# BUPT-GAMMA/GammaGL

Hardware: AMD Instinct MI355X
Metric: edges aggregated/sec, 3-layer GCN hidden=256 training step, ogbn-products-sized graph (higher is better)
Workload: dtype f32; 1 GPU; products: products-sized R-MAT, N=2449029, E=126167309 directed incl. self-loops, features 100->256x2->47, edge order=src, relabel=random, full-graph GCN train step (fwd+bwd+Adam), 6 aggregations/ste~; association=A (X W), hipgraph=no: eager launches, parallelism=1 GPU, rank0_local_edges=126167309, rank0_owned_rows=2449029, rank0_halo_rows=0, rank0_send_rows=0, matmul_precision=highest (IEEE f32), route=cpp

## Files before the change

### gammagl_amd/_lib.py

```python
import ctypes
import os
from ctypes import POINTER, c_char_p, c_float, c_int, c_int32, c_int64, c_size_t, c_void_p

import torch

_HERE = os.path.dirname(os.path.abspath(__file__))
HIP_LIB_PATH = os.path.join(_HERE, "lib", "libggl_mpops_hip.so")
HOST_LIB_PATH = os.path.join(_HERE, "lib", "libggl_mpops_host.so")

GGL_OK, GGL_EINVAL, GGL_EINDEX, GGL_EDTYPE, GGL_EHIP, GGL_EWORKSPACE = 0, -1, -2, -3, -4, -5
ABI_VERSION = 11


class SegPlanC(ctypes.Structure):

    _fields_ = [
        ("rowptr", c_void_p), ("perm", c_void_p), ("long_rows", c_void_p), ("chunk_ptr", c_void_p),
        ("n_long", c_int64), ("n_chunks", c_int64), ("chunk", c_int64), ("partial", c_void_p),
        ("N", c_int64), ("E", c_int64), ("row_order", c_void_p), ("xcd_run_rows", c_int64),
        ("long_order", c_void_p),
        ("max_len", c_int64),
    ]


# ... 30 lines not shown
    "ggl_plan_rows_bwd_rowptr": (c_int, [_V, _V, c_int64, c_int64, _V, _V, _V, _V, c_size_t, _V, POINTER(c_int64)]),
    "ggl_plan_rows_bwd_fill": (c_int, [_V, _V, _V, c_int64, _V, _V, _V, _V, _V]),
    "ggl_bias_grad_rows": (c_int, [_V, _V, c_int64, c_int64, c_int64, _V, _V, c_size_t, _V]),
    "ggl_partial_bytes": (c_size_t, [c_int, c_int64, c_int64, c_int]),
    "ggl_fill_i64": (c_int, [_V, c_int64, c_int64, _V]),
    "ggl_gather_i64_to_i32": (c_int, [_V, _V, c_int64, _V, _V]),
    "ggl_gather_rows_f32": (c_int, [_V, _V, c_int64, c_int64, _V, _V]),
    "ggl_gather_rows_f32_ex": (c_int, [_V, c_int64, _V, c_int64, c_int64, _V, c_int64, _V]),
    "ggl_ind2ptr_workspace_bytes": (c_size_t, [c_int64, c_int64]),
    "ggl_ind2ptr": (c_int, [_V, c_int64, c_int64, _V, _V, c_size_t, _V]),
    "ggl_ptr2ind": (c_int, [_V, c_int64, c_int64, _V, _V]),
    "ggl_sort_edges_workspace_bytes": (c_size_t, [c_int64, c_int64]),
    "ggl_sort_edges": (c_int, [_V, _V, c_int64, c_int64, _V, _V, c_size_t, _V]),
    "ggl_segment_sum": (c_int, [c_int, _V, _P, c_int64, _V, _V]),
    "ggl_segment_mean": (c_int, [c_int, _V, _P, c_int64, _V, _V]),
    "ggl_segment_max": (c_int, [c_int, _V, _P, c_int64, _V, _V, c_int64, _V]),
    "ggl_spmm_col_blocks": (c_int64, [c_int64, c_int64, c_int64]),
    "ggl_spmm_col_blocks_plan": (c_int64, [c_void_p, c_int64]),
    "ggl_segment_hub16_supported": (c_int, [c_int, c_int64, _V, _V]),
    "ggl_segment_hub16": (c_int, [c_int, c_int, _V, _P, c_int64, _V, _V]),
    "ggl_segment_sum_bwd": (c_int, [c_int, _V, _V, c_int64, c_int64, _V, _V]),
    "ggl_segment_mean_bwd": (c_int, [c_int, _V, _V, _V, c_int64, c_int64, _V, _V]),
    "ggl_segment_max_bwd": (c_int, [c_int, _V, _V, c_int64, c_int64, c_int64, _V, _V]),
    "ggl_spmm_sum": (c_int, [_P, _V, _V, c_int, _V, c_int64, _V, _V]),
    "ggl_spmm_sum_ex": (c_int, [_P, _V, _V, c_int, _V, c_int64, c_int64, _V, c_int64, c_int, _V]),
    "ggl_segment_sum_ex": (c_int, [c_int, _V, c_int64, _P, c_int64, _V, c_int64, c_int, _V]),
    "ggl_spmm_sum_bias_act": (c_int, [_P, _V, _V, c_int, _V, c_int64, _V, c_int, c_float, _V, _V, _V]),
    "ggl_spmm_mean": (c_int, [_P, _V, _V, c_int, _V, c_int64, _V, _V]),
    "ggl_spmm_max": (c_int, [_P, _V, _V, c_int, _V, c_int64, _V, _V, _V]),
    "ggl_spmm_mean_bwd": (c_int, [_P, _V, _V, c_int, _V, _V, c_int64, _V, _V]),
    "ggl_spmm_sum_x16": (c_int, [_P, _V, _V, c_int, c_int, _V, c_int64, c_int64, c_int, _V, c_int64, _V]),
    "ggl_spmm_mean_x16": (c_int, [_P, _V, _V, c_int, c_int, _V, c_int64, c_int64, c_int, _V, c_int64, _V]),
    "ggl_spmm_mean_bwd_x16": (c_int, [_P, _V, _V, c_int, c_int, _V, _V, c_int64, c_int, _V, _V]),
    "ggl_spmm_col_blocks_x16": (c_int64, [c_void_p, c_int64]),
    "ggl_spmm_max_bwd": (c_int, [_P, _V, _V, c_int, _V, _V, c_int64, _V, _V]),
    "ggl_spmm_max_bwd32": (c_int, [_P, _V, _V, c_int, _V, _V, c_int64, _V, _V]),
    "ggl_spmm_max_mask_bytes": (c_size_t, [c_int64, c_int64]),
    "ggl_spmm_max_mask": (c_int, [_P, _V, _V, c_int64, _V, _V]),
    "ggl_spmm_max_mask_words": (c_int64, [c_int64]),
    "ggl_spmm_max_bwd_mask": (c_int, [_P, _V, _V, c_int, _V, _V, _V, c_int64, _V, _V]),
    "ggl_bspmm_sum": (c_int, [_P, _V, _V, c_int, _V, c_int64, c_int64, _V, _V]),
    "ggl_bspmm_grad_w": (c_int, [_V, _V, _V, c_int64, c_int64, c_int64, _V, _V]),
    "ggl_bspmm_grad_w_sorted_scratch_bytes": (c_size_t, [c_int64, c_int64, c_int64, c_int64]),
    "ggl_bspmm_grad_w_sorted": (c_int, [_P, _V, _V, _V, _V, c_int64, c_int64, _V, _V, _V]),
    "ggl_spmm_grad_w_scratch_bytes": (c_size_t, [c_int64, c_int64, c_int64, c_int, c_int]),
    "ggl_spmm_grad_w": (c_int, [_P, _V, _V, c_int, _V, c_int, _V, _V, c_int64, _V, _V, _V]),
    "ggl_colsum_workspace_bytes": (c_size_t, [c_int64, c_int64]),
    "ggl_colsum_f32": (c_int, [_V, c_int64, c_int64, _V, _V, c_size_t, _V]),
    "ggl_bias_act_fwd": (c_int, [_V, _V, c_int64, c_int64, c_int, c_float, _V, _V, _V]),
    "ggl_bias_act_bwd_workspace_bytes": (c_size_t, [c_int64, c_int64]),
    "ggl_bias_act_bwd": (c_int, [_V, _V, c_int64, c_int64, c_int, c_float, _V, _V, _V, _V, c_size_t, _V]),
    "ggl_spmm_epi_ex": (c_int, [_P, _V, _V, c_int, _V, c_int64, c_int64, _V, c_int64, c_int, c_int, _V, c_int64,
                                _V, c_int, c_float, _V, c_int64, c_int64, c_int, _V]),
    "ggl_spmm_epi_x16": (c_int, [_P, _V, _V, c_int, c_int, _V, c_int64, c_int64, c_int, _V, c_int64, c_int, _V, c_int64,
                                 _V, c_int, c_float, _V, c_int64, c_int64, c_int, _V]),
    "ggl_bias_act_fwd_x16": (c_int, [c_int, _V, _V, c_int64, c_int64, c_int, c_float, _V, _V, _V]),
    "ggl_bias_act_bwd_x16": (c_int, [c_int, _V, _V, c_int64, c_int64, c_int, c_float, _V, _V, _V, _V, c_size_t, _V]),
    "ggl_segment_epi": (c_int, [_V, _P, c_int64, c_int, _V, c_int64, _V, c_int, c_float, _V, _V, _V]),
    "ggl_gat_fused_fwd": (c_int, [_P, _V, _V, _V, _V, c_float, c_int64, c_int64, c_float, _V, _V, _V, _V, _V]),
    "ggl_gat_partial_bytes": (c_size_t, [c_int64, c_int64, c_int64]),
    "ggl_gat_fused_bwd_dst": (c_int, [_P, _V, _V, _V, _V, _V, _V, _V, _V, _V, c_float, c_int64, c_int64,
                                      c_float, _V, _V, _V, _V, _V, _V]),
    "ggl_gat_fused_bwd_src": (c_int, [_P, _V, _V, _V, _V, _V, c_int64, c_int64, _V, _V, _V]),
    "ggl_edge_softmax_agg_fwd": (c_int, [_P, _V, _V, _V, c_int64, c_int64, c_float, _V, _V, _V, _V, _V]),
    "ggl_edge_softmax_agg_bwd_dst": (c_int, [_P, _V, _V, _V, _V, _V, _V, _V, c_int64, c_int64, c_float, _V, _V, _V, _V]),
    "ggl_edge_softmax_agg_bwd_src": (c_int, [_P, _V, _V, _V, _V, c_int64, c_int64, _V, _V]),
    "ggl_dot_attn_supported": (c_int, [c_int64, c_int64]),
    "ggl_policy_dot_attn_fused": (c_int, [c_int64, c_int64, c_int64, c_int64]),
    "ggl_dot_attn_fwd": (c_int, [_P, _V, _V, _V, _V, c_float, c_int64, c_int64, c_float, _V, _V, _V, _V, _V, _V]),
    "ggl_gat_fused_fwd_x16": (c_int, [_P, _V, _V, _V, c_int, _V, c_float, c_int64, c_int64, c_float, _V, c_int, _V, _V, _V,
                                      _V]),
    "ggl_gat_fused_bwd_dst_x16": (c_int, [_P, _V, _V, _V, c_int, _V, c_int, _V, c_int, _V, _V, _V, c_float, c_int64,
                                          c_int64, c_float, _V, _V, _V, _V, _V]),
    "ggl_gat_fused_bwd_src_x16": (c_int, [_P, _V, _V, _V, _V, c_int, _V, c_int64, c_int64, c_int, _V, _V, _V]),
    "ggl_gat_fast_supported": (c_int, [c_int64, c_int64]),
    "ggl_gat_fast_fwd": (c_int, [_P, _V, _V, _V, _V, c_int64, c_float, c_int64, c_int64, c_float, _V, _V, _V, _V, _V]),
    "ggl_gat_fast_bwd": (c_int, [_P, _V, _P, _V, _V, _V, _V, _V, _V, _V, _V, _V, c_float, c_int64, c_int64, c_float,
                                 _V, _V, _V, _V, _V, _V]),
    "ggl_gat_sh_supported": (c_int, [c_int64, c_int64, c_int64]),
    "ggl_gat_sh_partial_bytes": (c_size_t, [c_int64, c_int64]),
    "ggl_gat_sh_fwd": (c_int, [_P, _V, _V, _V, _V, c_int64, c_float, c_float, _V, _V, _V, _V, _V]),
    "ggl_gat_sh_stats": (c_int, [_V, _V, _V, _V, _V, c_int64, c_int64, _V, _V]),
    "ggl_gat_sh_bwd": (c_int, [_P, _V, _P, _V, _V, _V, _V, c_int64, _V, _V, _V, _V, c_int64, c_float, c_float, _V,
                               _V, _V, _V, _V]),
    "ggl_segment_softmax_supported": (c_int, [c_int64]),
    "ggl_segment_softmax_partial_bytes": (c_size_t, [c_int64, c_int64]),
    "ggl_segment_softmax_fwd": (c_int, [_V, _P, c_int64, _V, _V]),
    "ggl_segment_softmax_bwd": (c_int, [_V, _V, _P, c_int64, _V, _V]),
    "ggl_sample_count": (c_int, [_V, _V, c_int64, c_int64, c_int64, c_int, _V, _V]),
    "ggl_sample_pick": (c_int, [_V, _V, _V, c_int64, c_int64, c_int, _V, _V, _V, _V, _V]),
    "ggl_sample_hop_workspace_bytes": (c_size_t, [c_int64, c_int64]),
    "ggl_sample_hop": (c_int, [_V, _V, _V, _V, c_int64, c_int64, c_int64, c_int64, c_int64, _V, _V, _V, _V, _V, _V, _V,
                               _V, c_size_t, _V]),
    "ggl_sample_hop_ex": (c_int, [_V, _V, _V, _V, c_int64, c_int64, c_int64, c_int64, c_int64, _V, _V, _V, _V, _V, _V, _V,
                                  _V, c_size_t, _V, _V]),
    "ggl_block_transpose_workspace_bytes": (c_size_t, [c_int64, c_int64]),
    "ggl_block_transpose": (c_int, [_V, _V, c_int64, c_int64, c_int64, _V, _V, _V, c_size_t, _V]),
    "ggl_set_option": (c_int, [c_char_p, c_int64]),
    "ggl_get_option": (c_int64, [c_char_p]),
    "ggl_option_name": (c_char_p, [c_int]),
    "ggl_policy_chunk": (c_int64, [c_int64]),
    "ggl_policy_spmm_width": (c_int64, [c_int, c_int64, c_int64, c_int64]),
    "ggl_policy_head_channels": (c_int64, [c_int64, c_int64, c_int64]),
    "ggl_policy_mean_bwd_prescale": (c_int, [c_int64, c_int64]),
    "ggl_policy_gradw_sorted": (c_int, [c_int64, c_int64]),
    "ggl_policy_maxbwd_form": (c_int, [c_int64, c_int64, c_int64]),
# ... 46 lines not shown
```

### gammagl_amd/autograd.py

```python
import ctypes
import math

import torch
from torch.autograd.function import once_differentiable

from ._lib import _DTYPE_CODE, _X16_DTYPES, _ptr


def _flat(bias, add=None):
    return (bias.contiguous().reshape(-1) if bias is not None else None), (add.contiguous() if add is not None else None)


def segment_function(op):

    class Segment(torch.autograd.Function):
        @staticmethod
        def forward(ctx, eng, x, ids, N):
            ctx.eng = eng
            plan = eng.seg_plan(ids, N)
            out, _ = eng._segment_fwd(op, x, plan)
            ctx.save_for_backward(ids, *((plan.rowptr,) if op == "mean" else ()))
            ctx.x_shape = x.shape
            return out

# ... 539 lines not shown
        eng.spmm_epi_into(blk.plan, blk.col, None, x, y, mean=True, add=a, bias=b, relu=relu)
        ctx.blk, ctx.has_add = blk, add is not None
        ctx.epi = (relu, 0.0, None, None if bias is None else bias.shape)
        ctx.save_for_backward(y)
        return y

    @staticmethod
    def backward(ctx, g):
        eng = ctx.eng
        (y,) = ctx.saved_tensors
        ga, gb = eng._epi_bwd(g, y, *ctx.epi)
        gx = None
        if ctx.needs_input_grad[1]:
            blk = ctx.blk
            planT, dstT = blk.transposed()
            gx, _ = eng._spmm_fwd("mean_bwd", planT, dstT, None, ga, blk.n_src_cap, aux=blk.rowptr)
        return None, gx, None, (ga if ctx.has_add else None), gb, None


class SpMMRows(torch.autograd.Function):

    @staticmethod
    def forward(ctx, eng, gp, w, x, rows, bias):
        ctx.eng = eng
        dev = x.device
        K = int(x.shape[1])
        rp = eng.rows_plan(gp, w, rows)
        y = torch.empty((rp.R, K), dtype=torch.float32, device=dev)
        b, _ = _flat(bias)
        eng.spmm_epi_into(rp.fwd, rp.col, rp.w_fwd, x, y, bias=b)
        ctx.rp, ctx.bshape, ctx.K = rp, (None if bias is None else bias.shape), K
        return y

    @staticmethod
    @once_differentiable
    def backward(ctx, g):
        eng = ctx.eng
        rp, K = ctx.rp, ctx.K
        g = g.contiguous()
        dev = g.device
        gb = None
        if ctx.bshape is not None and ctx.needs_input_grad[5]:
            gb = torch.empty(K, dtype=torch.float32, device=dev)
            wsb = eng.lib.ggl_bias_act_bwd_workspace_bytes(rp.N_dst, K)
            ws = torch.empty(max(wsb, 4), dtype=torch.uint8, device=dev)
            eng._check(eng.lib.ggl_bias_grad_rows(_ptr(g), _ptr(rp.rows), rp.R, rp.N_dst, K, _ptr(gb), _ptr(ws), wsb,
                                                  eng._stream(dev)))
            gb = gb.reshape(ctx.bshape)
        gx = None
        if ctx.needs_input_grad[3]:
            gx = torch.empty((rp.N_src, K), dtype=torch.float32, device=dev)
            eng.spmm_sum_into(rp.bwd, rp.colT, rp.w_bwd, g, gx)
        return None, None, None, gx, None, gb
```

### gammagl_amd/cpp_ops.py

```python
import os

import torch

LIB_PATH = os.path.join(os.path.dirname(os.path.abspath(__file__)), "lib", "libggl_torch.so")
_loaded = False


def available():
    return os.path.exists(LIB_PATH)


def enabled():
    return available() and os.environ.get("GGL_CPP_OPS", "1") != "0"


def load():
    global _loaded
    if not _loaded:
        if not available():
            raise ImportError(f"{LIB_PATH} is not built: run `make -C gammagl_amd/csrc torch` "
                              f"(or __graft_entry__.build())")
        torch.ops.load_library(LIB_PATH)
        _loaded = True
    return torch.ops.ggl


def load_grad():
    load()
    return torch.ops.ggl_grad


def load_attn():
    load()
    return torch.ops.ggl_attn
```

### gammagl_amd/csrc/epilogue.hip

```cpp
#include "common.hpp"

namespace ggl {

struct alignas(8) H4 { uint16_t v[4]; };
template <typename T, int VEC> __device__ __forceinline__ void ldv(const typename TT<T>::S *__restrict__ p, float (&t)[VEC]) {
  if constexpr (!std::is_same<T, float>::value) {
    if (VEC == 4) {
      const H4 v = *reinterpret_cast<const H4 *>(p);
      t[0] = TT<T>::load(v.v[0]); t[1 % VEC] = TT<T>::load(v.v[1]); t[2 % VEC] = TT<T>::load(v.v[2]); t[3 % VEC] = TT<T>::load(v.v[3]);
    } else {
      t[0] = TT<T>::load(p[0]);
    }
  } else if (VEC == 4) {
    const float4 v = *reinterpret_cast<const float4 *>(p);
    t[0] = v.x; t[1 % VEC] = v.y; t[2 % VEC] = v.z; t[3 % VEC] = v.w;
  } else {
    t[0] = p[0];
  }
}
template <typename T, int VEC> __device__ __forceinline__ void stv(typename TT<T>::S *__restrict__ p, const float (&t)[VEC]) {
  if constexpr (!std::is_same<T, float>::value) {
    if (VEC == 4) {
      H4 o;
      o.v[0] = TT<T>::store(t[0]); o.v[1] = TT<T>::store(t[1 % VEC]); o.v[2] = TT<T>::store(t[2 % VEC]); o.v[3] = TT<T>::store(t[3 % VEC]);
// ... 125 lines not shown
      float gv[VEC], yv[VEC];
      ldv<T, VEC>(g + r * K + c * VEC, gv);
      if (MASKED == 1 || MASKED == 2) ldv<T, VEC>(y + r * K + c * VEC, yv);
      else yv[0] = 0.0f;
      finish(r, gv, yv);
    }
    if (partial) {
#pragma unroll
      for (int i = 0; i < VEC; ++i) partial[(block_id() * groups + j) * K + c * VEC + i] = acc[i];
    }
  }
}

static inline void geometry(int64_t N, int64_t K, bool vec4, int *kp, int *groups, int64_t *blocks,
                            int64_t *rpb) {
  const int64_t KV = vec4 ? K / 4 : K;
  *kp = (int)(KV < kBlock ? (KV > 0 ? KV : 1) : kBlock);
  *groups = kBlock / *kp;
  int64_t b = ceil_div(N > 0 ? N : 1, (int64_t)*groups * 8);
  if (b > 4096) b = 4096;
  if (b < 1) b = 1;
  *blocks = b;
  *rpb = ceil_div(N > 0 ? N : 1, b);
}

__global__ __launch_bounds__(kBlock) void bias_grad_rows_kernel(const float *__restrict__ g, const int64_t *__restrict__ rows,
                                                                int64_t R, int64_t N, int64_t K, int64_t nblocks,
                                                                int64_t rows_per_block, int kp, int groups,
                                                                float *__restrict__ partial) {
  const int j = threadIdx.x / kp;
  const int c0 = threadIdx.x - j * kp;
  if (j >= groups || block_id() >= nblocks) return;
  const int64_t KV = K / 4;
  const int64_t r0 = block_id() * rows_per_block;
  const int64_t r1 = (r0 + rows_per_block < N) ? r0 + rows_per_block : N;
  int64_t lo = 0, hi = R;
  while (lo < hi) {
    const int64_t mid = (lo + hi) >> 1;
    if (rows[mid] < r0) lo = mid + 1; else hi = mid;
  }
  for (int64_t c = c0; c < KV; c += kp) {
    float acc[4] = {0.0f, 0.0f, 0.0f, 0.0f};
    for (int64_t i = lo; i < R; ++i) {
      const int64_t r = rows[i];
      if (r >= r1) break;
      if ((int)(r - r0) % groups != j) continue;
      float gv[4];
      ldv<float, 4>(g + i * K + c * 4, gv);
#pragma unroll
      for (int k = 0; k < 4; ++k) acc[k] = __fadd_rn(acc[k], gv[k]);
    }
#pragma unroll
    for (int k = 0; k < 4; ++k) partial[(block_id() * groups + j) * K + c * 4 + k] = acc[k];
  }
}

int rng_advance(int64_t *rng_state, void *stream) {
  GGL_LAUNCH((rng_advance_kernel), 1, 64, as_stream(stream), rng_state, (int64_t)1);
  GGL_LAUNCH_CHECK();
  return GGL_OK;
}

}

using namespace ggl;

template <typename T> static inline bool aligned_v4(const void *p) {
  return (reinterpret_cast<uintptr_t>(p) & (4 * sizeof(typename TT<T>::S) - 1)) == 0;
}

template <typename T>
static int bias_act_fwd(const typename TT<T>::S *a, const float *bias, int64_t N, int64_t K, int relu, float p_drop,
                        int64_t *rng_state, typename TT<T>::S *y, void *stream) {
  GGL_REQUIRE(N >= 0 && K >= 0 && p_drop >= 0.0f && p_drop < 1.0f, GGL_EINVAL, "bad arguments");
  const int64_t total = N * K;
  if (total == 0) return GGL_OK;
  GGL_REQUIRE(a && y, GGL_EINVAL, "NULL pointer");
  GGL_REQUIRE(p_drop == 0.0f || rng_state, GGL_EINVAL, "dropout needs an rng_state");
  uint32_t thresh;
  float scale;
  dropout_params(p_drop, &thresh, &scale);
  hipStream_t s = as_stream(stream);
  const bool vec4 = (K % 4 == 0) && aligned_v4<T>(a) && aligned_v4<T>(y);
  int kp, groups;
  int64_t grid, rpb;
  geometry(N, K, vec4, &kp, &groups, &grid, &rpb);
  if (vec4)
    GGL_LAUNCH((bias_act_fwd_kernel<T, 4>), grid, kBlock, s, a, bias, (const int64_t *)rng_state, y, N, K, grid, rpb,
               kp, groups, relu, thresh, scale);
  else
    GGL_LAUNCH((bias_act_fwd_kernel<T, 1>), grid, kBlock, s, a, bias, (const int64_t *)rng_state, y, N, K, grid, rpb,
               kp, groups, relu, thresh, scale);
  GGL_LAUNCH_CHECK();
  if (thresh) return rng_advance(rng_state, stream);
  return GGL_OK;
}

extern "C" int ggl_bias_act_fwd(const float *a, const float *bias, int64_t N, int64_t K, int relu,
                                float p_drop, int64_t *rng_state, float *y, void *stream) {
  return bias_act_fwd<float>(a, bias, N, K, relu, p_drop, rng_state, y, stream);
}

static int x16_dtype_ok(int dtype, const char *what) {
  if (dtype == GGL_F16 || dtype == GGL_BF16) return GGL_OK;
  set_error("x16: %s must be f16 or bf16 (got dtype code %d)", what, dtype);
  return GGL_EDTYPE;
// ... 29 lines not shown
                        void *workspace, size_t workspace_bytes, void *stream) {
  GGL_REQUIRE(N >= 0 && K >= 0 && p_drop >= 0.0f && p_drop < 1.0f, GGL_EINVAL, "bad arguments");
  if (K == 0) return GGL_OK;
  GGL_REQUIRE((g && ga) || N == 0, GGL_EINVAL, "NULL pointer");
  const bool redraw = p_drop > 0.0f && rng_used != nullptr && !relu;
  const int masked = relu ? 1 : (redraw ? 3 : (p_drop > 0.0f ? 2 : 0));
  uint32_t thresh;
  float scale;
  dropout_params(p_drop, &thresh, &scale);
  GGL_REQUIRE(!masked || masked == 3 || y || N == 0, GGL_EINVAL, "y is needed to rebuild the ReLU/dropout mask");
  GGL_REQUIRE(!gbias || (workspace && workspace_bytes >= ggl_bias_act_bwd_workspace_bytes(N, K)),
              GGL_EWORKSPACE, "bias_act_bwd workspace too small");
  const bool vec4 = (K % 4 == 0) && aligned_v4<T>(g) && aligned_v4<T>(ga) && (!masked || masked == 3 || aligned_v4<T>(y));
  int kp, groups;
  int64_t blocks, rpb;
  geometry(N, K, vec4, &kp, &groups, &blocks, &rpb);
  hipStream_t s = as_stream(stream);
  float *partial = gbias ? static_cast<float *>(workspace) : nullptr;
#define GGL_BAB(V, M)                                                                                    \
  GGL_LAUNCH((bias_act_bwd_kernel<T, V, M>), blocks, kBlock, s, g, y, ga, N, K, blocks, rpb, kp, groups, scale, \
             redraw ? rng_used : nullptr, thresh, partial)
  if (vec4) {
    if (masked == 0) GGL_BAB(4, 0); else if (masked == 1) GGL_BAB(4, 1); else if (masked == 2) GGL_BAB(4, 2); else GGL_BAB(4, 3);
  } else {
    if (masked == 0) GGL_BAB(1, 0); else if (masked == 1) GGL_BAB(1, 1); else if (masked == 2) GGL_BAB(1, 2); else GGL_BAB(1, 3);
  }
#undef GGL_BAB
  GGL_LAUNCH_CHECK();
  if (gbias) {
    const size_t part = bwd_partial_bytes(N, K);
    return ggl_colsum_f32(partial, blocks * groups, K, gbias, static_cast<char *>(workspace) + part,
                          workspace_bytes - part, stream);
  }
  return GGL_OK;
}

extern "C" int ggl_bias_act_bwd(const float *g, const float *y, int64_t N, int64_t K, int relu,
                                float p_drop, const int64_t *rng_used, float *ga, float *gbias,
                                void *workspace, size_t workspace_bytes, void *stream) {
  return bias_act_bwd<float>(g, y, N, K, relu, p_drop, rng_used, ga, gbias, workspace, workspace_bytes, stream);
}

extern "C" int ggl_bias_act_bwd_x16(int dtype, const void *g, const void *y, int64_t N, int64_t K, int relu, float p_drop,
                                    const int64_t *rng_used, void *ga, float *gbias, void *workspace,
                                    size_t workspace_bytes, void *stream) {
  if (int rc = x16_dtype_ok(dtype, "g / y / ga")) return rc;
  const uint16_t *g16 = static_cast<const uint16_t *>(g), *y16 = static_cast<const uint16_t *>(y);
  uint16_t *ga16 = static_cast<uint16_t *>(ga);
  return dtype == GGL_BF16
             ? bias_act_bwd<mxbf16_t>(g16, y16, N, K, relu, p_drop, rng_used, ga16, gbias, workspace, workspace_bytes, stream)
             : bias_act_bwd<mxf16_t>(g16, y16, N, K, relu, p_drop, rng_used, ga16, gbias, workspace, workspace_bytes, stream);
}

extern "C" int ggl_bias_grad_rows(const float *g, const int64_t *rows, int64_t R, int64_t N, int64_t K, float *gbias,
                                  void *workspace, size_t workspace_bytes, void *stream) {
  GGL_REQUIRE(R >= 0 && N >= 0 && R <= N && K > 0 && K % 4 == 0, GGL_EINVAL,
              "bias_grad_rows needs R <= N rows of a multiple of 4 columns");
  GGL_REQUIRE(gbias && ((g && rows) || R == 0), GGL_EINVAL, "NULL pointer");
  GGL_REQUIRE(aligned16(g), GGL_EINVAL, "g must be 16-byte aligned");
  GGL_REQUIRE(workspace && workspace_bytes >= ggl_bias_act_bwd_workspace_bytes(N, K), GGL_EWORKSPACE,
              "bias_grad_rows workspace too small (ggl_bias_act_bwd_workspace_bytes(N, K))");
  int kp, groups;
  int64_t blocks, rpb;
  geometry(N, K, true, &kp, &groups, &blocks, &rpb);
  float *partial = static_cast<float *>(workspace);
  GGL_LAUNCH((bias_grad_rows_kernel), blocks, kBlock, as_stream(stream), g, rows, R, N, K, blocks, rpb, kp, groups, partial);
  GGL_LAUNCH_CHECK();
  const size_t part = bwd_partial_bytes(N, K);
  return ggl_colsum_f32(partial, blocks * groups, K, gbias, static_cast<char *>(workspace) + part, workspace_bytes - part,
                        stream);
}
```

### gammagl_amd/csrc/reduce.hip

```cpp
#include "common.hpp"

namespace ggl {

enum Mode {
  MODE_SEG = 0,
  MODE_SPMM = 1,
  MODE_BSPMM = 2,
  MODE_MEANBWD = 3,
  MODE_MAXBWD = 4,
  MODE_SPMM_EPI = 5,
  MODE_SEG_EPI = 6,
  MODE_MAXBWD32 = 7,
  MODE_MAXBWDM = 8
};
constexpr bool maxbwd_like(int mode) { return mode == MODE_MAXBWD || mode == MODE_MAXBWD32 || mode == MODE_MAXBWDM; }
constexpr bool spmm_like(int mode) { return mode == MODE_SPMM || mode == MODE_SPMM_EPI; }
constexpr bool seg_like(int mode) { return mode == MODE_SEG || mode == MODE_SEG_EPI; }
constexpr bool epi_mode(int mode) { return mode == MODE_SPMM_EPI || mode == MODE_SEG_EPI; }

enum IdxMode { IDX_RUNTIME = -1, IDX_NONE = 0, IDX_DIRECT = 1, IDX_PERM = 2 };

struct ReduceDims {
  int64_t N, K, E;
  int64_t arg_fill;
  int64_t chunk;
  int64_t nblocks;
  int64_t H, C;
  int64_t n_long, n_chunks;
  int64_t chunk_blocks;
  int exact_long;
  int logL;
  int swizzle;
  int w_by_pos;
  int64_t x_ld, out_ld;
  int accumulate;
  int epi_relu;
  int epi_vec;
  uint32_t epi_thresh;
  float epi_scale;
  int64_t epi_K, epi_col0;
  int64_t add_ld;
  int64_t mask_words;
  int64_t mask_col0;
};

template <typename S> struct RPtrs {
  const S *__restrict__ x;
  const int32_t *__restrict__ perm;
  const int32_t *__restrict__ col;
  const float *__restrict__ w;
  const int64_t *__restrict__ rowptr;
  const int64_t *__restrict__ aux_rowptr;
  const int64_t *__restrict__ aux_arg;
  const float *__restrict__ epi_bias;
  const int64_t *__restrict__ epi_rng;
  const S *__restrict__ epi_add;
};

template <typename S, int VEC> struct VecIO {
  static __device__ __forceinline__ void load(const S *__restrict__ p, S (&v)[VEC]) {
#pragma unroll
    for (int i = 0; i < VEC; ++i) v[i] = p[i];
  }
  static __device__ __forceinline__ void store(S *__restrict__ p, const S (&v)[VEC]) {
#pragma unroll
    for (int i = 0; i < VEC; ++i) p[i] = v[i];
  }
};
template <> struct VecIO<float, 4> {
  static __device__ __forceinline__ void load(const float *__restrict__ p, float (&v)[4]) {
    const float4 t = *reinterpret_cast<const float4 *>(p);
    v[0] = t.x; v[1] = t.y; v[2] = t.z; v[3] = t.w;
  }
  static __device__ __forceinline__ void store(float *__restrict__ p, const float (&v)[4]) {
    float4 t;
    t.x = v[0]; t.y = v[1]; t.z = v[2]; t.w = v[3];
    *reinterpret_cast<float4 *>(p) = t;
  }
};

template <> struct VecIO<float, 8> {
  static __device__ __forceinline__ void load(const float *__restrict__ p, float (&v)[8]) {
    const float4 t = *reinterpret_cast<const float4 *>(p), u = *reinterpret_cast<const float4 *>(p + 4);
    v[0] = t.x; v[1] = t.y; v[2] = t.z; v[3] = t.w; v[4] = u.x; v[5] = u.y; v[6] = u.z; v[7] = u.w;
  }
  static __device__ __forceinline__ void store(float *__restrict__ p, const float (&v)[8]) {
    float4 t, u;
    t.x = v[0]; t.y = v[1]; t.z = v[2]; t.w = v[3]; u.x = v[4]; u.y = v[5]; u.z = v[6]; u.w = v[7];
    *reinterpret_cast<float4 *>(p) = t;
    *reinterpret_cast<float4 *>(p + 4) = u;
  }
};
template <> struct VecIO<uint16_t, 8> {
  static __device__ __forceinline__ void load(const uint16_t *__restrict__ p, uint16_t (&v)[8]) {
    const uint4 t = *reinterpret_cast<const uint4 *>(p);
    v[0] = (uint16_t)t.x; v[1] = (uint16_t)(t.x >> 16); v[2] = (uint16_t)t.y; v[3] = (uint16_t)(t.y >> 16);
// ... 184 lines not shown
      for (int u = 0; u < TB; ++u) accumulate(raw[u], xrow[u], wv[u], who[u]);
    }
  }
  const int rem = (int)(end - p);
  if (rem > 0) {
    int64_t xrow[TB], who[TB];
    float wv[TB];
    S raw[TB][VEC];
#pragma unroll
    for (int u = 0; u < TB - 1; ++u)
      if (u < rem) element(p + u, xrow[u], wv[u], who[u]);
#pragma unroll
    for (int u = 0; u < TB - 1; ++u)
      if (u < rem) RowIO<S, VEC, RAG>::load(q.x + xrow[u] * d.x_ld + kk, raw[u], nv);
#pragma unroll
    for (int u = 0; u < TB - 1; ++u)
      if (u < rem) accumulate(raw[u], xrow[u], wv[u], who[u]);
  }
}

template <typename T, int VEC, int OP>
__device__ __forceinline__ void init_acc(typename TT<T>::A (&acc)[VEC], argreg_t (&arg)[VEC],
                                         int64_t arg_fill) {
#pragma unroll
  for (int i = 0; i < VEC; ++i) {
    acc[i] = (OP == OP_MAX) ? TT<T>::lowest() : TT<T>::zero();
    arg[i] = (argreg_t)arg_fill;
  }
}

template <typename T, int VEC, int OP, bool RAG = false>
__device__ __forceinline__ void seed_acc(const ReduceDims &d, const typename TO<T>::O *__restrict__ out,
                                         int64_t row, int64_t kk, typename TT<T>::A (&acc)[VEC]) {
  if (OP == OP_SUM && d.accumulate) {
    typename TO<T>::O o[VEC];
    RowIO<typename TO<T>::O, VEC, RAG>::load(out + row * d.out_ld + kk, o, valid_lanes<VEC, RAG>(d.K, kk));
#pragma unroll
    for (int i = 0; i < VEC; ++i) acc[i] = TO<T>::oload(o[i]);
  }
}

template <typename S, int VEC> struct EpiPre {
  float b[VEC];
  S a[VEC];
  uint32_t rw[VEC > 4 ? VEC : 4];
};
constexpr bool epi_late(int vec) { return vec > 4; }
template <int VEC, bool RAG>
__device__ __forceinline__ void epi_words(const int64_t *__restrict__ rng, const ReduceDims &d, int64_t row, int64_t kg, int nv,
                                          uint32_t (&rw)[VEC > 4 ? VEC : 4]) {
#pragma unroll
  for (int i = 0; i < (VEC > 4 ? VEC : 4); ++i) rw[i] = 0xffffffffu;
  if (!d.epi_thresh) return;
  const int64_t ev = d.epi_vec;
  const int sh = ev == 4 ? 2 : 0;
  const int64_t KV = (d.epi_K + ev - 1) >> sh;
  if (VEC > 1 && ev == 1 && (RAG || VEC > 4)) {
#pragma unroll
    for (int i = 0; i < VEC; ++i)
      rw[i] = i < nv ? philox4x32_10((uint64_t)(row * KV + kg + i), (uint64_t)rng[1], (uint64_t)rng[0]).x : 0xffffffffu;
  } else {
#pragma unroll
    for (int v = 0; v < (VEC > 4 ? VEC / 4 : 1); ++v) {
      const U4 u = philox4x32_10((uint64_t)(row * KV + (kg >> sh) + v), (uint64_t)rng[1], (uint64_t)rng[0]);
      rw[4 * v] = u.x; rw[4 * v + 1] = u.y; rw[4 * v + 2] = u.z; rw[4 * v + 3] = u.w;
    }
  }
}
template <typename T, int VEC, int MODE, bool RAG>
__device__ __forceinline__ void epi_prefetch(const RPtrs<typename TT<T>::S> &q, const ReduceDims &d, int64_t row,
                                             int64_t kk, EpiPre<typename TT<T>::S, VEC> &pre) {
  if (!epi_mode(MODE)) return;
  using S = typename TT<T>::S;
  const int nv = valid_lanes<VEC, RAG>(d.K, kk);
#pragma unroll
  for (int i = 0; i < VEC; ++i) pre.b[i] = (q.epi_bias && (!RAG || i < nv)) ? q.epi_bias[kk + i] : 0.0f;
  if (q.epi_add) RowIO<S, VEC, RAG>::load(q.epi_add + row * d.add_ld + kk, pre.a, nv);
  epi_words<VEC, RAG>(q.epi_rng, d, row, d.epi_col0 + kk, nv, pre.rw);
}

template <typename T, int VEC, int OP, int MODE, bool RAG = false>
__device__ __forceinline__ void finish_row(const RPtrs<typename TT<T>::S> &q, const ReduceDims &d,
                                           typename TO<T>::O *__restrict__ out,
                                           int64_t *__restrict__ argout, int64_t K, int64_t row,
                                           int64_t len, int64_t kk, typename TT<T>::A (&acc)[VEC],
                                           const argreg_t (&arg)[VEC], const EpiPre<typename TT<T>::S, VEC> &pre) {
  using O = typename TO<T>::O;
  const int nv = valid_lanes<VEC, RAG>(K, kk);
  if (OP == OP_MEAN) {
    if (seg_like(MODE)) {
      const typename TT<T>::A c = TT<T>::count(len);
      if (TT<T>::gt1(c)) {
#pragma unroll
        for (int i = 0; i < VEC; ++i) acc[i] = TT<T>::div(acc[i], c);
      }
    } else {
      if (len > 0) {
#pragma unroll
        for (int i = 0; i < VEC; ++i) acc[i] = (typename TT<T>::A)__fdiv_rn((float)acc[i], (float)len);
      }
    }
  }
  if (epi_mode(MODE)) {
    const int64_t ev = d.epi_vec;
    const int64_t kg = d.epi_col0 + kk;
    const uint32_t (&rw)[VEC > 4 ? VEC : 4] = pre.rw;
// ... 145 lines not shown
    init_acc<T, 1, OP>(acc, arg, d.arg_fill);
    seed_acc<T, 1, OP>(d, out, row, k, acc);
    for (int64_t c = c0; c < c1; ++c) {
      const A v = TO<T>::pload(partial[c * d.K + k]);
      if (OP == OP_MAX) {
        if (TT<T>::less(acc[0], v)) {
          acc[0] = v;
          arg[0] = (argreg_t)partial_arg[c * d.K + k];
        }
      } else {
        acc[0] = TT<T>::add(acc[0], v);
      }
    }
    EpiPre<typename TT<T>::S, 1> pre;
    epi_prefetch<T, 1, MODE, false>(q, d, row, k, pre);
    finish_row<T, 1, OP, MODE>(q, d, out, argout, d.K, row, len, k, acc, arg, pre);
  }
}

struct ReduceArgs {
  const void *x;
  const int32_t *perm;
  const int32_t *col;
  const float *w;
  int w_by_pos;
  const int64_t *rowptr;
  int64_t N, K, E;
  void *out;
  int64_t *arg;
  int64_t arg_fill;
  int64_t chunk;
  int64_t H, C;
  const int64_t *aux_rowptr;
  const int64_t *aux_arg;
  const int32_t *long_rows;
  const int64_t *chunk_ptr;
  const int32_t *row_order;
  const int32_t *long_order;
  int64_t max_len;
  int64_t xcd_run_rows;
  int64_t n_long, n_chunks;
  void *partial;
  int64_t *partial_arg;
  int64_t x_ld, out_ld;
  int accumulate;
  const float *epi_bias;
  const int64_t *epi_rng;
  int epi_relu;
  uint32_t epi_thresh;
  float epi_scale;
  const void *epi_add;
  int64_t add_ld;
  int64_t epi_K, epi_col0;
  int phase;
  int hub_forked;
  int64_t mask_words;
};

static inline int pow2_ceil_log2(int64_t v) {
  int l = 0;
  while (((int64_t)1 << l) < v) ++l;
  return l;
}

#define GGL_RPTR_ARGS(S)                                                                           \
  static_cast<const S *>(a.x), a.perm, a.col, a.w, a.rowptr, a.aux_rowptr, a.aux_arg, a.epi_bias, a.epi_rng, static_cast<const S *>(a.epi_add)

template <typename T, int OP, int MODE> constexpr bool exact_long_mode() {
  return OP != OP_MAX && ((std::is_same<T, float>::value && (seg_like(MODE) || spmm_like(MODE) || MODE == MODE_BSPMM)) ||
                          (std::is_same<T, double>::value && (MODE == MODE_SEG)) ||
                          (mx_code<T>::value != 0 && spmm_like(MODE)));
}

template <typename T, int OP, int MODE> static bool exact_long_applies(const ReduceArgs &a) {
#ifdef GGL_EMULATE
  return false;
#else
  if constexpr (exact_long_mode<T, OP, MODE>())
    return a.n_long > 0 && options().exact_long_rows != 0 && a.E < ((int64_t)1 << 31) &&
           (options().exact_long_max <= 0 || a.max_len <= options().exact_long_max);
  return false;
#endif
}

template <typename T, int MODE> static HubF32Args hub_args_of(const ReduceArgs &a, int64_t x_ld) {
  HubF32Args h{};
  constexpr int kWords = std::is_same<T, double>::value ? 2 : 1;
  h.f64 = kWords == 2 ? 1 : 0;
  h.x16 = mx_code<T>::value;
  h.x = reinterpret_cast<const float *>(a.x);
  h.x_ld = x_ld * kWords;
  h.perm = a.perm;
  h.col = seg_like(MODE) ? nullptr : a.col;
  h.w = seg_like(MODE) ? nullptr : a.w;
  h.w_by_pos = a.w_by_pos;
  h.H = a.H;
  h.C = (MODE == MODE_BSPMM) ? a.C : 0;
  h.rowptr = a.rowptr;
  h.long_rows = a.long_rows;
  h.long_order = a.long_order;
  h.n_long = a.n_long;
  h.K = a.K * kWords;
  h.partial = static_cast<float *>(a.partial);
  h.avg_long_len = a.n_chunks * a.chunk / (a.n_long > 0 ? a.n_long : 1);
  return h;
}
// ... 30 lines not shown
  }
#endif
  const int64_t grid = d.chunk_blocks + d.nblocks;
  GGL_REQUIRE(grid < ((int64_t)1 << 31), GGL_EINVAL, "grid too large");
  const int32_t *order = (options().row_order && (!uniform || options().row_order > 1)) ? a.row_order : nullptr;
#define GGL_RR_ARGS GGL_RPTR_ARGS(S), order, a.long_rows, a.chunk_ptr, static_cast<P *>(a.partial), a.partial_arg, out, a.arg, d
  if (a.phase == 2) {
  } else if (uniform) {
    if constexpr (!RAG) {
      if (std::is_same<T, float>::value && VEC == 4 && OP == OP_SUM && spmm_like(MODE) &&
          options().unroll >= 8) {
        GGL_LAUNCH((row_reduce_kernel<T, VEC, OP, MODE, IDX, std::is_same<T, float>::value, 8>), grid,
                   kBlock, stream, GGL_RR_ARGS);
      } else {
        GGL_LAUNCH((row_reduce_kernel<T, VEC, OP, MODE, IDX, std::is_same<T, float>::value, 4>), grid,
                   kBlock, stream, GGL_RR_ARGS);
      }
    }
  } else if (!RAG && (OP != OP_MAX || options().unroll_narrow_max) && d.logL <= 2 && options().unroll_narrow > 4) {
    GGL_LAUNCH((row_reduce_kernel<T, VEC, OP, MODE, IDX, false, 16>), grid, kBlock, stream, GGL_RR_ARGS);
  } else {
    GGL_LAUNCH((row_reduce_kernel<T, VEC, OP, MODE, IDX, false, 4, RAG>), grid, kBlock, stream, GGL_RR_ARGS);
  }
#undef GGL_RR_ARGS
  GGL_LAUNCH_CHECK();
  if (a.phase == 1) return GGL_OK;
#ifndef GGL_EMULATE
  if (forked) {
    const int rc = hub_f32_join(stream, forked);
    if (rc) return rc;
  }
#endif
  if (a.n_long > 0) {
    GGL_LAUNCH((long_final_kernel<T, OP, MODE>), a.n_long, kBlock, stream, a.rowptr, a.long_rows,
               a.chunk_ptr, static_cast<const P *>(a.partial), (const int64_t *)a.partial_arg, out,
               a.arg, a.epi_bias, a.epi_rng, static_cast<const S *>(a.epi_add), d);
    GGL_LAUNCH_CHECK();
  }
  return GGL_OK;
}

template <typename T, int VEC, int OP, int MODE, bool STATIC_IDX, bool RAG = false>
static int launch_typed(const ReduceArgs &a, hipStream_t stream) {
  ReduceDims d{};
  d.N = a.N; d.K = a.K; d.E = a.E; d.arg_fill = a.arg_fill; d.chunk = a.chunk; d.H = a.H; d.C = a.C;
  d.n_long = a.n_long; d.n_chunks = a.n_chunks; d.w_by_pos = a.w_by_pos;
  d.x_ld = a.x_ld > 0 ? a.x_ld : a.K; d.out_ld = a.out_ld > 0 ? a.out_ld : a.K; d.accumulate = a.accumulate;
  d.epi_relu = a.epi_relu; d.epi_thresh = a.epi_thresh; d.epi_scale = a.epi_scale;
  d.epi_K = a.epi_K > 0 ? a.epi_K : a.K; d.epi_col0 = a.epi_col0;
  d.epi_vec = (d.epi_K % 4 == 0) ? 4 : 1;
  d.add_ld = a.add_ld > 0 ? a.add_ld : a.K;
  d.mask_words = a.mask_words;
  d.mask_col0 = 0;
  const int64_t kv = ceil_div(a.K, VEC);
  d.logL = pow2_ceil_log2(kv < kWave ? kv : kWave);
  if (d.logL > 6) d.logL = 6;
  const int rows_per_block = kWavesPerBlock * (kWave >> d.logL);
  d.nblocks = ceil_div(a.N, rows_per_block);
  d.swizzle = (int)options().xcd_swizzle;
  if (a.xcd_run_rows > 0 && !d.swizzle) {
    const int64_t run_blocks = a.xcd_run_rows / rows_per_block;
    if (run_blocks >= 2 && d.nblocks >= 16 * run_blocks) d.swizzle = (int)run_blocks;
  }
  GGL_REQUIRE(d.nblocks < ((int64_t)1 << 30), GGL_EINVAL, "too many rows for one launch");
  GGL_REQUIRE(!RAG || (a.K >= VEC && !a.accumulate), GGL_EINVAL, "ragged rows: K >= the lane vector, no accumulate");
  if (a.N <= 0 || a.K <= 0) return GGL_OK;
  if constexpr (!STATIC_IDX || RAG) {
    return launch_idx<T, VEC, OP, MODE, IDX_RUNTIME, RAG>(a, d, stream);
  } else if constexpr (seg_like(MODE)) {
    if (a.perm) return launch_idx<T, VEC, OP, MODE, IDX_PERM>(a, d, stream);
    return launch_idx<T, VEC, OP, MODE, IDX_DIRECT>(a, d, stream);
  } else {
    if (!a.w) return launch_idx<T, VEC, OP, MODE, IDX_NONE>(a, d, stream);
    if (a.w_by_pos || !a.perm) return launch_idx<T, VEC, OP, MODE, IDX_DIRECT>(a, d, stream);
    return launch_idx<T, VEC, OP, MODE, IDX_PERM>(a, d, stream);
  }
}

template <int OP, int MODE>
static int launch_f32(const ReduceArgs &a, hipStream_t stream) {
  constexpr bool kStatic = (seg_like(MODE) || spmm_like(MODE) || MODE == MODE_MAXBWDM);
  const bool vec4 = !options().force_generic && (a.K % 4 == 0) && aligned16(a.x) &&
                    aligned16(a.out) && (!a.partial || aligned16(a.partial)) &&
                    (a.x_ld % 4 == 0) && (a.out_ld % 4 == 0) && (MODE != MODE_BSPMM || a.C % 4 == 0) &&
                    (!a.epi_add || (aligned16(a.epi_add) && a.add_ld % 4 == 0));
  if (vec4) return launch_typed<float, 4, OP, MODE, kStatic>(a, stream);
  if constexpr (seg_like(MODE) || spmm_like(MODE)) {
    if (!options().force_generic && options().ragged4 && a.K >= 32 && a.K <= 128 && !a.accumulate &&
        (OP != OP_MAX || spmm_like(MODE) || options().ragged_max))
      return launch_typed<float, 4, OP, MODE, kStatic, true>(a, stream);
  }
  return launch_typed<float, 1, OP, MODE, kStatic>(a, stream);
}

static int64_t col_block_width(int64_t E, int64_t K, int64_t N, int64_t xcd_run_rows = 0) {
  if (N > 0 && E < options().col_block_min_degree * N) return 0;
  int64_t bw = options().col_block;
  if (bw > 0 && E < options().col_block_min_edges) bw *= 2;
  else if (bw > 0 && xcd_run_rows > 0 && K >= 4 * bw && K % (2 * bw) == 0) bw *= 2;
  if (bw <= 0 || bw % 4 != 0 || K < 2 * bw || K % 4 != 0) return 0;
  if (K % bw != 0 && K <= 256) return 0;
  return bw;
}
extern "C" int64_t ggl_spmm_col_blocks(int64_t E, int64_t K, int64_t N) {
  const int64_t bw = col_block_width(E, K, N);
  return bw > 0 ? (K + bw - 1) / bw : 1;
// ... 275 lines not shown
}

extern "C" int ggl_spmm_sum(const ggl_segplan_t *plan, const int32_t *col, const float *w,
                            int w_by_pos, const float *x, int64_t K, float *out, void *stream) {
  return ggl_spmm_sum_ex(plan, col, w, w_by_pos, x, 0, K, out, 0, 0, stream);
}

extern "C" int ggl_spmm_sum_ex(const ggl_segplan_t *plan, const int32_t *col, const float *w, int w_by_pos,
                               const float *x, int64_t x_ld, int64_t K, float *out, int64_t out_ld,
                               int accumulate, void *stream) {
  ReduceArgs a{};
  int rc = spmm_common(a, plan, col, w, w_by_pos, x, K, out, false);
  if (rc) return rc;
  GGL_REQUIRE((x_ld == 0 || x_ld >= K) && (out_ld == 0 || out_ld >= K), GGL_EINVAL, "row stride < K");
  a.x_ld = x_ld; a.out_ld = out_ld; a.accumulate = accumulate ? 1 : 0;
  return launch_f32_cols<OP_SUM, MODE_SPMM>(a, as_stream(stream));
}

static int fill_epilogue(ReduceArgs &a, const void *add, int64_t add_ld, const float *bias, int relu, float p_drop,
                         int64_t *rng_state) {
  GGL_REQUIRE(p_drop >= 0.0f && p_drop < 1.0f, GGL_EINVAL, "p_drop must be in [0, 1)");
  GGL_REQUIRE(p_drop == 0.0f || rng_state, GGL_EINVAL, "dropout needs an rng_state");
  a.epi_bias = bias;
  a.epi_add = add; a.add_ld = add_ld;
  a.epi_rng = rng_state;
  a.epi_relu = relu ? 1 : 0;
  dropout_params(p_drop, &a.epi_thresh, &a.epi_scale);
  return GGL_OK;
}

extern "C" int ggl_spmm_epi_ex(const ggl_segplan_t *plan, const int32_t *col, const float *w, int w_by_pos,
                               const float *x, int64_t x_ld, int64_t K, float *out, int64_t out_ld,
                               int accumulate, int mean, const float *add, int64_t add_ld, const float *bias,
                               int relu, float p_drop, int64_t *rng_state, int64_t epi_K, int64_t epi_col0,
                               int advance_rng, void *stream) {
  ReduceArgs a{};
  int rc = spmm_common(a, plan, col, w, w_by_pos, x, K, out, false);
  if (rc) return rc;
  GGL_REQUIRE((x_ld == 0 || x_ld >= K) && (out_ld == 0 || out_ld >= K) && (add_ld == 0 || add_ld >= K),
              GGL_EINVAL, "row stride < K");
  GGL_REQUIRE(!(mean && accumulate), GGL_EINVAL, "mean cannot accumulate onto a partial result");
  rc = fill_epilogue(a, add, add_ld, bias, relu, p_drop, rng_state);
  if (rc) return rc;
  GGL_REQUIRE(epi_col0 >= 0 && (epi_K == 0 || epi_col0 + K <= epi_K), GGL_EINVAL, "column block outside the row");
  a.x_ld = x_ld; a.out_ld = out_ld; a.accumulate = accumulate ? 1 : 0;
  a.epi_K = epi_K; a.epi_col0 = epi_col0;
  rc = !mean ? launch_f32_cols<OP_SUM, MODE_SPMM_EPI>(a, as_stream(stream))
             : launch_f32_cols<OP_MEAN, MODE_SPMM_EPI>(a, as_stream(stream));
  if (rc) return rc;
  if (a.epi_thresh && advance_rng && plan->N > 0 && K > 0) return rng_advance(rng_state, stream);
  return GGL_OK;
}

extern "C" int ggl_spmm_sum_bias_act(const ggl_segplan_t *plan, const int32_t *col, const float *w,
                                     int w_by_pos, const float *x, int64_t K, const float *bias, int relu,
                                     float p_drop, int64_t *rng_state, float *out, void *stream) {
  return ggl_spmm_epi_ex(plan, col, w, w_by_pos, x, 0, K, out, 0, 0, 0, nullptr, 0, bias, relu, p_drop, rng_state, 0, 0, 1,
                         stream);
}

extern "C" int ggl_segment_epi(const float *x, const ggl_segplan_t *plan, int64_t K, int mean, const float *add,
                               int64_t add_ld, const float *bias, int relu, float p_drop, int64_t *rng_state,
                               float *out, void *stream) {
  ReduceArgs a{};
  int rc = fill_plan(a, plan, GGL_F32, K, false);
  if (rc) return rc;
  GGL_REQUIRE((x || plan->E * K == 0) && (out || plan->N * K == 0), GGL_EINVAL, "x/out is NULL");
  GGL_REQUIRE(add_ld == 0 || add_ld >= K, GGL_EINVAL, "row stride < K");
  rc = fill_epilogue(a, add, add_ld, bias, relu, p_drop, rng_state);
  if (rc) return rc;
  a.x = x;
  a.out = out;
  rc = mean ? launch_f32<OP_MEAN, MODE_SEG_EPI>(a, as_stream(stream))
            : launch_f32<OP_SUM, MODE_SEG_EPI>(a, as_stream(stream));
  if (rc) return rc;
  if (a.epi_thresh && plan->N > 0 && K > 0) return rng_advance(rng_state, stream);
  return GGL_OK;
}

extern "C" int ggl_spmm_mean(const ggl_segplan_t *plan, const int32_t *col, const float *w,
                             int w_by_pos, const float *x, int64_t K, float *out, void *stream) {
  ReduceArgs a{};
  int rc = spmm_common(a, plan, col, w, w_by_pos, x, K, out, false);
  if (rc) return rc;
  return launch_f32_cols<OP_MEAN, MODE_SPMM>(a, as_stream(stream));
}

extern "C" int ggl_spmm_max(const ggl_segplan_t *plan, const int32_t *col, const float *w,
                            int w_by_pos, const float *x, int64_t K, float *out, int64_t *argsrc,
                            void *stream) {
  ReduceArgs a{};
  int rc = spmm_common(a, plan, col, w, w_by_pos, x, K, out, true);
  if (rc) return rc;
  GGL_REQUIRE(argsrc || plan->N * K == 0, GGL_EINVAL, "argsrc is NULL");
  a.arg = argsrc;
  a.arg_fill = 0;
  return launch_f32<OP_MAX, MODE_SPMM>(a, as_stream(stream));
}

extern "C" int ggl_spmm_mean_bwd(const ggl_segplan_t *planT, const int32_t *colT, const float *w,
                                 int w_by_pos, const float *g, const int64_t *fwd_rowptr, int64_t K,
                                 float *gx, void *stream) {
  ReduceArgs a{};
  int rc = spmm_common(a, planT, colT, w, w_by_pos, g, K, gx, false);
  if (rc) return rc;
  GGL_REQUIRE(fwd_rowptr != nullptr, GGL_EINVAL, "fwd_rowptr is NULL");
// ... 295 lines not shown
```

### gammagl_amd/csrc/torch/ggl_torch.cpp

```cpp
#include <ATen/ATen.h>
#include <ATen/core/dispatch/Dispatcher.h>
#include <c10/core/DeviceGuard.h>
#include <c10/hip/HIPGraphsC10Utils.h>
#include <c10/hip/HIPStream.h>
#include <dlfcn.h>
#include <torch/csrc/autograd/custom_function.h>
#include <torch/library.h>

#include <cstdlib>
#include <cstring>
#include <list>
#include <memory>
#include <mutex>
#include <string>

#include "ggl_mpops.h"

namespace ggl_torch {

using at::Tensor;
using torch::autograd::AutogradContext;
using torch::autograd::variable_list;

#define GGL_FNS(X)                                                                                                  \
  X(ggl_abi_version) X(ggl_last_error) X(ggl_plan_workspace_bytes) X(ggl_plan_build) X(ggl_plan_long_workspace_bytes) \
  X(ggl_plan_long_count) X(ggl_plan_long_fill) X(ggl_partial_bytes) X(ggl_gather_i64_to_i32) X(ggl_gather_rows_f32)  \
  X(ggl_segment_sum) X(ggl_segment_mean) X(ggl_segment_max) X(ggl_segment_hub16_supported) X(ggl_segment_hub16)      \
  X(ggl_segment_sum_bwd) X(ggl_segment_mean_bwd) X(ggl_segment_max_bwd) X(ggl_spmm_sum) X(ggl_spmm_mean)             \
  X(ggl_spmm_max) X(ggl_spmm_mean_bwd) X(ggl_spmm_max_bwd) X(ggl_bspmm_sum) X(ggl_bspmm_grad_w)                      \
  X(ggl_bspmm_grad_w_sorted_scratch_bytes) X(ggl_bspmm_grad_w_sorted)                                                \
  X(ggl_spmm_grad_w_scratch_bytes) X(ggl_spmm_grad_w)                                                                \
  X(ggl_gat_partial_bytes) X(ggl_gat_fused_fwd) X(ggl_gat_fused_bwd_dst) X(ggl_gat_fused_bwd_src)                      \
  X(ggl_gat_fused_fwd_x16) X(ggl_gat_fused_bwd_dst_x16) X(ggl_gat_fused_bwd_src_x16)                                    \
  X(ggl_edge_softmax_agg_fwd) X(ggl_edge_softmax_agg_bwd_dst) X(ggl_edge_softmax_agg_bwd_src)                          \
  X(ggl_dot_attn_supported) X(ggl_policy_dot_attn_fused) X(ggl_dot_attn_fwd)                                           \
  X(ggl_gat_fast_supported) X(ggl_gat_fast_fwd) X(ggl_gat_fast_bwd) X(ggl_bias_act_fwd)                                \
  X(ggl_bias_act_bwd_workspace_bytes) X(ggl_bias_act_bwd) X(ggl_spmm_epi_ex) X(ggl_segment_epi)                        \
  X(ggl_sample_hop_workspace_bytes) X(ggl_sample_hop)                                                                \
  X(ggl_policy_chunk) X(ggl_policy_spmm_width) X(ggl_policy_head_channels) X(ggl_policy_mean_bwd_prescale)            \
  X(ggl_policy_gradw_sorted) X(ggl_policy_xcd_run_rows) X(ggl_policy_row_order)                                     \
  X(ggl_spmm_max_mask_bytes) X(ggl_spmm_max_mask) X(ggl_spmm_max_bwd_mask) X(ggl_get_option)                         \
  X(ggl_spmm_max_bwd32) X(ggl_policy_maxbwd_form)                                                                   \
  X(ggl_segment_softmax_supported) X(ggl_segment_softmax_partial_bytes) X(ggl_segment_softmax_fwd) X(ggl_segment_softmax_bwd) \
  X(ggl_policy_softmax_sublanes) X(ggl_spmm_sum_x16) X(ggl_spmm_mean_x16) X(ggl_spmm_mean_bwd_x16)                    \
  X(ggl_plan_rows_workspace_bytes) X(ggl_plan_rows_rank) X(ggl_plan_rows_fwd_rowptr) X(ggl_plan_rows_fwd_fill)        \
  X(ggl_plan_rows_bwd_rowptr) X(ggl_plan_rows_bwd_fill) X(ggl_bias_grad_rows)                                          \
  X(ggl_spmm_epi_x16) X(ggl_bias_act_fwd_x16) X(ggl_bias_act_bwd_x16)

struct Api {
  void *handle = nullptr;
  std::string path;
#define X(n) decltype(&::n) n = nullptr;
  GGL_FNS(X)
#undef X
};

static std::string here() {
  Dl_info info;
  if (dladdr(reinterpret_cast<void *>(&here), &info) == 0 || info.dli_fname == nullptr) return ".";
  std::string p(info.dli_fname);
  auto slash = p.rfind('/');
  return slash == std::string::npos ? "." : p.substr(0, slash);
}

static Api load(const char *env, const char *file, const char *what) {
  Api a;
  const char *over = std::getenv(env);
  a.path = over != nullptr ? std::string(over) : here() + "/" + file;
  a.handle = dlopen(a.path.c_str(), RTLD_NOW | RTLD_LOCAL);
  TORCH_CHECK(a.handle != nullptr, "gammagl_amd: cannot load ", a.path, " (", dlerror(), "): ", what,
              " tensors are served by this library only — build it with `make -C gammagl_amd/csrc`");
#define X(n)                                                                     \
  a.n = reinterpret_cast<decltype(a.n)>(dlsym(a.handle, #n));                    \
  TORCH_CHECK(a.n != nullptr, "gammagl_amd: ", a.path, " does not export " #n);
  GGL_FNS(X)
#undef X
  TORCH_CHECK(a.ggl_abi_version() == GGL_ABI_VERSION, "gammagl_amd: ", a.path, " has C ABI version ",
              a.ggl_abi_version(), ", this binding was built against ", GGL_ABI_VERSION);
  return a;
}

static const Api &api_for(const c10::Device &d) {
  if (d.is_cuda()) {
    static const Api hip = load("GGL_TORCH_HIP_LIB", "libggl_mpops_hip.so", "GPU");
    return hip;
  }
  TORCH_CHECK(d.is_cpu(), "gammagl_amd: no kernels for device ", d);
  static const Api host = load("GGL_TORCH_HOST_LIB", "libggl_mpops_host.so", "CPU");
  return host;
}

static void check(const Api &a, int rc) {
  if (rc == GGL_OK) return;
  const char *m = a.ggl_last_error();
  std::string msg(m != nullptr ? m : "");
  TORCH_CHECK_INDEX(rc != GGL_EINDEX, msg);
  TORCH_CHECK(false, "ggl_mpops error ", rc, ": ", msg);
}

static void *stream_of(const c10::Device &d) {
// ... 1257 lines not shown
  const Api &a = api_for(x.device());
  const int64_t K = s.x.size(1);
  if (add.defined()) {
    if (x16) {
      TORCH_CHECK(add.scalar_type() == s.x.scalar_type(), "expected scalar type Float (add in x's dtype, ", s.x.scalar_type(),
                  ") but found ", add.scalar_type(), " (add)");
    } else {
      f32("add", add);
    }
    TORCH_CHECK(add.dim() == 2 && add.size(0) == s.gp->N_dst && add.size(1) == K, "add must be [destination rows, feature width]");
    add = add.contiguous();
  }
  if (bias.defined()) {
    f32("bias", bias);
    bias = bias.contiguous().reshape({-1});
    TORCH_CHECK(bias.numel() == K, "bias must hold one value per column");
  }
  const SegPlan &p_ = *s.gp->fwd;
  Tensor y = at::empty({s.gp->N_dst, K}, s.x.options());
  Tensor part;
  if (x16) {
    if (p_.n_long > 0)
      part = at::empty({static_cast<int64_t>(a.ggl_partial_bytes(GGL_F32, p_.n_chunks, K, 0)) + 16}, s.x.options().dtype(at::kByte));
  } else {
    part = partial_for(a, p_, s.x, K, false);
  }
  ggl_segplan_t cs = p_.c(part);
  Tensor keep;
  auto [wp, by_pos] = weights_for(a, *s.gp, p_, s.w, keep);
  const Draw d = draw(x.device(), p);
  if (x16) {
    const int xc = dtype_code(s.x);
    check(a, a.ggl_spmm_epi_x16(&cs, s.gp->col.data_ptr<int32_t>(), wp, by_pos, xc, s.x.data_ptr(), K, K, xc, y.data_ptr(), K,
                                mean ? 1 : 0, add.defined() ? add.data_ptr() : nullptr, add.defined() ? K : 0,
                                bias.defined() ? bias.data_ptr<float>() : nullptr, relu ? 1 : 0, static_cast<float>(p), d.ptr(),
                                0, 0, 1, stream_of(x.device())));
    return {y, d.used};
  }
  check(a, a.ggl_spmm_epi_ex(&cs, s.gp->col.data_ptr<int32_t>(), wp, by_pos, s.x.data_ptr<float>(), K, K, y.data_ptr<float>(),
                             K, 0, mean ? 1 : 0, add.defined() ? add.data_ptr<float>() : nullptr, add.defined() ? K : 0,
                             bias.defined() ? bias.data_ptr<float>() : nullptr, relu ? 1 : 0, static_cast<float>(p),
                             d.ptr(), 0, 0, 1, stream_of(x.device())));
  return {y, d.used};
}

struct RowsPlan {
  int64_t R = 0, N_dst = 0, N_src = 0;
  Tensor rows, col, colT, w_fwd, w_bwd;
  std::shared_ptr<SegPlan> fwd, bwd;
  bool has_w = false;
  const void *w_storage = nullptr;
  int64_t w_offset = 0, w_version = 0;
  c10::optional<c10::weak_intrusive_ptr<c10::StorageImpl>> w_ref;
};

static Cache<RowsPlan> &rows_cache() {
  static Cache<RowsPlan> c(8);
  return c;
}

static std::shared_ptr<SegPlan> plan_from_rowptr(const Api &a, const Tensor &rowptr, int64_t E, int64_t chunk, void *st) {
  auto p = std::make_shared<SegPlan>();
  p->N = rowptr.size(0) - 1;
  p->E = E;
  p->chunk = chunk;
  p->rowptr = rowptr;
  p->sorted = true;
  p->max_len = p->N > 0 ? p->counts().max().item<int64_t>() : 0;
  fill_long_rows(a, *p, st);
  p->uid = ++g_plans_built;
  return p;
}

static std::shared_ptr<RowsPlan> rows_plan(GraphPlan &gp, const Tensor &index, const Tensor &w, const Tensor &rows_in) {
  TORCH_CHECK(rows_in.dim() == 1 && rows_in.scalar_type() == at::kLong, "rows must be a 1-D int64 tensor, got ", rows_in.sizes(),
              " ", rows_in.scalar_type());
  const void *w_storage = w.defined() ? w.storage().unsafeGetStorageImpl() : nullptr;
  const int64_t w_offset = w.defined() ? w.storage_offset() : 0;
  const int64_t w_version = (w.defined() && !w.is_inference()) ? static_cast<int64_t>(w._version()) : 0;
  TensorKey k = TensorKey::of(rows_in, static_cast<int64_t>(gp.fwd->uid),
                              static_cast<int64_t>(reinterpret_cast<uintptr_t>(w_storage)));
  if (auto hit = rows_cache().get(k)) {
    if (hit->has_w == w.defined() && hit->w_storage == w_storage && hit->w_offset == w_offset && hit->w_version == w_version &&
        (!hit->has_w || !hit->w_ref->expired())) {
      ++g_plan_hits;
      return hit;
    }
  }
  const auto dev = rows_in.device();
  TORCH_CHECK(!capturing(dev), "spmm_rows: the restricted plan of this row list must be built before a hipGraph capture "
                               "(run one eager step first)");
  const Api &a = api_for(dev);
  void *st = stream_of(dev);
  gp.need_bwd(index);
  Tensor rows = rows_in.contiguous();
  const int64_t R = rows.size(0), N = gp.N_dst, E = gp.E;
  auto i64 = rows.options(), i32 = rows.options().dtype(at::kInt), f32o = rows.options().dtype(at::kFloat);
  const size_t wsb = a.ggl_plan_rows_workspace_bytes(E, std::max(gp.N_dst, gp.N_src), R);
  Tensor ws = at::empty({static_cast<int64_t>(wsb)}, rows.options().dtype(at::kByte));
  Tensor rank = at::empty({std::max<int64_t>(N, 1)}, i32);
  check(a, a.ggl_plan_rows_rank(rows.data_ptr<int64_t>(), R, N, rank.data_ptr<int32_t>(), ws.data_ptr(), wsb, st));
  auto rp = std::make_shared<RowsPlan>();
  rp->R = R;
  rp->N_dst = gp.N_dst;
  rp->N_src = gp.N_src;
  rp->rows = rows;
// ... 33 lines not shown
                                       const OptT_ &bias_) {
  c10::OptionalDeviceGuard guard(x.device());
  SpArgs s = spmm_args(index, weight, x);
  Tensor bias = opt(bias_);
  same_device({&x, &rows, &bias});
  TORCH_CHECK(s.x.dim() == 2 && s.x.size(1) > 0 && s.x.size(1) % 4 == 0,
              "spmm_rows needs a 2-D f32 x whose width is a multiple of 4, got ", x.sizes());
  const Api &a = api_for(x.device());
  const int64_t K = s.x.size(1);
  if (bias.defined()) {
    f32("bias", bias);
    bias = bias.contiguous().reshape({-1});
    TORCH_CHECK(bias.numel() == K, "bias must hold one value per column");
  }
  auto rp = rows_plan(*s.gp, index, s.w, rows);
  const SegPlan &p_ = *rp->fwd;
  Tensor y = at::empty({rp->R, K}, s.x.options());
  Tensor part = partial_for(a, p_, s.x, K, false);
  ggl_segplan_t cs = p_.c(part);
  check(a, a.ggl_spmm_epi_ex(&cs, rp->col.data_ptr<int32_t>(), rp->has_w ? rp->w_fwd.data_ptr<float>() : nullptr, 1,
                             s.x.data_ptr<float>(), K, K, y.data_ptr<float>(), K, 0, 0, nullptr, 0,
                             bias.defined() ? bias.data_ptr<float>() : nullptr, 0, 0.0f, nullptr, 0, 0, 1, stream_of(x.device())));
  return y;
}

static std::tuple<Tensor, Tensor> spmm_rows_backward_kernel(const Tensor &index, const OptT_ &weight, const Tensor &grad,
                                                            const Tensor &rows, int64_t n_src, bool has_bias) {
  Tensor g = grad.contiguous(), w = opt_dense(weight);
  f32("grad", g);
  if (w.defined()) f32("weight", w);
  c10::OptionalDeviceGuard guard(g.device());
  const Api &a = api_for(g.device());
  auto gp = bwd_plan(index, n_src);
  auto rp = rows_plan(*gp, index, w, rows);
  TORCH_CHECK(g.dim() == 2 && g.size(0) == rp->R && g.size(1) % 4 == 0, "grad must be [len(rows), K], K a multiple of 4");
  const int64_t K = g.size(1);
  void *st = stream_of(g.device());
  Tensor gb = at::empty({has_bias ? K : 0}, g.options());
  if (has_bias) {
    const size_t wsb = a.ggl_bias_act_bwd_workspace_bytes(rp->N_dst, K);
    Tensor ws = at::empty({static_cast<int64_t>(std::max<size_t>(wsb, 4))}, g.options().dtype(at::kByte));
    check(a, a.ggl_bias_grad_rows(g.data_ptr<float>(), rp->rows.data_ptr<int64_t>(), rp->R, rp->N_dst, K, gb.data_ptr<float>(),
                                  ws.data_ptr(), wsb, st));
  }
  const SegPlan &p_ = *rp->bwd;
  Tensor gx = at::empty({rp->N_src, K}, g.options());
  Tensor part = partial_for(a, p_, g, K, false);
  ggl_segplan_t cs = p_.c(part);
  check(a, a.ggl_spmm_sum(&cs, rp->colT.data_ptr<int32_t>(), rp->has_w ? rp->w_bwd.data_ptr<float>() : nullptr, 1,
                          g.data_ptr<float>(), K, gx.data_ptr<float>(), st));
  return {gx, gb};
}

static Tensor segment_epi_forward_kernel(const Tensor &x_, const Tensor &index, int64_t N, bool mean, const OptT_ &add_,
                                         const OptT_ &bias_, bool relu) {
  seg_args(x_, index);
  Tensor x = x_.contiguous(), add = opt(add_), bias = opt(bias_);
  same_device({&x, &add, &bias});
  f32("msg", x);
  TORCH_CHECK(x.dim() == 2, "segment_epi expects [E, K] messages");
  c10::OptionalDeviceGuard guard(x.device());
  const Api &a = api_for(x.device());
  auto plan = seg_plan(index, N);
  const int64_t K = x.size(1);
  if (add.defined()) {
    f32("add", add);
    TORCH_CHECK(add.dim() == 2 && add.size(0) == N && add.size(1) == K, "add must be [num_segments, feature width]");
    add = add.contiguous();
  }
  if (bias.defined()) {
    f32("bias", bias);
    bias = bias.contiguous().reshape({-1});
    TORCH_CHECK(bias.numel() == K, "bias must hold one value per column");
  }
  Tensor y = at::empty({N, K}, x.options());
  Tensor part = partial_for(a, *plan, x, K, false);
  ggl_segplan_t cs = plan->c(part);
  check(a, a.ggl_segment_epi(x.data_ptr<float>(), &cs, K, mean ? 1 : 0, add.defined() ? add.data_ptr<float>() : nullptr, 0,
                             bias.defined() ? bias.data_ptr<float>() : nullptr, relu ? 1 : 0, 0.0f, nullptr,
                             y.data_ptr<float>(), stream_of(x.device())));
  return y;
}

static std::tuple<Tensor, Tensor, Tensor, Tensor, Tensor> sample_hop_kernel(const Tensor &rowptr, const Tensor &col,
                                                                            const Tensor &seeds, const Tensor &n_seeds,
                                                                            int64_t num_nodes, int64_t fanout, int64_t e_cap,
                                                                            int64_t s_cap, Tensor &first_pos) {
  same_device({&rowptr, &col, &seeds, &n_seeds, &first_pos});
  const Tensor *all5[5] = {&rowptr, &col, &seeds, &n_seeds, &first_pos};
  for (const Tensor *t : all5)
    TORCH_CHECK(t->scalar_type() == at::kLong && t->is_contiguous(), "sample_hop takes contiguous int64 tensors");
  TORCH_CHECK(fanout > 0 && first_pos.numel() >= num_nodes && rowptr.numel() == num_nodes + 1, "bad sample_hop arguments");
  c10::OptionalDeviceGuard guard(rowptr.device());
  const Api &a = api_for(rowptr.device());
  const int64_t b_cap = seeds.size(0);
  auto i64 = rowptr.options();
  Tensor out_rowptr = at::empty({b_cap + 1}, i64), out_col = at::empty({std::max<int64_t>(e_cap, 1)}, i64.dtype(at::kInt));
  Tensor out_eid = at::empty({std::max<int64_t>(e_cap, 1)}, i64), out_nid = at::empty({s_cap}, i64), counts = at::empty({3}, i64);
  const size_t wsb = a.ggl_sample_hop_workspace_bytes(b_cap, e_cap);
  Tensor ws = at::empty({static_cast<int64_t>(wsb)}, i64.dtype(at::kByte));
  Tensor rng = rng_state(rowptr.device());
  check(a, a.ggl_sample_hop(rowptr.data_ptr<int64_t>(), col.data_ptr<int64_t>(), seeds.data_ptr<int64_t>(),
                            n_seeds.data_ptr<int64_t>(), b_cap, num_nodes, fanout, e_cap, s_cap, rng.data_ptr<int64_t>(),
                            first_pos.data_ptr<int64_t>(), out_rowptr.data_ptr<int64_t>(), out_col.data_ptr<int32_t>(),
                            out_eid.data_ptr<int64_t>(), out_nid.data_ptr<int64_t>(), counts.data_ptr<int64_t>(), ws.data_ptr(),
                            wsb, stream_of(rowptr.device())));
// ... 359 lines not shown
    ctx->saved_data["p"] = p;
    ctx->saved_data["has_add"] = opt(add).defined();
    save_bias(ctx, bias);
    return std::get<0>(r);
  }
  static variable_list backward(AutogradContext *ctx, variable_list grads) {
    auto s = ctx->get_saved_variables();
    auto [ga, gb] = epi_backward(ctx, grads[0], s[2], ctx->saved_data["p"].toDouble(), s[3]);
    OptT_ w = s[1].defined() ? OptT_(s[1]) : OptT_();
    static auto sum_bwd = op_handle<SpSig>("ggl::spmm_sum_backward");
    static auto mean_bwd = op_handle<SpSig>("ggl::spmm_mean_backward");
    const bool mean = ctx->saved_data["mean"].toBool();
    Tensor gx = mean ? mean_bwd.call(s[0], w, ga) : sum_bwd.call(s[0], w, ga);
    return {Tensor(), grad_w(s, 4, ga, mean), gx, Tensor(), ctx->saved_data["has_add"].toBool() ? ga : Tensor(), gb, Tensor(),
            Tensor()};
  }
};
static Tensor spmm_epi_autograd(const Tensor &index, const OptT_ &weight, const Tensor &x, bool mean, const OptT_ &add,
                                const OptT_ &bias, bool relu, double p) {
  if (x.dim() == 2 && (x.size(1) % 4 == 0 || is_x16(x))) return SpMMEpiFn::apply(index, weight, x, mean, add, bias, relu, p);
  Tensor out = mean ? spmm_mean_autograd(index, weight, x) : spmm_sum_autograd(index, weight, x);
  if (opt(add).defined()) out = out + *add;
  return BiasActFn::apply(out, bias, relu, p);
}

struct SpMMRowsFn : public torch::autograd::Function<SpMMRowsFn> {
  static Tensor forward(AutogradContext *ctx, const Tensor &index, const OptT_ &weight, const Tensor &x, const Tensor &rows,
                        const OptT_ &bias) {
    at::AutoDispatchBelowADInplaceOrView below;
    static auto op = op_handle<Tensor(const Tensor &, const OptT_ &, const Tensor &, const Tensor &, const OptT_ &)>(
        "ggl::spmm_rows_forward");
    Tensor y = op.call(index, weight, x, rows, bias);
    ctx->save_for_backward({index, opt(weight), rows});
    ctx->saved_data["n_src"] = x.size(0);
    save_bias(ctx, bias);
    return y;
  }
  static variable_list backward(AutogradContext *ctx, variable_list grads) {
    auto s = ctx->get_saved_variables();
    static auto op = op_handle<std::tuple<Tensor, Tensor>(const Tensor &, const OptT_ &, const Tensor &, const Tensor &, int64_t,
                                                          bool)>("ggl::spmm_rows_backward");
    OptT_ w = s[1].defined() ? OptT_(s[1]) : OptT_();
    auto r = op.call(s[0], w, grads[0], s[2], ctx->saved_data["n_src"].toInt(), has_bias(ctx));
    return {Tensor(), Tensor(), std::get<0>(r), Tensor(), bias_grad(ctx, std::get<1>(r))};
  }
};
static Tensor spmm_rows_autograd(const Tensor &index, const OptT_ &weight, const Tensor &x, const Tensor &rows,
                                 const OptT_ &bias) {
  TORCH_CHECK(!(opt(weight).defined() && opt(weight).requires_grad()),
              "spmm_rows has no gradient for the edge weights: pass detached weights (bspmm_sum is the op with a weight gradient)");
  return SpMMRowsFn::apply(index, weight, x, rows, bias);
}

struct SegEpiFn : public torch::autograd::Function<SegEpiFn> {
  static Tensor forward(AutogradContext *ctx, const Tensor &x, const Tensor &index, int64_t N, bool mean, const OptT_ &add,
                        const OptT_ &bias, bool relu) {
    at::AutoDispatchBelowADInplaceOrView below;
    static auto op = op_handle<Tensor(const Tensor &, const Tensor &, int64_t, bool, const OptT_ &, const OptT_ &, bool)>(
        "ggl::segment_epi_forward");
    Tensor y = op.call(x, index, N, mean, add, bias, relu);
    ctx->save_for_backward({index, y});
    ctx->saved_data["x_shape"] = x.sizes().vec();
    ctx->saved_data["N"] = N;
    ctx->saved_data["mean"] = mean;
    ctx->saved_data["relu"] = relu;
    ctx->saved_data["has_add"] = opt(add).defined();
    save_bias(ctx, bias);
    return y;
  }
  static variable_list backward(AutogradContext *ctx, variable_list grads) {
    auto s = ctx->get_saved_variables();
    auto [ga, gb] = epi_backward(ctx, grads[0], s[1], 0.0, at::empty({0}, s[0].options()));
    auto shape = ctx->saved_data["x_shape"].toIntVector();
    Tensor gx;
    if (ctx->saved_data["mean"].toBool()) {
      static auto op = op_handle<Tensor(const Tensor &, const Tensor &, int64_t, c10::IntArrayRef)>("ggl::segment_mean_backward");
      gx = op.call(ga, s[0], ctx->saved_data["N"].toInt(), shape);
    } else {
      static auto op = op_handle<Tensor(const Tensor &, const Tensor &, c10::IntArrayRef)>("ggl::segment_sum_backward");
      gx = op.call(ga, s[0], shape);
    }
    return {gx, Tensor(), Tensor(), Tensor(), ctx->saved_data["has_add"].toBool() ? ga : Tensor(), gb, Tensor()};
  }
};
static Tensor segment_epi_autograd(const Tensor &x, const Tensor &index, int64_t N, bool mean, const OptT_ &add,
                                   const OptT_ &bias, bool relu) {
  return SegEpiFn::apply(x, index, N, mean, add, bias, relu);
}

static Tensor seg_meta(const Tensor &x, const Tensor &, int64_t N) { return at::empty(out_shape(x, N), x.options()); }
static std::tuple<Tensor, Tensor> seg_max_meta(const Tensor &x, const Tensor &, int64_t N) {
  return {at::empty(out_shape(x, N), x.options()), at::empty(out_shape(x, N), x.options().dtype(at::kLong))};
}
static Tensor like_x_meta(const Tensor &, const OptT &, const Tensor &x) { return at::empty_like(x); }
static Tensor x16_meta(const Tensor &, const OptT &, const Tensor &x, bool out_f32) {
  return out_f32 ? at::empty(x.sizes(), x.options().dtype(at::kFloat)) : at::empty_like(x);
}
static Tensor spmm_grad_w_meta(const Tensor &index, const Tensor &, const Tensor &g, bool) {
  return at::empty({index.size(1)}, g.options().dtype(at::kFloat));
}
static std::tuple<Tensor, Tensor> spmm_max_arg_meta(const Tensor &, const OptT &, const Tensor &x) {
  return {at::empty_like(x), at::empty(x.sizes(), x.options().dtype(at::kLong))};
}
static Tensor bspmm_meta(const Tensor &, const Tensor &, const Tensor &x) { return at::empty_like(x); }
static Tensor softmax_meta(const Tensor &x, const Tensor &, int64_t) { return at::empty_like(x); }
static Tensor softmax_bwd_meta(const Tensor &, const Tensor &y, const Tensor &, int64_t) { return at::empty_like(y); }
// ... 53 lines not shown
          at::empty({0}, o.dtype(at::kLong)), keep ? at::empty({index.size(1), v.size(1)}, o) : at::empty({0}, o)};
}
static std::tuple<Tensor, Tensor, Tensor> dot_bwd_meta(const Tensor &, const Tensor &q, const Tensor &k, const Tensor &v, const Tensor &,
                                                       const Tensor &, const Tensor &, const Tensor &, const Tensor &, const Tensor &,
                                                       int64_t, double, double, bool need_q, bool need_k, bool need_v) {
  auto e = [&]() { return at::empty({0}, v.options()); };
  return {need_q ? at::empty_like(q) : e(), need_k ? at::empty_like(k) : e(), need_v ? at::empty_like(v) : e()};
}
static Tensor dot_meta(const Tensor &, const Tensor &q, const Tensor &, const Tensor &v, c10::optional<int64_t> n,
                       c10::optional<double>, double) {
  const int64_t N = n.has_value() ? *n : q.size(0);
  if (v.dim() == 2) return at::empty({N, v.size(1)}, v.options());
  return at::empty({N, v.size(1), v.size(2)}, v.options());
}
static std::tuple<Tensor, Tensor, Tensor, Tensor, bool> gat_csr_fwd_meta(const Tensor &rp, const Tensor &, const Tensor &,
                                                                         const Tensor &, const Tensor &, const Tensor &,
                                                                         const Tensor &, const Tensor &x, double, double) {
  const int64_t n = rp.size(0) - 1;
  auto o = x.options(), f = x.options().dtype(at::kFloat);
  return {at::empty({n, x.size(1), x.size(2)}, o), at::empty({n, x.size(1)}, f), at::empty({n, x.size(1)}, f),
          at::empty({0}, o.dtype(at::kLong)), false};
}
static std::tuple<Tensor, Tensor, Tensor> gat_csr_bwd_meta(const Tensor &, const Tensor &, const Tensor &, const Tensor &,
                                                           const Tensor &, const Tensor &el, const Tensor &er, const Tensor &x,
                                                           const Tensor &, const Tensor &, const Tensor &, const Tensor &,
                                                           const Tensor &, double, double, bool) {
  return {at::empty_like(el), at::empty_like(er), at::empty_like(x)};
}
static Tensor gat_csr_meta(const Tensor &rp, const Tensor &, const Tensor &, const Tensor &, const Tensor &, const Tensor &,
                           const Tensor &, const Tensor &x, double, double) {
  return at::empty({rp.size(0) - 1, x.size(1), x.size(2)}, x.options());
}
static std::tuple<Tensor, Tensor> bias_fwd_meta(const Tensor &a, const OptT_ &, bool, double) {
  return {at::empty_like(a), at::empty({0}, a.options().dtype(at::kLong))};
}
static std::tuple<Tensor, Tensor> bias_bwd_meta(const Tensor &g, const Tensor &, bool hb, bool, double, const Tensor &) {
  const int64_t N = g.dim() > 0 ? g.size(0) : 1;
  return {at::empty_like(g), at::empty({hb && N > 0 ? g.numel() / N : 0}, g.options().dtype(at::kFloat))};
}
static Tensor bias_meta(const Tensor &a, const OptT_ &, bool, double) { return at::empty_like(a); }
static std::tuple<Tensor, Tensor> epi_fwd_meta(const Tensor &, const OptT_ &, const Tensor &x, bool, const OptT_ &, const OptT_ &,
                                               bool, double) {
  return {at::empty_like(x), at::empty({0}, x.options().dtype(at::kLong))};
}
static Tensor epi_meta(const Tensor &, const OptT_ &, const Tensor &x, bool, const OptT_ &, const OptT_ &, bool, double) {
  return at::empty_like(x);
}
static Tensor rows_meta(const Tensor &, const OptT_ &, const Tensor &x, const Tensor &rows, const OptT_ &) {
  return at::empty({rows.size(0), x.size(1)}, x.options());
}
static std::tuple<Tensor, Tensor> rows_bwd_meta(const Tensor &, const OptT_ &, const Tensor &g, const Tensor &, int64_t n_src,
                                                bool hb) {
  return {at::empty({n_src, g.size(1)}, g.options()), at::empty({hb ? g.size(1) : 0}, g.options())};
}
static Tensor seg_epi_meta(const Tensor &x, const Tensor &, int64_t N, bool, const OptT_ &, const OptT_ &, bool) {
  return at::empty(out_shape(x, N), x.options());
}

static void clear_caches() {
  seg_cache().clear();
  graph_cache().clear();
  csr_cache().clear();
  rows_cache().clear();
}
static std::vector<int64_t> plan_stats() {
  return {static_cast<int64_t>(g_plans_built.load()), static_cast<int64_t>(g_plan_hits.load())};
}

}

TORCH_LIBRARY(ggl, m) {
  m.def("segment_sum(Tensor x, Tensor index, int N) -> Tensor");
  m.def("segment_mean(Tensor x, Tensor index, int N) -> Tensor");
  m.def("segment_max(Tensor x, Tensor index, int N) -> (Tensor, Tensor)");
  m.def("segment_softmax(Tensor x, Tensor index, int N) -> Tensor");
  m.def("segment_softmax_backward(Tensor grad, Tensor y, Tensor index, int N) -> Tensor");
  m.def("spmm_sum(Tensor index, Tensor? weight, Tensor x) -> Tensor");
  m.def("spmm_mean(Tensor index, Tensor? weight, Tensor x) -> Tensor");
  m.def("spmm_max(Tensor index, Tensor? weight, Tensor x) -> Tensor");
  m.def("bspmm_sum(Tensor index, Tensor weight, Tensor x) -> Tensor");
  m.def("spmm_sum_x16(Tensor index, Tensor? weight, Tensor x, bool out_f32=False) -> Tensor");
  m.def("spmm_mean_x16(Tensor index, Tensor? weight, Tensor x, bool out_f32=False) -> Tensor");
  m.def("segment_sum_backward(Tensor grad, Tensor index, int[] x_shape) -> Tensor");
  m.def("segment_mean_backward(Tensor grad, Tensor index, int N, int[] x_shape) -> Tensor");
  m.def("segment_max_backward(Tensor grad, Tensor arg, int[] x_shape) -> Tensor");
  m.def("spmm_sum_backward(Tensor index, Tensor? weight, Tensor grad) -> Tensor");
  m.def("spmm_mean_backward(Tensor index, Tensor? weight, Tensor grad) -> Tensor");
  m.def("spmm_max_arg(Tensor index, Tensor? weight, Tensor x) -> (Tensor, Tensor)");
  m.def("spmm_max_backward(Tensor index, Tensor? weight, Tensor grad, Tensor arg) -> Tensor");
  m.def("bspmm_sum_backward(Tensor index, Tensor weight, Tensor x, Tensor grad) -> (Tensor, Tensor)");
  m.def("gat_fused(Tensor index, Tensor el, Tensor er, Tensor x, float negative_slope=0.2, int? num_nodes=None, "
        "float dropout_rate=0.0) -> Tensor");
  m.def("gat_fused_forward(Tensor index, Tensor el, Tensor er, Tensor x, float negative_slope, int num_nodes, "
        "float dropout_rate) -> (Tensor, Tensor, Tensor, Tensor, bool)");
  m.def("gat_fused_backward(Tensor index, Tensor el, Tensor er, Tensor x, Tensor grad, Tensor out, Tensor rowmax, "
        "Tensor rowden, Tensor rng_used, float negative_slope, int num_nodes, float dropout_rate, bool fast) -> "
        "(Tensor, Tensor, Tensor)");
  m.def("gat_fused_x16(Tensor index, Tensor el, Tensor er, Tensor x, float negative_slope=0.2, int? num_nodes=None, "
        "float dropout_rate=0.0, bool out_f32=False) -> Tensor");
  m.def("gat_fused_x16_forward(Tensor index, Tensor el, Tensor er, Tensor x, float negative_slope, int num_nodes, "
        "float dropout_rate, bool out_f32) -> (Tensor, Tensor, Tensor, Tensor)");
  m.def("gat_fused_csr(Tensor row_ptr, Tensor col_ind, Tensor col_ptr, Tensor row_ind, Tensor permute, Tensor el, "
        "Tensor er, Tensor x, float negative_slope=0.2, float dropout_rate=0.0) -> Tensor");
  m.def("gat_fused_csr_forward(Tensor row_ptr, Tensor col_ind, Tensor col_ptr, Tensor row_ind, Tensor permute, Tensor el, "
        "Tensor er, Tensor x, float negative_slope, float dropout_rate) -> (Tensor, Tensor, Tensor, Tensor, bool)");
  m.def("gat_fused_csr_backward(Tensor row_ptr, Tensor col_ind, Tensor col_ptr, Tensor row_ind, Tensor permute, Tensor el, "
// ... 72 lines not shown
  m.impl("bias_act", ggl_torch::bias_act_autograd);
  m.impl("spmm_epi", ggl_torch::spmm_epi_autograd);
  m.impl("segment_epi", ggl_torch::segment_epi_autograd);
  m.impl("spmm_rows", ggl_torch::spmm_rows_autograd);
}

TORCH_LIBRARY_IMPL(ggl, Meta, m) {
  m.impl("segment_sum", ggl_torch::seg_meta);
  m.impl("segment_mean", ggl_torch::seg_meta);
  m.impl("segment_max", ggl_torch::seg_max_meta);
  m.impl("segment_softmax", ggl_torch::softmax_meta);
  m.impl("segment_softmax_backward", ggl_torch::softmax_bwd_meta);
  m.impl("spmm_sum", ggl_torch::like_x_meta);
  m.impl("spmm_mean", ggl_torch::like_x_meta);
  m.impl("spmm_max", ggl_torch::like_x_meta);
  m.impl("bspmm_sum", ggl_torch::bspmm_meta);
  m.impl("spmm_sum_x16", ggl_torch::x16_meta);
  m.impl("spmm_mean_x16", ggl_torch::x16_meta);
  m.impl("segment_sum_backward", ggl_torch::seg_bwd_meta);
  m.impl("segment_mean_backward", ggl_torch::seg_mean_bwd_meta);
  m.impl("segment_max_backward", ggl_torch::seg_bwd_meta);
  m.impl("spmm_sum_backward", ggl_torch::like_x_meta);
  m.impl("spmm_mean_backward", ggl_torch::like_x_meta);
  m.impl("spmm_max_arg", ggl_torch::spmm_max_arg_meta);
  m.impl("spmm_max_backward", ggl_torch::spmm_max_bwd_meta);
  m.impl("bspmm_sum_backward", ggl_torch::bspmm_bwd_meta);
  m.impl("gat_fused", ggl_torch::gat_meta);
  m.impl("gat_fused_forward", ggl_torch::gat_fwd_meta);
  m.impl("gat_fused_x16", ggl_torch::gat_x16_meta);
  m.impl("gat_fused_x16_forward", ggl_torch::gat_x16_fwd_meta);
  m.impl("gat_fused_backward", ggl_torch::gat_bwd_meta);
  m.impl("gat_fused_csr", ggl_torch::gat_csr_meta);
  m.impl("gat_fused_csr_forward", ggl_torch::gat_csr_fwd_meta);
  m.impl("gat_fused_csr_backward", ggl_torch::gat_csr_bwd_meta);
  m.impl("bias_act", ggl_torch::bias_meta);
  m.impl("bias_act_forward", ggl_torch::bias_fwd_meta);
  m.impl("bias_act_backward", ggl_torch::bias_bwd_meta);
  m.impl("spmm_epi", ggl_torch::epi_meta);
  m.impl("spmm_epi_forward", ggl_torch::epi_fwd_meta);
  m.impl("segment_epi", ggl_torch::seg_epi_meta);
  m.impl("spmm_rows", ggl_torch::rows_meta);
  m.impl("spmm_rows_forward", ggl_torch::rows_meta);
  m.impl("spmm_rows_backward", ggl_torch::rows_bwd_meta);
  m.impl("segment_epi_forward", ggl_torch::seg_epi_meta);
}

TORCH_LIBRARY(ggl_grad, m) {
  m.def("spmm_grad_w(Tensor index, Tensor x, Tensor grad, bool mean) -> Tensor");
}
TORCH_LIBRARY_IMPL(ggl_grad, CPU, m) { m.impl("spmm_grad_w", ggl_torch::spmm_grad_w_kernel); }
TORCH_LIBRARY_IMPL(ggl_grad, CUDA, m) { m.impl("spmm_grad_w", ggl_torch::spmm_grad_w_kernel); }
TORCH_LIBRARY_IMPL(ggl_grad, Meta, m) { m.impl("spmm_grad_w", ggl_torch::spmm_grad_w_meta); }

TORCH_LIBRARY(ggl_attn, m) {
  m.def("edge_softmax_aggregate(Tensor index, Tensor logits, Tensor x, int? num_nodes=None, float dropout_rate=0.) -> Tensor");
  m.def("edge_softmax_aggregate_forward(Tensor index, Tensor logits, Tensor x, int num_nodes, float dropout_rate) -> "
        "(Tensor, Tensor, Tensor, Tensor)");
  m.def("edge_softmax_aggregate_backward(Tensor index, Tensor logits, Tensor x, Tensor grad, Tensor out, Tensor rowmax, "
        "Tensor rowden, Tensor rng_used, int num_nodes, float dropout_rate, bool need_logits, bool need_x) -> (Tensor, Tensor)");
  m.def("dot_attention(Tensor index, Tensor q, Tensor k, Tensor v, int? num_nodes=None, float? scale=None, "
        "float dropout_rate=0.) -> Tensor");
  m.def("dot_attention_forward(Tensor index, Tensor q, Tensor k, Tensor v, int num_nodes, float scale, float dropout_rate, "
        "bool keep_logits) -> (Tensor, Tensor, Tensor, Tensor, Tensor)");
  m.def("dot_attention_backward(Tensor index, Tensor q, Tensor k, Tensor v, Tensor logits, Tensor grad, Tensor out, "
        "Tensor rowmax, Tensor rowden, Tensor rng_used, int num_nodes, float scale, float dropout_rate, bool need_q, "
        "bool need_k, bool need_v) -> (Tensor, Tensor, Tensor)");
}
#define GGL_ATTN_IMPL(KEY)                                                                          \
  TORCH_LIBRARY_IMPL(ggl_attn, KEY, m) {                                                            \
    m.impl("edge_softmax_aggregate_forward", ggl_torch::esa_forward_kernel);                        \
    m.impl("edge_softmax_aggregate_backward", ggl_torch::esa_backward_kernel);                      \
    m.impl("dot_attention_forward", ggl_torch::dot_forward_kernel);                                 \
    m.impl("dot_attention_backward", ggl_torch::dot_backward_kernel);                               \
  }
GGL_ATTN_IMPL(CPU)
GGL_ATTN_IMPL(CUDA)
#undef GGL_ATTN_IMPL
TORCH_LIBRARY_IMPL(ggl_attn, Autograd, m) {
  m.impl("edge_softmax_aggregate", ggl_torch::esa_autograd);
  m.impl("dot_attention", ggl_torch::dot_autograd);
}
TORCH_LIBRARY_IMPL(ggl_attn, Meta, m) {
  m.impl("edge_softmax_aggregate", ggl_torch::esa_meta);
  m.impl("edge_softmax_aggregate_forward", ggl_torch::esa_fwd_meta);
  m.impl("edge_softmax_aggregate_backward", ggl_torch::esa_bwd_meta);
  m.impl("dot_attention", ggl_torch::dot_meta);
  m.impl("dot_attention_forward", ggl_torch::dot_fwd_meta);
  m.impl("dot_attention_backward", ggl_torch::dot_bwd_meta);
}
```

### gammagl_amd/dist.py

```python
import os
import time

import torch
import torch.distributed as dist
import torch.nn.functional as F

from . import engine as _default_engine
from .dense import wgrad

HALO_CHUNKS = int(os.environ.get("GGL_HALO_CHUNKS", "0"))
DIST_EXACT = os.environ.get("GGL_DIST_EXACT", "1") == "1"
A2A_MODE = os.environ.get("GGL_HALO_A2A", "a2a")
OUT_ROWS = os.environ.get("GGL_OUT_ROWS", "1") != "0"


def balanced_bounds(dst, num_nodes, world):
    deg = torch.bincount(dst, minlength=num_nodes)
    cum = torch.cumsum(deg, 0)
    total = int(cum[-1]) if num_nodes > 0 else 0
    targets = torch.arange(1, world, device=dst.device, dtype=torch.float64) * (total / world)
    cuts = torch.searchsorted(cum.double(), targets).clamp(max=num_nodes)
    return [0] + [int(c) for c in cuts.tolist()] + [int(num_nodes)]


class _Done:

    def wait(self):
        return True


class _Works:

    def __init__(self, works):
        self.works = list(works)

    def wait(self):
        for w in self.works:
            w.wait()
        return True


def _cpp_ops():
    from . import cpp_ops

    return cpp_ops.load()


def _default_route(eng):
    want = os.environ.get("GGL_ROUTE", "auto")
    if want not in ("auto", "cpp", "ctypes"):
        raise ValueError(f"GGL_ROUTE={want!r}: expected auto, cpp or ctypes")
    if want == "ctypes":
        return "ctypes"
    from . import cpp_ops

    product = getattr(eng, "is_product", False)
    if want == "cpp":
        if not cpp_ops.available():
            raise ImportError(f"GGL_ROUTE=cpp but {cpp_ops.LIB_PATH} is not built")
        return "cpp"
    return "cpp" if (product and cpp_ops.enabled()) else "ctypes"


class PartitionedGraph:

    def __init__(self, edge_index, edge_weight, num_nodes, rank=0, world=1, group=None, eng=None,
# ... 16 lines not shown
               send_rows=None):
        self.eng = eng if eng is not None else _default_engine()
        self.rank, self.world, self.group = rank, world, group
        self.route = _default_route(self.eng)
        self.dry = send_rows is not None
        self.comm = world > 1 or self_halo_from is not None or self.dry
        _apply_dist_exact(self)
        dev = s.device
        self.bounds = list(bounds)
        lo, hi = self.bounds[rank], self.bounds[rank + 1]
        self.lo, self.hi, self.n_local, self.n_global = lo, hi, hi - lo, int(num_nodes)
        self.e_global = int(e_global)
        self.e_local = int(s.shape[0])
        is_loc = (s >= lo) & (s < (hi if self_halo_from is None else int(self_halo_from)))
        self.ei_loc = torch.stack([s[is_loc] - lo, d[is_loc]]).contiguous()
        self.w_loc = w[is_loc].contiguous()
        self.gp_loc = self.eng.graph_plan(self.ei_loc, self.n_local, self.n_local)
        rem = ~is_loc
        rs, rd = s[rem], d[rem]
        self.halo_ids = torch.unique(rs)
        self.n_halo = int(self.halo_ids.shape[0])
        bt = torch.tensor(self.bounds, device=dev, dtype=torch.int64)
        owner_start = torch.searchsorted(self.halo_ids, bt)
        self.recv_splits = (owner_start[1:] - owner_start[:-1]).tolist()
        if self.n_halo > 0:
            self.ei_halo = torch.stack([torch.searchsorted(self.halo_ids, rs), rd]).contiguous()
            self.w_halo = w[rem].contiguous()
            self.gp_halo = self.eng.graph_plan(self.ei_halo, self.n_local, self.n_halo)
        else:
            self.ei_halo = self.w_halo = self.gp_halo = None
        del rs, rd, rem, is_loc
        if self.dry:
            self.send_splits = [int(t.numel()) for t in send_rows]
            self.send_idx = torch.cat([t.to(torch.int64) for t in send_rows]).contiguous()
        elif self.comm:
            rc = torch.tensor(self.recv_splits, device=dev, dtype=torch.int64)
            sc = torch.empty_like(rc)
            dist.all_to_all_single(sc, rc, group=group)
            self.send_splits = sc.tolist()
            req = torch.empty(int(sc.sum()), device=dev, dtype=torch.int64)
            dist.all_to_all_single(req, self.halo_ids.contiguous(), self.send_splits, self.recv_splits,
                                   group=group)
            self.send_idx = (req - lo).contiguous()
        else:
            self.send_splits = [0]
            self.send_idx = torch.empty(0, device=dev, dtype=torch.int64)
        assert self.send_idx.numel() == 0 or (int(self.send_idx.min()) >= 0 and int(self.send_idx.max()) < self.n_local)
        self.n_send = int(self.send_idx.shape[0])
        self.send_plan = self.eng.seg_plan(self.send_idx, self.n_local) if self.n_send > 0 else None
        self._bufs = {}
        self.halo_chunks = {}
        self._const = {}
        self.profile = None

    def _buf(self, tag, rows, cols, dtype, device):
        need = int(rows) * int(cols)
        b = self._bufs.get(tag)
        if b is None or b.device != device or b.dtype != dtype or b.numel() < need:
            b = torch.empty(max(need, 1), dtype=dtype, device=device)
            self._bufs[tag] = b
        return b[:need].view(int(rows), int(cols))

    def with_halo(self, x):
        if not self.comm:
            return x
        key = (x.untyped_storage()._cdata, x.storage_offset(), tuple(x.shape), x._version, str(x.device))
        hit = self._const.get(key)
        if hit is None:
            with torch.no_grad():
                xc = x.detach().contiguous()
                send = xc.index_select(0, self.send_idx) if self.n_send > 0 else xc.new_empty((0,) + tuple(xc.shape[1:]))
                recv = torch.empty((self.n_halo,) + tuple(xc.shape[1:]), dtype=xc.dtype, device=xc.device)
                if self.dry:
                    recv.zero_()
                else:
                    dist.all_to_all_single(recv, send, self.recv_splits, self.send_splits, group=self.group)
                hit = torch.cat([xc, recv], 0)
            self._const.clear()
            self._const[key] = hit
            self._const_ref = x
        return hit

    def _note(self, **kw):
        if self.profile is not None:
            for k, v in kw.items():
                self.profile[k] = self.profile.get(k, 0) + v

    def _timed_wait(self, work, dev):
        if self.profile is None:
            work.wait()
            return
        if dev.type == "cuda":
            e0, e1 = torch.cuda.Event(enable_timing=True), torch.cuda.Event(enable_timing=True)
            e0.record()
            work.wait()
            e1.record()
            self.profile.setdefault("_events", []).append((e0, e1))
        else:
            t0 = time.perf_counter()
            work.wait()
            self.profile["exposed_ms"] = self.profile.get("exposed_ms", 0.0) + (time.perf_counter() - t0) * 1e3

    def profile_summary(self, steps):
        p = dict(self.profile or {})
        ev = p.pop("_events", [])
        ms = p.pop("exposed_ms", 0.0) + sum(a.elapsed_time(b) for a, b in ev)
        s = max(int(steps), 1)
        return {"halo_exposed_ms": ms / s, "a2a_calls": p.get("a2a_calls", 0) / s,
                "a2a_GB_in": p.get("bytes_in", 0) / s / 1e9, "a2a_GB_out": p.get("bytes_out", 0) / s / 1e9}

    def _a2a(self, out_rows, inp, out_splits, in_splits, tag="a2a"):
        out = self._buf(tag, out_rows, inp.shape[1], inp.dtype, inp.device)
        self._note(a2a_calls=1, bytes_in=out.numel() * out.element_size(), bytes_out=inp.numel() * inp.element_size())
        if self.dry:
            out.zero_()
            return out, _Done()
        if A2A_MODE == "p2p":
            ops, o0, i0 = [], 0, 0
            me = dist.get_rank(self.group)
            for peer, (no, ni) in enumerate(zip(out_splits, in_splits)):
                if peer == me:
                    if no:
                        out[o0:o0 + no].copy_(inp[i0:i0 + ni])
                elif no or ni:
                    gpeer = dist.get_global_rank(self.group, peer) if self.group is not None else peer
                    if ni:
                        ops.append(dist.P2POp(dist.isend, inp[i0:i0 + ni], gpeer, group=self.group))
                    if no:
                        ops.append(dist.P2POp(dist.irecv, out[o0:o0 + no], gpeer, group=self.group))
                o0, i0 = o0 + no, i0 + ni
            return out, (_Works(dist.batch_isend_irecv(ops)) if ops else _Done())
        work = dist.all_to_all_single(out, inp, out_splits, in_splits, group=self.group, async_op=True)
        return out, work

    def release(self):
        _restore_dist_exact(self)

    def aggregate(self, h, bias=None, relu=False, p_drop=0.0, training=True, halo_included=False, out_rows=None):
        p = float(p_drop) if training else 0.0
        if out_rows is not None:
            if self.comm or halo_included or relu or p > 0 or h.shape[1] % 4 != 0:
                raise RuntimeError("aggregate(out_rows=...) is the one-GPU output layer's form: no halo, no ReLU / dropout, "
                                   "a feature width that is a multiple of 4")
            if self.route == "cpp":
                return _cpp_ops().spmm_rows(self.ei_loc, self.w_loc, h, out_rows, bias)
            return self.eng.spmm_rows(self.gp_loc, self.w_loc, h, out_rows, bias)
        if self.route == "cpp" and not self.comm and not halo_included and h.shape[1] % 4 == 0:
            return _cpp_ops().spmm_epi(self.ei_loc, self.w_loc, h, False, None, bias, bool(relu), p)
        return _HaloAggregate.apply(h, self, bias, bool(relu), p, bool(halo_included))


def _restore_dist_exact(pg):
    before = getattr(pg.eng, "_exact_before_dist", None)
    if before is not None:
        pg.eng.lib.ggl_set_option(b"exact_long_rows", int(before))
        del pg.eng._exact_before_dist


def _apply_dist_exact(pg):
    if pg.comm and not DIST_EXACT:
        if not hasattr(pg.eng, "_exact_before_dist"):
            pg.eng._exact_before_dist = int(pg.eng.lib.ggl_get_option(b"exact_long_rows"))
        pg.eng.lib.ggl_set_option(b"exact_long_rows", 0)
        import warnings

        warnings.warn("GGL_DIST_EXACT=0: library option exact_long_rows set to 0 for this process until "
                      "PartitionedGraph.release() (partitioned hub rows walk chunked)", stacklevel=3)


class _HaloAggregate(torch.autograd.Function):
    @staticmethod
    def _pad4(t):
        k = t.shape[1]
        return t if k % 4 == 0 else torch.nn.functional.pad(t, (0, (-k) % 4))

    @staticmethod
    def _chunks(K, pg=None, kind="exchange"):
        tuned = pg.halo_chunks.get(kind) if (pg is not None and K >= 128) else None
        n = HALO_CHUNKS if HALO_CHUNKS > 0 else tuned if tuned else (4 if K >= 256 else 2 if K >= 128 else 1)
        while n > 1 and K % (4 * n) != 0:
            n -= 1
        w = K // n
        return [(i * w, (i + 1) * w) for i in range(n)]

    @staticmethod
    def forward(ctx, h, pg, bias, relu, p_drop, pre=False):
        eng = pg.eng
        pre = bool(pre and pg.comm)
        if h.shape[0] != pg.n_local + (pg.n_halo if pre else 0):
            raise RuntimeError(f"aggregate: expected {pg.n_local + (pg.n_halo if pre else 0)} rows, got {h.shape[0]}")
        ctx.k_orig = h.shape[1]
        epi = bias is not None or relu or p_drop > 0
        fused = epi and h.shape[1] % 4 == 0
        h = _HaloAggregate._pad4(h.contiguous())
        K = h.shape[1]
        dev = h.device
# ... 129 lines not shown
        ctx.side, ctx.sink, ctx.pad_out = side, sink, int(pad_out)
        wt = w.t() if not pad_out else F.pad(w, (0, 0, 0, int(pad_out))).t()
        return x @ wt

    @staticmethod
    def backward(ctx, g):
        x, w = ctx.saved_tensors
        side, n_out = ctx.side, w.shape[0]
        gx = None
        if ctx.needs_input_grad[0]:
            gx = g @ (w if not ctx.pad_out else F.pad(w, (0, 0, 0, ctx.pad_out)))
        gw = None
        if ctx.needs_input_grad[1]:
            g = g.contiguous()
            if side is None or not g.is_cuda:
                gw = wgrad(g, x)[:n_out]
            else:
                cur = torch.cuda.current_stream(g.device)
                side.wait_stream(cur)
                with torch.cuda.stream(side):
                    gws = wgrad(g, x)[:n_out]
                gws.record_stream(cur)
                ctx.sink.append((w, gws, g, x))
        return gx, gw, None, None, None


class DistGCN(torch.nn.Module):

    def __init__(self, feature_dim, hidden_dim, num_class, num_layers=3, drop_rate=0.5, overlap_wgrad=True,
                 aggregate_first=False, const_input_halo=True):
        super().__init__()
        self.overlap_wgrad, self.aggregate_first = overlap_wgrad, aggregate_first
        self.const_input_halo = const_input_halo
        self.agg_per_step = 2 * num_layers
        dims = [feature_dim] + [hidden_dim] * (num_layers - 1) + [num_class]
        self.lin = torch.nn.ModuleList([torch.nn.Linear(a, b, bias=False) for a, b in zip(dims[:-1], dims[1:])])
        self.bias = torch.nn.ParameterList([torch.nn.Parameter(torch.zeros(1, b)) for b in dims[1:]])
        for lin in self.lin:
            torch.nn.init.xavier_uniform_(lin.weight)
        self.dropout = torch.nn.Dropout(drop_rate)
        self.side = None
        self._sink = []

    def join(self):
        if self.side is not None:
            torch.cuda.current_stream().wait_stream(self.side)
        for w, gw, *_held in self._sink:
            if w.grad is None:
                w.grad = gw
            else:
                w.grad.add_(gw)
        self._sink.clear()

    def forward(self, x, pg, out_rows=None):
        n = len(self.lin)
        if x.is_cuda and self.side is None and self.overlap_wgrad:
            self.side = torch.cuda.Stream(device=x.device)
        n_agg = 0
        pre = bool(self.const_input_halo and pg.comm and not x.requires_grad)
        if pre:
            x = pg.with_halo(x)
        for i in range(n):
            hidden = i < n - 1
            n_out = self.lin[i].weight.shape[0]
            pad = (-n_out) % 4 if n_out >= 8 else 0
            bias = self.bias[i] if not pad else F.pad(self.bias[i], (0, pad))
            p = self.dropout.p if hidden else 0.0
            if self.aggregate_first and x.shape[1] < n_out and x.shape[1] % 4 == 0:
                n_agg += 2 if x.requires_grad else 1
                z = pg.aggregate(x, halo_included=pre)
                h = _LinearSideWgrad.apply(z, self.lin[i].weight, self.side, self._sink, pad)
                x = pg.eng.bias_act(h, bias, relu=hidden, p_drop=p, training=self.training)
            else:
                n_agg += 2
                if pre and (n_out + pad) % 4 == 0:
                    x = _ConstInputLayer.apply(x, self.lin[i].weight, pg, bias, hidden,
                                               p if self.training else 0.0, pad)
                else:
                    h = _LinearSideWgrad.apply(x, self.lin[i].weight, self.side, self._sink, pad)
                    rows = out_rows if (i == n - 1 and out_rows is not None and not pg.comm and not pre
                                        and (n_out + pad) % 4 == 0) else None
                    x = pg.aggregate(h, bias, relu=hidden, p_drop=p, training=self.training, halo_included=pre, out_rows=rows)
                    if rows is not None:
                        out_rows = None
                        if pad:
                            x = x[:, :n_out].contiguous()
                        continue
            pre = False
            if pad:
                x = x[:, :n_out]
        self.agg_per_step = n_agg
        return x if out_rows is None else x[out_rows]


class DistGCNTrainer:
    def __init__(self, pg, feature_dim, hidden_dim, num_class, num_layers=3, drop_rate=0.5, lr=0.01,
                 l2_coef=5e-4, seed=0, device="cuda", aggregate_first=False, capturable=False, const_input_halo=True):
        self.pg = pg
        torch.manual_seed(seed)
        self.net = DistGCN(feature_dim, hidden_dim, num_class, num_layers, drop_rate,
                           aggregate_first=aggregate_first, const_input_halo=const_input_halo).to(device)
        on_gpu = torch.device(device).type == "cuda"
        try:
            self.opt = torch.optim.Adam(self.net.parameters(), lr=lr, weight_decay=l2_coef, fused=on_gpu,
                                        capturable=bool(capturable) and on_gpu)
        except (RuntimeError, TypeError):
            self.opt = torch.optim.Adam(self.net.parameters(), lr=lr, weight_decay=l2_coef)
        self.graph = None
        from .plans import _PlanCache

        self._rows_ok = _PlanCache(cap=16)
        torch.manual_seed(seed + 1000 * (pg.rank + 1))

    def _out_rows(self, train_local):
        if not OUT_ROWS or self.pg.comm or not torch.is_tensor(train_local) or train_local.dtype != torch.int64 \
                or train_local.dim() != 1:
            return None
        if int(self.pg.ei_loc.shape[1]) >= 2**31 - 1:
            return None
        ok = self._rows_ok.get(train_local, ())
        if ok is None:
            if train_local.is_cuda and torch.cuda.is_current_stream_capturing():
                return None
            t = train_local
            ok = bool(t.numel() == 0 or (int(t[0]) >= 0 and int(t[-1]) < self.pg.n_local and
                                         (t.numel() == 1 or bool((t[1:] > t[:-1]).all()))))
            self._rows_ok.put(train_local, (), ok)
        return train_local if ok else None

    def step(self, x_local, y_local, train_local, n_train_global):
        pg = self.pg
        self.net.train()
        self.opt.zero_grad(set_to_none=True)
        rows = self._out_rows(train_local)
        if rows is not None:
# ... 112 lines not shown
```

### gammagl_amd/ops.py

```python
import ctypes
import math
import os

import torch
from torch.multiprocessing.reductions import StorageWeakRef

from . import _lib, autograd
from ._lib import _DTYPE_CODE, _FLOAT_DTYPES, _X16_DTYPES, _ptr
from .plans import GraphPlan, RowsPlan, SegPlan, _PlanCache

DEFAULT_CHUNK = int(os.environ.get("GGL_LONG_ROW", "0"))


class Engine:
    def __init__(self, lib, require_cuda=True, cpu_only=False):
        self.lib = lib
        self.require_cuda = require_cuda
        self.is_product = False
        self.cpu_only = cpu_only
        self.seg_cache = _PlanCache()
        self.graph_cache = _PlanCache()
        self.w_cache = _PlanCache(cap=8)
        self.rows_cache = _PlanCache(cap=8)
        self._rng = {}
# ... 155 lines not shown

    def graph_plan(self, index, n_dst, n_src=None):
        n_src = n_dst if n_src is None else n_src
        gp = self.graph_cache.get(index, (int(n_dst), int(n_src), self.chunk))
        if gp is None:
            self._dev(index)
            if index.dim() != 2 or index.shape[0] != 2:
                raise RuntimeError("index must have shape [2, num_edges]")
            idx = index if index.dtype == torch.int64 else index.to(torch.int64)
            gp = GraphPlan(self, idx.contiguous(), n_dst, n_src)
            self.graph_cache.put(index, (int(n_dst), int(n_src), self.chunk), gp)
        else:
            self.stats["plan_hits"] += 1
        return gp

    def graph_plan_from_csr(self, row_ptr, col_ind, col_ptr, row_ind, permute, n_rows=None, n_cols=None):
        n_rows = int(row_ptr.shape[0]) - 1 if n_rows is None else int(n_rows)
        n_cols = int(col_ptr.shape[0]) - 1 if n_cols is None else int(n_cols)
        extra = ("csr", n_rows, n_cols, self.chunk) + tuple(_PlanCache.key(t, ()) for t in (col_ind, col_ptr, row_ind, permute))
        gp = self.graph_cache.get(row_ptr, extra)
        if gp is not None and any(r.expired() for r in gp.aux.get("_csr_refs", ())):
            gp = None
        if gp is None:
            gp = GraphPlan.from_csr(self, row_ptr, col_ind, col_ptr, row_ind, permute, n_rows, n_cols)
            gp.aux["_csr_refs"] = tuple(StorageWeakRef(t.untyped_storage()) for t in (col_ind, col_ptr, row_ind, permute))
            self.graph_cache.put(row_ptr, extra, gp)
        else:
            self.stats["plan_hits"] += 1
        return gp

    def rows_plan(self, gp, weight, rows):
        if rows.dim() != 1 or rows.dtype != torch.int64:
            raise RuntimeError(f"rows must be a 1-D int64 tensor, got {tuple(rows.shape)} {rows.dtype}")
        self._dev(rows, weight)
        extra = ("rows", gp.fwd.uid, gp.N_dst, gp.N_src) + (_PlanCache.key(weight, ()) if weight is not None else (None,))
        rp = self.rows_cache.get(rows, extra)
        if rp is not None and (rp.w_ref is None or not rp.w_ref.expired()):
            self.stats["plan_hits"] += 1
            return rp
        if rows.is_cuda and torch.cuda.is_current_stream_capturing():
            raise RuntimeError("spmm_rows: the restricted plan of this row list must be built before a hipGraph capture "
                               "(run one eager step first)")
        rows = rows.contiguous()
        dev, L, st = rows.device, self.lib, self._stream(rows.device)
        R, N, E = int(rows.shape[0]), gp.N_dst, gp.E
        wsb = L.ggl_plan_rows_workspace_bytes(E, max(gp.N_dst, gp.N_src), R)
        ws = torch.empty(wsb, dtype=torch.uint8, device=dev)
        rank = torch.empty(max(N, 1), dtype=torch.int32, device=dev)
        self._check(L.ggl_plan_rows_rank(_ptr(rows), R, N, _ptr(rank), _ptr(ws), wsb, st))
        bwd, colT = gp.bwd, gp.colT
        w = weight
        rp = RowsPlan()
        rp.R, rp.N_dst, rp.N_src, rp.rows = R, gp.N_dst, gp.N_src, rows
        rp.w_ref = StorageWeakRef(weight.untyped_storage()) if weight is not None else None
        rowptr_r = torch.empty(R + 1, dtype=torch.int64, device=dev)
        n = ctypes.c_int64(0)
        self._check(L.ggl_plan_rows_fwd_rowptr(_ptr(gp.fwd.rowptr), _ptr(rows), R, _ptr(rowptr_r), _ptr(ws), wsb, st,
                                               ctypes.byref(n)))
        E_r = int(n.value)
        rp.col = torch.empty(E_r, dtype=torch.int32, device=dev)
        rp.w_fwd = torch.empty(E_r, dtype=torch.float32, device=dev) if w is not None else None
        wperm = gp.fwd.perm if gp.fwd.perm is not None else gp.fwd.wperm
        self._check(L.ggl_plan_rows_fwd_fill(_ptr(gp.fwd.rowptr), _ptr(gp.col), _ptr(w), _ptr(wperm), _ptr(rows), R,
                                             _ptr(rowptr_r), E_r, _ptr(rp.col), _ptr(rp.w_fwd), st))
        rp.fwd = self.plan_from_rowptr(rowptr_r, E_r, chunk=gp.fwd.chunk)
        pos = torch.empty(E + 1, dtype=torch.int32, device=dev)
        rowptrT_r = torch.empty(gp.N_src + 1, dtype=torch.int64, device=dev)
        self._check(L.ggl_plan_rows_bwd_rowptr(_ptr(bwd.rowptr), _ptr(colT), gp.N_src, E, _ptr(rank), _ptr(pos),
                                               _ptr(rowptrT_r), _ptr(ws), wsb, st, ctypes.byref(n)))
        if int(n.value) != E_r:
            raise RuntimeError(f"restricted plans disagree: {E_r} forward elements, {int(n.value)} transposed")
        rp.colT = torch.empty(E_r, dtype=torch.int32, device=dev)
        rp.w_bwd = torch.empty(E_r, dtype=torch.float32, device=dev) if w is not None else None
        wpermT = bwd.perm if bwd.perm is not None else bwd.wperm
        self._check(L.ggl_plan_rows_bwd_fill(_ptr(colT), _ptr(w), _ptr(wpermT), E, _ptr(rank), _ptr(pos), _ptr(rp.colT),
                                             _ptr(rp.w_bwd), st))
        rp.bwd = self.plan_from_rowptr(rowptrT_r, E_r, chunk=bwd.chunk)
        del pos, rank, ws
        self.rows_cache.put(rows, extra, rp)
        return rp

    def spmm_rows(self, gp, weight, x, rows, bias=None):
        self._dev(x, weight, bias, rows)
        self._check_f32("x", x)
        if x.dim() != 2 or x.shape[1] % 4 != 0 or x.shape[1] == 0:
            raise RuntimeError(f"spmm_rows needs a 2-D f32 x whose width is a multiple of 4, got {tuple(x.shape)}")
        if int(x.shape[0]) != gp.N_src:
            raise RuntimeError(f"spmm_rows: x has {int(x.shape[0])} rows, the graph {gp.N_src} source nodes")
        if weight is not None and weight.requires_grad:
            raise RuntimeError("spmm_rows has no gradient for the edge weights: pass detached weights (c_bspmm_sum is the "
                               "op with a weight gradient)")
        weight = self._check_weight(weight, gp)
        if bias is not None:
            self._check_f32("bias", bias)
            if bias.numel() != x.shape[1]:
                raise RuntimeError("bias must hold one value per column")
        return autograd.SpMMRows.apply(self, gp, weight, x.contiguous(), rows, bias)

    def gather_i32(self, src_i64, perm):
        dev = src_i64.device
        src_i64 = src_i64.contiguous()
        E = int(src_i64.shape[0])
        out = torch.empty(E, dtype=torch.int32, device=dev)
        self._check(self.lib.ggl_gather_i64_to_i32(_ptr(src_i64), _ptr(perm), E, _ptr(out),
                                                   self._stream(dev)))
        return out

    @staticmethod
    def _hub_partial(plan, nbytes, dev):
        if plan.n_long == 0:
            return None
        return torch.empty(nbytes(plan.n_chunks) + 16, dtype=torch.uint8, device=dev)

    def _partial(self, plan, dtype, K, with_arg, dev):
        return self._hub_partial(
            plan, lambda n: self.lib.ggl_partial_bytes(_DTYPE_CODE[dtype], n, K, 1 if with_arg else 0), dev)

    def _softmax_partial(self, plan, K, dev):
        return self._hub_partial(plan, lambda n: self.lib.ggl_segment_softmax_partial_bytes(n, K), dev)

    def _gat_partial(self, plan, H, C, dev):
        return self._hub_partial(plan, lambda n: self.lib.ggl_gat_partial_bytes(n, H, C), dev)

    def _gat_sh_partial(self, plan, width, dev):
        return self._hub_partial(plan, lambda n: self.lib.ggl_gat_sh_partial_bytes(n, width), dev)

    def _softmax_width(self, x, plan):
        E = int(x.shape[0])
        if E != plan.E:
            raise IndexError("fisrt dimension of x and index should be same")
        self._check_f32("x", x)
        K = int(math.prod(x.shape[1:]))
        if not self.lib.ggl_segment_softmax_supported(K):
            raise RuntimeError(f"segment_softmax: no kernel for rows of {K} columns (ggl_segment_softmax_supported); "
                               "gammagl_amd.utils.segment_softmax composes such rows from the segment ops")
        return K

    def _softmax_fwd(self, x, plan):
        K = self._softmax_width(x, plan)
        dev = x.device
        y = torch.empty_like(x)
        part = self._softmax_partial(plan, K, dev)
        cs = plan.c_struct(part)
        self._check(self.lib.ggl_segment_softmax_fwd(_ptr(x), ctypes.byref(cs), K, _ptr(y), self._stream(dev)))
        return y

    def _softmax_bwd(self, y, g, plan):
        K = self._softmax_width(y, plan)
        dev = y.device
        g = g.contiguous()
# ... 613 lines not shown
```

### gammagl_amd/plans.py

```python
import os
from collections import OrderedDict

import torch
from torch.multiprocessing.reductions import StorageWeakRef

from ._lib import SegPlanC


class SegPlan:

    __slots__ = ("N", "E", "rowptr", "perm", "is_sorted", "max_len", "chunk", "long_rows", "chunk_ptr", "n_long", "n_chunks",
                 "device", "row_order", "uid", "xcd_run", "order_fn", "uses", "wperm", "long_order", "hub_first")

    def __init__(self, N, E, rowptr, chunk, max_len, device, perm=None, is_sorted=True, n_long=0, n_chunks=0, long_rows=None,
                 chunk_ptr=None, long_order=None, row_order=None, order_fn=None, uses=0, xcd_run=0, hub_first=False,
                 wperm=None, uid=-1):
        self.N, self.E, self.rowptr, self.chunk, self.max_len, self.device = int(N), int(E), rowptr, int(chunk), int(max_len), device
        self.perm, self.is_sorted = perm, is_sorted
        self.n_long, self.n_chunks, self.long_rows, self.chunk_ptr, self.long_order = n_long, n_chunks, long_rows, chunk_ptr, long_order
        self.row_order, self.order_fn, self.uses = row_order, order_fn, uses
        self.xcd_run, self.hub_first, self.wperm, self.uid = xcd_run, hub_first, wperm, uid

    def c_struct(self, partial=None, perm_override=None, unsplit=False, skip_long=False):
        perm = self.perm if perm_override is None else perm_override
# ... 75 lines not shown
        pos = torch.arange(S, device=self.col.device, dtype=torch.int64) * (E // S)
        rows = torch.searchsorted(self.fwd.rowptr, pos, right=True) - 1
        near = (self.col[pos].long() - rows).abs() < max(N // 64, 4096)
        return float(near.float().mean())

    def _schedule(self):
        eng = self.engine
        run = int(eng.xcd_run_rows)
        if run < 0:
            need = int(eng.lib.ggl_policy_xcd_run_rows(self.E, 1.0)) > 0 or int(eng.lib.ggl_policy_xcd_run_rows(self.E, 0.0)) > 0
            run = int(eng.lib.ggl_policy_xcd_run_rows(self.E, self.locality() if need else 0.0))
        self.fwd.xcd_run = run
        if self._bwd is not None:
            self._bwd.xcd_run = run

    @property
    def rowidx(self):
        if self._rowidx is None:
            if self.index is not None:
                self._rowidx = self.engine.gather_i32(self.index[1], self.fwd.perm)
            else:
                self._rowidx = torch.repeat_interleave(
                    torch.arange(self.N_dst, device=self.fwd.rowptr.device, dtype=torch.int32), self.fwd.counts())
        return self._rowidx

    @property
    def bwd(self):
        if self._bwd is None:
            self._bwd = self.engine.seg_plan(self.index[0], self.N_src)
            self._colT = self.engine.gather_i32(self.index[1], self._bwd.perm)
            self._bwd.xcd_run = self.fwd.xcd_run
        return self._bwd

    @property
    def colT(self):
        self.bwd
        return self._colT

    @property
    def posT(self):
        if self._posT is None:
            E, dev = self.E, self.index.device
            ar = torch.arange(E, device=dev, dtype=torch.int32)
            pf = self.fwd.perm if self.fwd.perm is not None else ar
            pt = self.bwd.perm if self.bwd.perm is not None else ar
            inv = torch.empty(E, device=dev, dtype=torch.int32)
            inv[pf.long()] = ar
            self._posT = inv[pt.long()].contiguous()
        return self._posT


class RowsPlan:

    __slots__ = ("R", "N_dst", "N_src", "rows", "fwd", "col", "w_fwd", "bwd", "colT", "w_bwd", "w_ref")


class _PlanCache:

    def __init__(self, cap=16, max_bytes=None):
        self.cap = cap
        self.max_bytes = int(float(os.environ.get("GGL_PLAN_CACHE_GB", "48")) * 2**30) if max_bytes is None else max_bytes
        self.d = OrderedDict()
        self.bytes = 0
        self.verify = os.environ.get("GGL_VERIFY_PLANS", "0") == "1"

    @staticmethod
    def key(t, extra):
        st = t.untyped_storage()
        return (st._cdata, t.storage_offset(), tuple(t.shape), tuple(t.stride()), t._version,
                t.dtype, str(t.device)) + tuple(extra)

    @staticmethod
    def _checksum(t):
        if t.numel() == 0:
            return (0, 0, 0)
        f = t.reshape(-1)
        return (int(f[0]), int(f[-1]), int(f.sum()))

    @staticmethod
    def _nbytes(val):
        if isinstance(val, SegPlan):
            own = sum(t.untyped_storage().nbytes() for t in (val.rowptr, val.perm, val.long_rows, val.chunk_ptr)
                      if t is not None)
            return own + 4 * val.N
        seen, total = set(), 0

        def visit(o, depth=0):
            nonlocal total
            if isinstance(o, torch.Tensor):
                k = o.untyped_storage()._cdata
                if k not in seen:
                    seen.add(k)
                    total += o.untyped_storage().nbytes()
            elif depth < 3 and hasattr(o, "__slots__"):
                for a in o.__slots__:
                    if a not in ("engine", "index"):
                        visit(getattr(o, a, None), depth + 1)
            elif depth < 3 and isinstance(o, dict):
                for v in o.values():
                    visit(v, depth + 1)

        visit(val)
        return total

    def get(self, t, extra):
        k = self.key(t, extra)
        hit = self.d.get(k)
# ... 29 lines not shown
```

### include/ggl_mpops.h

```cpp
#ifndef GGL_MPOPS_H
#define GGL_MPOPS_H

#include <stddef.h>
#include <stdint.h>

#ifdef __cplusplus
extern "C" {
#endif

#define GGL_ABI_VERSION 11

enum {
  GGL_U8 = 0, GGL_I8 = 1, GGL_I16 = 2, GGL_I32 = 3, GGL_I64 = 4,
  GGL_F16 = 5, GGL_BF16 = 6, GGL_F32 = 7, GGL_F64 = 8
};

enum {
  GGL_OK = 0,
  GGL_EINVAL = -1,
  GGL_EINDEX = -2,
  GGL_EDTYPE = -3,
  GGL_EHIP = -4,
  GGL_EWORKSPACE = -5
};
// ... 99 lines not shown
int ggl_spmm_mean_bwd(const ggl_segplan_t *planT, const int32_t *colT, const float *w, int w_by_pos,
                      const float *g, const int64_t *fwd_rowptr, int64_t K, float *gx,
                      void *stream);
int ggl_spmm_max_bwd(const ggl_segplan_t *planT, const int32_t *colT, const float *w, int w_by_pos,
                     const float *g, const int64_t *argsrc, int64_t K, float *gx, void *stream);
int ggl_spmm_sum_x16(const ggl_segplan_t *plan, const int32_t *col, const float *w, int w_by_pos, int x_dtype,
                     const void *x, int64_t x_ld, int64_t K, int out_dtype, void *out, int64_t out_ld, void *stream);
int ggl_spmm_mean_x16(const ggl_segplan_t *plan, const int32_t *col, const float *w, int w_by_pos, int x_dtype,
                      const void *x, int64_t x_ld, int64_t K, int out_dtype, void *out, int64_t out_ld, void *stream);
int ggl_spmm_mean_bwd_x16(const ggl_segplan_t *planT, const int32_t *colT, const float *w, int w_by_pos, int g_dtype,
                          const void *g, const int64_t *fwd_rowptr, int64_t K, int gx_dtype, void *gx, void *stream);
int64_t ggl_spmm_col_blocks_x16(const ggl_segplan_t *plan, int64_t K);
int ggl_spmm_max_bwd32(const ggl_segplan_t *planT, const int32_t *colT, const float *w, int w_by_pos,
                       const float *g, const int32_t *argsrc32, int64_t K, float *gx, void *stream);
int64_t ggl_spmm_max_mask_words(int64_t K);
size_t ggl_spmm_max_mask_bytes(int64_t E, int64_t K);
int ggl_spmm_max_mask(const ggl_segplan_t *planF, const int32_t *colF, const int64_t *argsrc, int64_t K, uint32_t *mask,
                      void *stream);
int ggl_spmm_max_bwd_mask(const ggl_segplan_t *planT, const int32_t *colT, const float *w, int w_by_pos,
                          const float *g, const uint32_t *mask, const int32_t *mask_pos, int64_t K, float *gx,
                          void *stream);

int ggl_bspmm_sum(const ggl_segplan_t *plan, const int32_t *col, const float *w, int w_by_pos,
                  const float *x, int64_t H, int64_t C, float *out, void *stream);
int ggl_bspmm_grad_w(const int64_t *index , const float *x, const float *g,
                     int64_t E, int64_t H, int64_t C, float *gw, void *stream);
size_t ggl_bspmm_grad_w_sorted_scratch_bytes(int64_t E, int64_t N, int64_t H, int64_t C);
int ggl_bspmm_grad_w_sorted(const ggl_segplan_t *plan, const int32_t *col, const int32_t *rowidx, const float *x,
                            const float *g, int64_t H, int64_t C, float *gw, float *scratch, void *stream);
size_t ggl_spmm_grad_w_scratch_bytes(int64_t E, int64_t N_dst, int64_t K, int x_dtype, int mean);
int ggl_spmm_grad_w(const ggl_segplan_t *plan, const int32_t *col, const int32_t *rowidx, int x_dtype, const void *x,
                    int g_dtype, const void *g, const int64_t *mean_rowptr, int64_t K, float *gw, void *scratch,
                    void *stream);

size_t ggl_colsum_workspace_bytes(int64_t N, int64_t K);
int ggl_colsum_f32(const float *g, int64_t N, int64_t K, float *out, void *workspace,
                   size_t workspace_bytes, void *stream);

int ggl_bias_act_fwd(const float *a, const float *bias, int64_t N, int64_t K, int relu, float p_drop,
                     int64_t *rng_state, float *y, void *stream);
int ggl_spmm_sum_bias_act(const ggl_segplan_t *plan, const int32_t *col, const float *w, int w_by_pos,
                          const float *x, int64_t K, const float *bias, int relu, float p_drop,
                          int64_t *rng_state, float *out, void *stream);
size_t ggl_bias_act_bwd_workspace_bytes(int64_t N, int64_t K);
int ggl_bias_act_bwd(const float *g, const float *y, int64_t N, int64_t K, int relu, float p_drop,
                     const int64_t *rng_used, float *ga, float *gbias, void *workspace,
                     size_t workspace_bytes, void *stream);
int ggl_bias_grad_rows(const float *g, const int64_t *rows, int64_t R, int64_t N, int64_t K, float *gbias,
                       void *workspace, size_t workspace_bytes, void *stream);
int ggl_spmm_epi_ex(const ggl_segplan_t *plan, const int32_t *col, const float *w, int w_by_pos,
                    const float *x, int64_t x_ld, int64_t K, float *out, int64_t out_ld, int accumulate,
                    int mean, const float *add, int64_t add_ld, const float *bias, int relu, float p_drop,
                    int64_t *rng_state, int64_t epi_K, int64_t epi_col0, int advance_rng, void *stream);
int ggl_spmm_epi_x16(const ggl_segplan_t *plan, const int32_t *col, const float *w, int w_by_pos, int x_dtype, const void *x,
                     int64_t x_ld, int64_t K, int out_dtype, void *out, int64_t out_ld, int mean, const void *add,
                     int64_t add_ld, const float *bias, int relu, float p_drop, int64_t *rng_state, int64_t epi_K,
                     int64_t epi_col0, int advance_rng, void *stream);
int ggl_bias_act_fwd_x16(int dtype, const void *a, const float *bias, int64_t N, int64_t K, int relu, float p_drop,
                         int64_t *rng_state, void *y, void *stream);
int ggl_bias_act_bwd_x16(int dtype, const void *g, const void *y, int64_t N, int64_t K, int relu, float p_drop,
                         const int64_t *rng_used, void *ga, float *gbias, void *workspace, size_t workspace_bytes,
                         void *stream);
int ggl_segment_epi(const float *x, const ggl_segplan_t *plan, int64_t K, int mean, const float *add,
                    int64_t add_ld, const float *bias, int relu, float p_drop, int64_t *rng_state, float *out,
                    void *stream);

int ggl_gat_fused_fwd(const ggl_segplan_t *plan, const int32_t *col, const float *el,
                      const float *er, const float *x, float slope, int64_t H, int64_t C,
                      float p_drop, int64_t *rng_state, float *out, float *rowmax, float *rowden,
                      void *stream);
size_t ggl_gat_partial_bytes(int64_t n_chunks, int64_t H, int64_t C);
int ggl_gat_fused_bwd_dst(const ggl_segplan_t *plan, const int32_t *col, const int32_t *rowidx,
                          const float *el, const float *er, const float *x, const float *g,
                          const float *out, const float *rowmax, const float *rowden, float slope,
                          int64_t H, int64_t C, float p_drop, const int64_t *rng_used, float *alpha,
                          float *de, float *ger, float *dot_ws, void *stream);
int ggl_gat_fused_bwd_src(const ggl_segplan_t *planT, const int32_t *colT, const int32_t *posT,
                          const float *alpha, const float *de, const float *g, int64_t H,
                          int64_t C, float *gx, float *gel, void *stream);
int ggl_gat_fused_fwd_x16(const ggl_segplan_t *plan, const int32_t *col, const float *el, const float *er, int x_dtype,
                          const void *x, float slope, int64_t H, int64_t C, float p_drop, int64_t *rng_state,
                          int out_dtype, void *out, float *rowmax, float *rowden, void *stream);
int ggl_gat_fused_bwd_dst_x16(const ggl_segplan_t *plan, const int32_t *col, const float *el, const float *er,
                              int x_dtype, const void *x, int g_dtype, const void *g, int out_dtype, const void *out,
                              const float *rowmax, const float *rowden, float slope, int64_t H, int64_t C, float p_drop,
                              const int64_t *rng_used, float *alpha, float *de, float *ger, void *stream);
int ggl_gat_fused_bwd_src_x16(const ggl_segplan_t *planT, const int32_t *colT, const int32_t *posT, const float *alpha,
                              const float *de, int g_dtype, const void *g, int64_t H, int64_t C, int gx_dtype, void *gx,
                              float *gel, void *stream);
int ggl_edge_softmax_agg_fwd(const ggl_segplan_t *plan, const int32_t *col, const float *z, const float *x, int64_t H,
                             int64_t C, float p_drop, int64_t *rng_state, float *out, float *rowmax, float *rowden,
                             void *stream);
int ggl_edge_softmax_agg_bwd_dst(const ggl_segplan_t *plan, const int32_t *col, const float *z, const float *x,
                                 const float *g, const float *out, const float *rowmax, const float *rowden, int64_t H,
                                 int64_t C, float p_drop, const int64_t *rng_used, float *alpha, float *gz, void *stream);
int ggl_edge_softmax_agg_bwd_src(const ggl_segplan_t *planT, const int32_t *colT, const int32_t *posT, const float *alpha,
                                 const float *g, int64_t H, int64_t C, float *gx, void *stream);
int ggl_dot_attn_supported(int64_t H, int64_t C);
int ggl_policy_dot_attn_fused(int64_t H, int64_t C, int64_t E, int64_t N_in);
int ggl_dot_attn_fwd(const ggl_segplan_t *plan, const int32_t *col, const float *q, const float *k, const float *v,
                     float scale, int64_t H, int64_t C, float p_drop, int64_t *rng_state, float *out, float *rowmax,
                     float *rowden, float *z_out, void *stream);
int ggl_gat_fast_supported(int64_t H, int64_t C);
int ggl_gat_fast_fwd(const ggl_segplan_t *plan, const int32_t *col, const float *el, const float *er,
                     const float *x, int64_t N_src, float slope, int64_t H, int64_t C, float p_drop,
                     int64_t *rng_state, float *out, float *rowmax, float *rowden, void *stream);
// ... 66 lines not shown
```

Before: 10.88 billion edges/s.

## Restrict penultimate GCN layer to source rows feeding the output rows

Adds row-restricted aggregation paths. One is a SpMM with a fused bias/ReLU/dropout epilogue over a listed subset of destination rows; the other aggregates from a compacted source set, each with a matching rows-aware backward kernel. The layer stack can now compute the second-to-last layer only for the nodes whose features the restricted last layer reads, so aggregation and epilogue work on unneeded rows is skipped. In exchange it adds extra planning work (unique sources, a rank map, a compacted backward plan) that is cached per rows tensor. On a dense R-MAT graph the needed source set may cover most nodes, and the path only runs under a HIDDEN_ROWS setting and an output-row restriction.

```diff
diff --git a/gammagl_amd/_lib.py b/gammagl_amd/_lib.py
--- a/gammagl_amd/_lib.py
+++ b/gammagl_amd/_lib.py
@@ -106,6 +106,9 @@
     "ggl_bias_act_bwd": (c_int, [_V, _V, c_int64, c_int64, c_int, c_float, _V, _V, _V, _V, c_size_t, _V]),
     "ggl_spmm_epi_ex": (c_int, [_P, _V, _V, c_int, _V, c_int64, c_int64, _V, c_int64, c_int, c_int, _V, c_int64,
                                 _V, c_int, c_float, _V, c_int64, c_int64, c_int, _V]),
+    "ggl_spmm_rows_epi": (c_int, [_P, _V, _V, c_int, _V, c_int64, c_int64, _V, c_int64, _V, c_int64, _V, c_int, c_float, _V,
+                                  c_int64, c_int64, c_int, _V]),
+    "ggl_bias_act_bwd_rows": (c_int, [_V, _V, _V, c_int64, c_int64, c_int64, c_int, c_float, _V, c_int, _V, _V, _V, c_size_t, _V]),
     "ggl_spmm_epi_x16": (c_int, [_P, _V, _V, c_int, c_int, _V, c_int64, c_int64, c_int, _V, c_int64, c_int, _V, c_int64,
                                  _V, c_int, c_float, _V, c_int64, c_int64, c_int, _V]),
     "ggl_bias_act_fwd_x16": (c_int, [c_int, _V, _V, c_int64, c_int64, c_int, c_float, _V, _V, _V]),
diff --git a/gammagl_amd/autograd.py b/gammagl_amd/autograd.py
--- a/gammagl_amd/autograd.py
+++ b/gammagl_amd/autograd.py
@@ -615,3 +615,97 @@
             gx = torch.empty((rp.N_src, K), dtype=torch.float32, device=dev)
             eng.spmm_sum_into(rp.bwd, rp.colT, rp.w_bwd, g, gx)
         return None, None, None, gx, None, gb
+
+
+class SpMMRowsEpi(torch.autograd.Function):
+
+    @staticmethod
+    def forward(ctx, eng, gp, w, x, rows, bias, relu, p_drop, full=False):
+        ctx.eng = eng
+        dev = x.device
+        K = int(x.shape[1])
+        rp = eng.rows_plan(gp, w, rows)
+        rng, rng_used = eng._draw(dev, p_drop)
+        b, _ = _flat(bias)
+        if full:
+            y = torch.empty((gp.N_dst, K), dtype=torch.float32, device=dev)
+            eng.spmm_epi_into(gp.fwd, gp.col, w, x, y, bias=b, relu=relu, p_drop=p_drop, rng=rng)
+        else:
+            y = torch.empty((rp.R, K), dtype=torch.float32, device=dev)
+            plan = rp.fwd
+            part = eng._partial(plan, torch.float32, K, False, dev)
+            ww, w_by_pos, wp = eng._weights(plan, rp.w_fwd)
+            cs = plan.c_struct(part, wp)
+            eng._check(eng.lib.ggl_spmm_rows_epi(ctypes.byref(cs), _ptr(rp.col), _ptr(ww), w_by_pos, _ptr(x), K, K, _ptr(y), K,
+                                                 _ptr(rp.rows), rp.N_dst, _ptr(b), int(relu), float(p_drop), _ptr(rng), 0, 0, 1,
+                                                 eng._stream(dev)))
+        ctx.rp, ctx.K, ctx.full = rp, K, bool(full)
+        ctx.epi = (relu, p_drop, rng_used, None if bias is None else bias.shape)
+        ctx.save_for_backward(y if (relu or p_drop > 0) else None)
+        return y
+
+    @staticmethod
+    @once_differentiable
+    def backward(ctx, g):
+        eng, rp, K = ctx.eng, ctx.rp, ctx.K
+        relu, p_drop, rng_used, bshape = ctx.epi
+        (y,) = ctx.saved_tensors
+        g = g.contiguous()
+        dev = g.device
+        masked = relu or p_drop > 0
+        if ctx.full and not masked:
+            g = g.index_select(0, rp.rows)
+        ga, gb = g, None
+        if masked or bshape is not None:
+            ga = torch.empty((rp.R, K), dtype=torch.float32, device=dev) if masked else g
+            gb = torch.empty(K, dtype=torch.float32, device=dev) if bshape is not None else None
+            wsb = eng.lib.ggl_bias_act_bwd_workspace_bytes(rp.N_dst, K)
+            ws = torch.empty(max(wsb, 4), dtype=torch.uint8, device=dev)
+            if relu or p_drop > 0:
+                eng._check(eng.lib.ggl_bias_act_bwd_rows(_ptr(g), _ptr(y), _ptr(rp.rows), rp.R, rp.N_dst, K, int(relu),
+                                                         float(p_drop), _ptr(rng_used), int(ctx.full), _ptr(ga), _ptr(gb),
+                                                         _ptr(ws), wsb, eng._stream(dev)))
+            else:
+                eng._check(eng.lib.ggl_bias_grad_rows(_ptr(g), _ptr(rp.rows), rp.R, rp.N_dst, K, _ptr(gb), _ptr(ws), wsb,
+                                                      eng._stream(dev)))
+            gb = gb.reshape(bshape) if gb is not None else None
+        gx = None
+        if ctx.needs_input_grad[3]:
+            gx = torch.empty((rp.N_src, K), dtype=torch.float32, device=dev)
+            eng.spmm_sum_into(rp.bwd, rp.colT, rp.w_bwd, ga, gx)
+        return None, None, None, gx, None, gb, None, None, None
+
+
+class SpMMRowsFrom(torch.autograd.Function):
+
+    @staticmethod
+    def forward(ctx, eng, gp, w, x, rows, src_rows, bias):
+        ctx.eng = eng
+        K = int(x.shape[1])
+        rp = eng.rows_plan(gp, w, rows)
+        col_c, bwd_c = eng.rows_src_plan(rp, src_rows)
+        y = torch.empty((rp.R, K), dtype=torch.float32, device=x.device)
+        b, _ = _flat(bias)
+        eng.spmm_epi_into(rp.fwd, col_c, rp.w_fwd, x, y, bias=b)
+        ctx.rp, ctx.bwd_c, ctx.bshape, ctx.K = rp, bwd_c, (None if bias is None else bias.shape), K
+        return y
+
+    @staticmethod
+    @once_differentiable
+    def backward(ctx, g):
+        eng, rp, K = ctx.eng, ctx.rp, ctx.K
+        g = g.contiguous()
+        dev = g.device
+        gb = None
+        if ctx.bshape is not None and ctx.needs_input_grad[6]:
+            gb = torch.empty(K, dtype=torch.float32, device=dev)
+            wsb = eng.lib.ggl_bias_act_bwd_workspace_bytes(rp.N_dst, K)
+            ws = torch.empty(max(wsb, 4), dtype=torch.uint8, device=dev)
+            eng._check(eng.lib.ggl_bias_grad_rows(_ptr(g), _ptr(rp.rows), rp.R, rp.N_dst, K, _ptr(gb), _ptr(ws), wsb,
+                                                  eng._stream(dev)))
+            gb = gb.reshape(ctx.bshape)
+        gx = None
+        if ctx.needs_input_grad[3]:
+            gx = torch.empty((ctx.bwd_c.N, K), dtype=torch.float32, device=dev)
+            eng.spmm_sum_into(ctx.bwd_c, rp.colT, rp.w_bwd, g, gx)
+        return None, None, None, gx, None, None, gb
diff --git a/gammagl_amd/cpp_ops.py b/gammagl_amd/cpp_ops.py
--- a/gammagl_amd/cpp_ops.py
+++ b/gammagl_amd/cpp_ops.py
@@ -33,3 +33,8 @@
 def load_attn():
     load()
     return torch.ops.ggl_attn
+
+
+def load_rows():
+    load()
+    return torch.ops.ggl_rows
diff --git a/gammagl_amd/csrc/epilogue.hip b/gammagl_amd/csrc/epilogue.hip
--- a/gammagl_amd/csrc/epilogue.hip
+++ b/gammagl_amd/csrc/epilogue.hip
@@ -201,6 +201,55 @@
     }
 #pragma unroll
     for (int k = 0; k < 4; ++k) partial[(block_id() * groups + j) * K + c * 4 + k] = acc[k];
+  }
+}
+
+template <int MASKED>
+__global__ __launch_bounds__(kBlock) void bias_act_bwd_rows_kernel(const float *__restrict__ g, const float *__restrict__ y,
+                                                                   float *__restrict__ ga, const int64_t *__restrict__ rows,
+                                                                   int64_t R, int64_t N, int64_t K, int64_t nblocks,
+                                                                   int64_t rows_per_block, int kp, int groups, float scale,
+                                                                   const int64_t *__restrict__ rng, uint32_t drop_thresh,
+                                                                   float *__restrict__ partial, int gy_full) {
+  const int j = threadIdx.x / kp;
+  const int c0 = threadIdx.x - j * kp;
+  if (j >= groups || block_id() >= nblocks) return;
+  const int64_t KV = K / 4;
+  const int64_t r0 = block_id() * rows_per_block;
+  const int64_t r1 = (r0 + rows_per_block < N) ? r0 + rows_per_block : N;
+  int64_t lo = 0, hi = R;
+  while (lo < hi) {
+    const int64_t mid = (lo + hi) >> 1;
+    if (rows[mid] < r0) lo = mid + 1; else hi = mid;
+  }
+  for (int64_t c = c0; c < KV; c += kp) {
+    float acc[4] = {0.0f, 0.0f, 0.0f, 0.0f};
+    for (int64_t i = lo; i < R; ++i) {
+      const int64_t r = rows[i];
+      if (r >= r1) break;
+      if ((int)(r - r0) % groups != j) continue;
+      float gv[4], yv[4] = {0.0f, 0.0f, 0.0f, 0.0f};
+      const int64_t gi = gy_full ? r : i;
+      ldv<float, 4>(g + gi * K + c * 4, gv);
+      if (MASKED == 1 || MASKED == 2) ldv<float, 4>(y + gi * K + c * 4, yv);
+      uint32_t rw[4] = {0xffffffffu, 0xffffffffu, 0xffffffffu, 0xffffffffu};
+      if (MASKED == 3) {
+        const U4 u = philox4x32_10((uint64_t)(r * KV + c), (uint64_t)rng[1], (uint64_t)rng[0]);
+        rw[0] = u.x; rw[1] = u.y; rw[2] = u.z; rw[3] = u.w;
+      }
+#pragma unroll
+      for (int k = 0; k < 4; ++k) {
+        if (MASKED == 1) gv[k] = (yv[k] > 0.0f) ? __fmul_rn(gv[k], scale) : 0.0f;
+        else if (MASKED == 2) gv[k] = (yv[k] != 0.0f) ? __fmul_rn(gv[k], scale) : 0.0f;
+        else if (MASKED == 3) gv[k] = (rw[k] >= drop_thresh) ? __fmul_rn(gv[k], scale) : 0.0f;
+        acc[k] = __fadd_rn(acc[k], gv[k]);
+      }
+      stv<float, 4>(ga + i * K + c * 4, gv);
+    }
+    if (partial) {
+#pragma unroll
+      for (int k = 0; k < 4; ++k) partial[(block_id() * groups + j) * K + c * 4 + k] = acc[k];
+    }
   }
 }
 
@@ -336,6 +385,42 @@
              : bias_act_bwd<mxf16_t>(g16, y16, N, K, relu, p_drop, rng_used, ga16, gbias, workspace, workspace_bytes, stream);
 }
 
+extern "C" int ggl_bias_act_bwd_rows(const float *g, const float *y, const int64_t *rows, int64_t R, int64_t N, int64_t K,
+                                     int relu, float p_drop, const int64_t *rng_used, int gy_full, float *ga, float *gbias,
+                                     void *workspace, size_t workspace_bytes, void *stream) {
+  GGL_REQUIRE(R >= 0 && N >= 0 && R <= N && K > 0 && K % 4 == 0 && p_drop >= 0.0f && p_drop < 1.0f, GGL_EINVAL,
+              "bias_act_bwd_rows needs R <= N rows of a multiple of 4 columns and p_drop in [0, 1)");
+  GGL_REQUIRE((g && ga && rows) || R == 0, GGL_EINVAL, "NULL pointer");
+  const bool redraw = p_drop > 0.0f && rng_used != nullptr && !relu;
+  const int masked = relu ? 1 : (redraw ? 3 : (p_drop > 0.0f ? 2 : 0));
+  GGL_REQUIRE(!masked || masked == 3 || y || R == 0, GGL_EINVAL, "y is needed to rebuild the ReLU/dropout mask");
+  GGL_REQUIRE(aligned16(g) && aligned16(ga) && (masked == 0 || masked == 3 || aligned16(y)), GGL_EINVAL,
+              "g, y and ga must be 16-byte aligned");
+  GGL_REQUIRE(!gbias || (workspace && workspace_bytes >= ggl_bias_act_bwd_workspace_bytes(N, K)), GGL_EWORKSPACE,
+              "bias_act_bwd_rows workspace too small (ggl_bias_act_bwd_workspace_bytes(N, K))");
+  if (R == 0 && !gbias) return GGL_OK;
+  uint32_t thresh;
+  float scale;
+  dropout_params(p_drop, &thresh, &scale);
+  int kp, groups;
+  int64_t blocks, rpb;
+  geometry(N, K, true, &kp, &groups, &blocks, &rpb);
+  hipStream_t s = as_stream(stream);
+  float *partial = gbias ? static_cast<float *>(workspace) : nullptr;
+#define GGL_BABR(M)                                                                                                     \
+  GGL_LAUNCH((bias_act_bwd_rows_kernel<M>), blocks, kBlock, s, g, y, ga, rows, R, N, K, blocks, rpb, kp, groups, scale, \
+             redraw ? rng_used : nullptr, thresh, partial, gy_full ? 1 : 0)
+  if (masked == 0) GGL_BABR(0); else if (masked == 1) GGL_BABR(1); else if (masked == 2) GGL_BABR(2); else GGL_BABR(3);
+#undef GGL_BABR
+  GGL_LAUNCH_CHECK();
+  if (gbias) {
+    const size_t part = bwd_partial_bytes(N, K);
+    return ggl_colsum_f32(partial, blocks * groups, K, gbias, static_cast<char *>(workspace) + part, workspace_bytes - part,
+                          stream);
+  }
+  return GGL_OK;
+}
+
 extern "C" int ggl_bias_grad_rows(const float *g, const int64_t *rows, int64_t R, int64_t N, int64_t K, float *gbias,
                                   void *workspace, size_t workspace_bytes, void *stream) {
   GGL_REQUIRE(R >= 0 && N >= 0 && R <= N && K > 0 && K % 4 == 0, GGL_EINVAL,
diff --git a/gammagl_amd/csrc/reduce.hip b/gammagl_amd/csrc/reduce.hip
--- a/gammagl_amd/csrc/reduce.hip
+++ b/gammagl_amd/csrc/reduce.hip
@@ -42,6 +42,7 @@
   int64_t add_ld;
   int64_t mask_words;
   int64_t mask_col0;
+  const int64_t *epi_rows;
 };
 
 template <typename S> struct RPtrs {
@@ -332,6 +333,7 @@
 #pragma unroll
   for (int i = 0; i < (VEC > 4 ? VEC : 4); ++i) rw[i] = 0xffffffffu;
   if (!d.epi_thresh) return;
+  if (d.epi_rows) row = d.epi_rows[row];
   const int64_t ev = d.epi_vec;
   const int sh = ev == 4 ? 2 : 0;
   const int64_t KV = (d.epi_K + ev - 1) >> sh;
@@ -583,6 +585,7 @@
   const void *epi_add;
   int64_t add_ld;
   int64_t epi_K, epi_col0;
+  const int64_t *epi_rows;
   int phase;
   int hub_forked;
   int64_t mask_words;
@@ -719,6 +722,7 @@
   d.add_ld = a.add_ld > 0 ? a.add_ld : a.K;
   d.mask_words = a.mask_words;
   d.mask_col0 = 0;
+  d.epi_rows = a.epi_rows;
   const int64_t kv = ceil_div(a.K, VEC);
   d.logL = pow2_ceil_log2(kv < kWave ? kv : kWave);
   if (d.logL > 6) d.logL = 6;
@@ -1100,6 +1104,29 @@
   return GGL_OK;
 }
 
+extern "C" int ggl_spmm_rows_epi(const ggl_segplan_t *plan, const int32_t *col, const float *w, int w_by_pos,
+                                 const float *x, int64_t x_ld, int64_t K, float *out, int64_t out_ld,
+                                 const int64_t *rows, int64_t N_full, const float *bias, int relu, float p_drop,
+                                 int64_t *rng_state, int64_t epi_K, int64_t epi_col0, int advance_rng, void *stream) {
+  ReduceArgs a{};
+  int rc = spmm_common(a, plan, col, w, w_by_pos, x, K, out, false);
+  if (rc) return rc;
+  GGL_REQUIRE(K % 4 == 0, GGL_EINVAL, "spmm_rows_epi needs a multiple of 4 columns");
+  GGL_REQUIRE((x_ld == 0 || x_ld >= K) && (out_ld == 0 || out_ld >= K), GGL_EINVAL, "row stride < K");
+  GGL_REQUIRE(rows || plan->N == 0, GGL_EINVAL, "rows is NULL");
+  GGL_REQUIRE(N_full >= plan->N, GGL_EINVAL, "more listed rows than the graph has");
+  rc = fill_epilogue(a, nullptr, 0, bias, relu, p_drop, rng_state);
+  if (rc) return rc;
+  GGL_REQUIRE(epi_col0 >= 0 && (epi_K == 0 || epi_col0 + K <= epi_K), GGL_EINVAL, "column block outside the row");
+  a.x_ld = x_ld; a.out_ld = out_ld;
+  a.epi_K = epi_K; a.epi_col0 = epi_col0;
+  a.epi_rows = rows;
+  rc = launch_f32_cols<OP_SUM, MODE_SPMM_EPI>(a, as_stream(stream));
+  if (rc) return rc;
+  if (a.epi_thresh && advance_rng && N_full > 0 && K > 0) return rng_advance(rng_state, stream);
+  return GGL_OK;
+}
+
 extern "C" int ggl_spmm_sum_bias_act(const ggl_segplan_t *plan, const int32_t *col, const float *w,
                                      int w_by_pos, const float *x, int64_t K, const float *bias, int relu,
                                      float p_drop, int64_t *rng_state, float *out, void *stream) {
diff --git a/gammagl_amd/csrc/torch/ggl_torch.cpp b/gammagl_amd/csrc/torch/ggl_torch.cpp
--- a/gammagl_amd/csrc/torch/ggl_torch.cpp
+++ b/gammagl_amd/csrc/torch/ggl_torch.cpp
@@ -45,7 +45,8 @@
   X(ggl_policy_softmax_sublanes) X(ggl_spmm_sum_x16) X(ggl_spmm_mean_x16) X(ggl_spmm_mean_bwd_x16)                    \
   X(ggl_plan_rows_workspace_bytes) X(ggl_plan_rows_rank) X(ggl_plan_rows_fwd_rowptr) X(ggl_plan_rows_fwd_fill)        \
   X(ggl_plan_rows_bwd_rowptr) X(ggl_plan_rows_bwd_fill) X(ggl_bias_grad_rows)                                          \
-  X(ggl_spmm_epi_x16) X(ggl_bias_act_fwd_x16) X(ggl_bias_act_bwd_x16)
+  X(ggl_spmm_epi_x16) X(ggl_bias_act_fwd_x16) X(ggl_bias_act_bwd_x16)                                                  \
+  X(ggl_spmm_rows_epi) X(ggl_bias_act_bwd_rows)
 
 struct Api {
   void *handle = nullptr;
@@ -1409,6 +1410,13 @@
   const void *w_storage = nullptr;
   int64_t w_offset = 0, w_version = 0;
   c10::optional<c10::weak_intrusive_ptr<c10::StorageImpl>> w_ref;
+  Tensor srcs;
+  Tensor c_col;
+  std::shared_ptr<SegPlan> c_bwd;
+  const void *c_storage = nullptr;
+  int64_t c_offset = 0, c_numel = 0, c_version = 0;
+  c10::optional<c10::weak_intrusive_ptr<c10::StorageImpl>> c_ref;
+  std::mutex mu;
 };
 
 static Cache<RowsPlan> &rows_cache() {
@@ -1548,6 +1556,207 @@
   return {gx, gb};
 }
 
+static void no_capture(const c10::Device &dev, const char *what) {
+  TORCH_CHECK(!capturing(dev), what, " must be built before a hipGraph capture (run one eager step first)");
+}
+
+static Tensor rows_sources_kernel(const Tensor &index, const OptT_ &weight, const Tensor &rows, int64_t n) {
+  Tensor w = opt_dense(weight);
+  same_device({&index, &w, &rows});
+  if (w.defined()) f32("weight", w);
+  c10::OptionalDeviceGuard guard(rows.device());
+  auto gp = graph_plan(index, n, n);
+  auto rp = rows_plan(*gp, index, w, rows);
+  std::lock_guard<std::mutex> lock(rp->mu);
+  if (!rp->srcs.defined()) {
+    no_capture(rows.device(), "rows_sources: the source list");
+    rp->srcs = std::get<0>(at::_unique(rp->col, true, false)).to(at::kLong);
+  } else {
+    ++g_plan_hits;
+  }
+  return rp->srcs;
+}
+
+struct SrcPlan {
+  Tensor col;
+  std::shared_ptr<SegPlan> bwd;
+};
+static SrcPlan rows_src_plan(RowsPlan &rp, const Tensor &src_in) {
+  TORCH_CHECK(src_in.dim() == 1 && src_in.scalar_type() == at::kLong, "src_rows must be a 1-D int64 tensor, got ", src_in.sizes(),
+              " ", src_in.scalar_type());
+  const void *storage = src_in.storage().unsafeGetStorageImpl();
+  const int64_t offset = src_in.storage_offset(), numel = src_in.numel();
+  const int64_t version = src_in.is_inference() ? 0 : static_cast<int64_t>(src_in._version());
+  std::lock_guard<std::mutex> lock(rp.mu);
+  if (rp.c_bwd && rp.c_storage == storage && rp.c_offset == offset && rp.c_numel == numel && rp.c_version == version &&
+      !rp.c_ref->expired()) {
+    ++g_plan_hits;
+    return {rp.c_col, rp.c_bwd};
+  }
+  const auto dev = src_in.device();
+  no_capture(dev, "spmm_rows_from: the compacted-source plan");
+  const Api &a = api_for(dev);
+  void *st = stream_of(dev);
+  Tensor src = src_in.contiguous();
+  const int64_t S = src.size(0), E_r = rp.col.size(0);
+  const size_t wsb = a.ggl_plan_rows_workspace_bytes(E_r, rp.N_src, S);
+  Tensor ws = at::empty({static_cast<int64_t>(wsb)}, src.options().dtype(at::kByte));
+  Tensor rank = at::empty({std::max<int64_t>(rp.N_src, 1)}, src.options().dtype(at::kInt));
+  check(a, a.ggl_plan_rows_rank(src.data_ptr<int64_t>(), S, rp.N_src, rank.data_ptr<int32_t>(), ws.data_ptr(), wsb, st));
+  Tensor col_c = rank.index_select(0, rp.col.to(at::kLong));
+  TORCH_CHECK(E_r == 0 || col_c.min().item<int32_t>() >= 0,
+              "src_rows does not hold every source of the edges into the listed rows");
+  Tensor rowptr_c = at::cat({rp.bwd->rowptr.index_select(0, src), rp.bwd->rowptr.slice(0, rp.N_src, rp.N_src + 1)});
+  rp.c_bwd = plan_from_rowptr(a, rowptr_c, E_r, rp.bwd->chunk, st);
+  rp.c_col = col_c;
+  rp.c_storage = storage;
+  rp.c_offset = offset;
+  rp.c_numel = numel;
+  rp.c_version = version;
+  rp.c_ref = src_in.storage().getWeakStorageImpl();
+  return {rp.c_col, rp.c_bwd};
+}
+
+static Tensor rows_bias(const OptT_ &bias_, int64_t K) {
+  Tensor bias = opt(bias_);
+  if (bias.defined()) {
+    f32("bias", bias);
+    bias = bias.contiguous().reshape({-1});
+    TORCH_CHECK(bias.numel() == K, "bias must hold one value per column");
+  }
+  return bias;
+}
+
+static std::tuple<Tensor, Tensor> spmm_rows_epi_forward_kernel(const Tensor &index, const OptT_ &weight, const Tensor &x,
+                                                               const Tensor &rows, const OptT_ &bias_, bool relu, double p,
+                                                               bool full) {
+  c10::OptionalDeviceGuard guard(x.device());
+  SpArgs s = spmm_args(index, weight, x);
+  same_device({&x, &rows});
+  TORCH_CHECK(s.x.dim() == 2 && s.x.size(1) > 0 && s.x.size(1) % 4 == 0,
+              "spmm_rows_epi needs a 2-D f32 x whose width is a multiple of 4, got ", x.sizes());
+  TORCH_CHECK(p >= 0.0 && p < 1.0, "p_drop must be in [0, 1)");
+  const Api &a = api_for(x.device());
+  const int64_t K = s.x.size(1);
+  Tensor bias = rows_bias(bias_, K);
+  same_device({&x, &bias});
+  auto rp = rows_plan(*s.gp, index, s.w, rows);
+  if (full)
+    return spmm_epi_forward_kernel(index, weight, x, false, OptT_(), bias_, relu, p);
+  const SegPlan &p_ = *rp->fwd;
+  Tensor y = at::empty({rp->R, K}, s.x.options());
+  Tensor part = partial_for(a, p_, s.x, K, false);
+  ggl_segplan_t cs = p_.c(part);
+  const Draw d = draw(x.device(), p);
+  check(a, a.ggl_spmm_rows_epi(&cs, rp->col.data_ptr<int32_t>(), rp->has_w ? rp->w_fwd.data_ptr<float>() : nullptr, 1,
+                               s.x.data_ptr<float>(), K, K, y.data_ptr<float>(), K, rp->rows.data_ptr<int64_t>(), rp->N_dst,
+                               bias.defined() ? bias.data_ptr<float>() : nullptr, relu ? 1 : 0, static_cast<float>(p), d.ptr(),
+                               0, 0, 1, stream_of(x.device())));
+  return {y, d.used};
+}
+
+static std::tuple<Tensor, Tensor> spmm_rows_epi_backward_kernel(const Tensor &index, const OptT_ &weight, const Tensor &grad,
+                                                                const Tensor &y, const Tensor &rows, int64_t n_src,
+                                                                bool has_bias, bool relu, double p, const Tensor &rng_used,
+                                                                bool full) {
+  Tensor g = grad.contiguous(), w = opt_dense(weight);
+  f32("grad", g);
+  if (w.defined()) f32("weight", w);
+  c10::OptionalDeviceGuard guard(g.device());
+  const Api &a = api_for(g.device());
+  auto gp = bwd_plan(index, n_src);
+  auto rp = rows_plan(*gp, index, w, rows);
+  TORCH_CHECK(g.dim() == 2 && g.size(0) == (full ? rp->N_dst : rp->R) && g.size(1) % 4 == 0,
+              "grad must be [len(rows), K] ([N, K] for the full form), K a multiple of 4");
+  const int64_t K = g.size(1);
+  void *st = stream_of(g.device());
+  const bool masked = relu || p > 0;
+  if (full && !masked) g = g.index_select(0, rp->rows);
+  Tensor ga = g, gb = at::empty({has_bias ? K : 0}, g.options());
+  if (masked || has_bias) {
+    const size_t wsb = a.ggl_bias_act_bwd_workspace_bytes(rp->N_dst, K);
+    Tensor ws = at::empty({static_cast<int64_t>(std::max<size_t>(wsb, 4))}, g.options().dtype(at::kByte));
+    if (masked) {
+      Tensor yc = y.contiguous();
+      TORCH_CHECK(yc.sizes() == g.sizes() && yc.scalar_type() == at::kFloat, "y must be the forward's f32 output, shaped like grad");
+      ga = at::empty({rp->R, K}, g.options());
+      check(a, a.ggl_bias_act_bwd_rows(g.data_ptr<float>(), yc.data_ptr<float>(), rp->rows.data_ptr<int64_t>(), rp->R,
+                                       rp->N_dst, K, relu ? 1 : 0, static_cast<float>(p), used_ptr(p, rng_used), full ? 1 : 0,
+                                       ga.data_ptr<float>(), has_bias ? gb.data_ptr<float>() : nullptr, ws.data_ptr(), wsb, st));
+    } else {
+      check(a, a.ggl_bias_grad_rows(g.data_ptr<float>(), rp->rows.data_ptr<int64_t>(), rp->R, rp->N_dst, K,
+                                    gb.data_ptr<float>(), ws.data_ptr(), wsb, st));
+    }
+  }
+  const SegPlan &p_ = *rp->bwd;
+  Tensor gx = at::empty({rp->N_src, K}, g.options());
+  Tensor part = partial_for(a, p_, g, K, false);
+  ggl_segplan_t cs = p_.c(part);
+  check(a, a.ggl_spmm_sum(&cs, rp->colT.data_ptr<int32_t>(), rp->has_w ? rp->w_bwd.data_ptr<float>() : nullptr, 1,
+                          ga.data_ptr<float>(), K, gx.data_ptr<float>(), st));
+  return {gx, gb};
+}
+
+static Tensor spmm_rows_from_forward_kernel(const Tensor &index, const OptT_ &weight, const Tensor &x, const Tensor &rows,
+                                            const Tensor &src_rows, int64_t n, const OptT_ &bias_) {
+  c10::OptionalDeviceGuard guard(x.device());
+  Tensor w = opt_dense(weight), xc = x.contiguous();
+  same_device({&index, &w, &x, &rows, &src_rows});
+  f32("x", xc);
+  if (w.defined()) f32("weight", w);
+  TORCH_CHECK(xc.dim() == 2 && xc.size(1) > 0 && xc.size(1) % 4 == 0,
+              "spmm_rows_from needs a 2-D f32 x whose width is a multiple of 4, got ", x.sizes());
+  TORCH_CHECK(src_rows.dim() == 1 && xc.size(0) == src_rows.size(0), "spmm_rows_from: x has ", xc.size(0), " rows, src_rows ",
+              src_rows.numel(), " entries");
+  const Api &a = api_for(x.device());
+  const int64_t K = xc.size(1);
+  Tensor bias = rows_bias(bias_, K);
+  same_device({&x, &bias});
+  auto gp = graph_plan(index, n, n);
+  if (w.defined()) TORCH_CHECK(w.dim() == 1 && w.size(0) == gp->E, "edge weight must hold one value per edge: got ", w.sizes(),
+                               " for ", gp->E, " edges");
+  auto rp = rows_plan(*gp, index, w, rows);
+  SrcPlan cp = rows_src_plan(*rp, src_rows);
+  const SegPlan &p_ = *rp->fwd;
+  Tensor y = at::empty({rp->R, K}, xc.options());
+  Tensor part = partial_for(a, p_, xc, K, false);
+  ggl_segplan_t cs = p_.c(part);
+  check(a, a.ggl_spmm_epi_ex(&cs, cp.col.data_ptr<int32_t>(), rp->has_w ? rp->w_fwd.data_ptr<float>() : nullptr, 1,
+                             xc.data_ptr<float>(), K, K, y.data_ptr<float>(), K, 0, 0, nullptr, 0,
+                             bias.defined() ? bias.data_ptr<float>() : nullptr, 0, 0.0f, nullptr, 0, 0, 1, stream_of(x.device())));
+  return y;
+}
+
+static std::tuple<Tensor, Tensor> spmm_rows_from_backward_kernel(const Tensor &index, const OptT_ &weight, const Tensor &grad,
+                                                                 const Tensor &rows, const Tensor &src_rows, int64_t n,
+                                                                 bool has_bias) {
+  Tensor g = grad.contiguous(), w = opt_dense(weight);
+  f32("grad", g);
+  if (w.defined()) f32("weight", w);
+  c10::OptionalDeviceGuard guard(g.device());
+  const Api &a = api_for(g.device());
+  auto gp = bwd_plan(index, n);
+  auto rp = rows_plan(*gp, index, w, rows);
+  SrcPlan cp = rows_src_plan(*rp, src_rows);
+  TORCH_CHECK(g.dim() == 2 && g.size(0) == rp->R && g.size(1) % 4 == 0, "grad must be [len(rows), K], K a multiple of 4");
+  const int64_t K = g.size(1);
+  void *st = stream_of(g.device());
+  Tensor gb = at::empty({has_bias ? K : 0}, g.options());
+  if (has_bias) {
+    const size_t wsb = a.ggl_bias_act_bwd_workspace_bytes(rp->N_dst, K);
+    Tensor ws = at::empty({static_cast<int64_t>(std::max<size_t>(wsb, 4))}, g.options().dtype(at::kByte));
+    check(a, a.ggl_bias_grad_rows(g.data_ptr<float>(), rp->rows.data_ptr<int64_t>(), rp->R, rp->N_dst, K, gb.data_ptr<float>(),
+                                  ws.data_ptr(), wsb, st));
+  }
+  const SegPlan &p_ = *cp.bwd;
+  Tensor gx = at::empty({p_.N, K}, g.options());
+  Tensor part = partial_for(a, p_, g, K, false);
+  ggl_segplan_t cs = p_.c(part);
+  check(a, a.ggl_spmm_sum(&cs, rp->colT.data_ptr<int32_t>(), rp->has_w ? rp->w_bwd.data_ptr<float>() : nullptr, 1,
+                          g.data_ptr<float>(), K, gx.data_ptr<float>(), st));
+  return {gx, gb};
+}
+
 static Tensor segment_epi_forward_kernel(const Tensor &x_, const Tensor &index, int64_t N, bool mean, const OptT_ &add_,
                                          const OptT_ &bias_, bool relu) {
   seg_args(x_, index);
@@ -2013,6 +2222,67 @@
   return SpMMRowsFn::apply(index, weight, x, rows, bias);
 }
 
+struct SpMMRowsEpiFn : public torch::autograd::Function<SpMMRowsEpiFn> {
+  static Tensor forward(AutogradContext *ctx, const Tensor &index, const OptT_ &weight, const Tensor &x, const Tensor &rows,
+                        const OptT_ &bias, bool relu, double p, bool full) {
+    at::AutoDispatchBelowADInplaceOrView below;
+    static auto op = op_handle<std::tuple<Tensor, Tensor>(const Tensor &, const OptT_ &, const Tensor &, const Tensor &,
+                                                          const OptT_ &, bool, double, bool)>("ggl_rows::spmm_rows_epi_forward");
+    auto r = op.call(index, weight, x, rows, bias, relu, p, full);
+    ctx->saved_data["full"] = full;
+    ctx->save_for_backward({index, opt(weight), rows, std::get<0>(r), std::get<1>(r)});
+    ctx->saved_data["n_src"] = x.size(0);
+    ctx->saved_data["relu"] = relu;
+    ctx->saved_data["p"] = p;
+    save_bias(ctx, bias);
+    return std::get<0>(r);
+  }
+  static variable_list backward(AutogradContext *ctx, variable_list grads) {
+    auto s = ctx->get_saved_variables();
+    static auto op = op_handle<std::tuple<Tensor, Tensor>(const Tensor &, const OptT_ &, const Tensor &, const Tensor &,
+                                                          const Tensor &, int64_t, bool, bool, double, const Tensor &, bool)>(
+        "ggl_rows::spmm_rows_epi_backward");
+    OptT_ w = s[1].defined() ? OptT_(s[1]) : OptT_();
+    auto r = op.call(s[0], w, grads[0], s[3], s[2], ctx->saved_data["n_src"].toInt(), has_bias(ctx),
+                     ctx->saved_data["relu"].toBool(), ctx->saved_data["p"].toDouble(), s[4], ctx->saved_data["full"].toBool());
+    return {Tensor(), Tensor(), std::get<0>(r), Tensor(), bias_grad(ctx, std::get<1>(r)), Tensor(), Tensor(), Tensor()};
+  }
+};
+static Tensor spmm_rows_epi_autograd(const Tensor &index, const OptT_ &weight, const Tensor &x, const Tensor &rows,
+                                     const OptT_ &bias, bool relu, double p, bool full) {
+  TORCH_CHECK(!(opt(weight).defined() && opt(weight).requires_grad()),
+              "spmm_rows_epi has no gradient for the edge weights: pass detached weights (bspmm_sum is the op with a weight gradient)");
+  return SpMMRowsEpiFn::apply(index, weight, x, rows, bias, relu, p, full);
+}
+
+struct SpMMRowsFromFn : public torch::autograd::Function<SpMMRowsFromFn> {
+  static Tensor forward(AutogradContext *ctx, const Tensor &index, const OptT_ &weight, const Tensor &x, const Tensor &rows,
+                        const Tensor &src_rows, int64_t n, const OptT_ &bias) {
+    at::AutoDispatchBelowADInplaceOrView below;
+    static auto op = op_handle<Tensor(const Tensor &, const OptT_ &, const Tensor &, const Tensor &, const Tensor &, int64_t,
+                                      const OptT_ &)>("ggl_rows::spmm_rows_from_forward");
+    Tensor y = op.call(index, weight, x, rows, src_rows, n, bias);
+    ctx->save_for_backward({index, opt(weight), rows, src_rows});
+    ctx->saved_data["n"] = n;
+    save_bias(ctx, bias);
+    return y;
+  }
+  static variable_list backward(AutogradContext *ctx, variable_list grads) {
+    auto s = ctx->get_saved_variables();
+    static auto op = op_handle<std::tuple<Tensor, Tensor>(const Tensor &, const OptT_ &, const Tensor &, const Tensor &,
+                                                          const Tensor &, int64_t, bool)>("ggl_rows::spmm_rows_from_backward");
+    OptT_ w = s[1].defined() ? OptT_(s[1]) : OptT_();
+    auto r = op.call(s[0], w, grads[0], s[2], s[3], ctx->saved_data["n"].toInt(), has_bias(ctx));
+    return {Tensor(), Tensor(), std::get<0>(r), Tensor(), Tensor(), Tensor(), bias_grad(ctx, std::get<1>(r))};
+  }
+};
+static Tensor spmm_rows_from_autograd(const Tensor &index, const OptT_ &weight, const Tensor &x, const Tensor &rows,
+                                      const Tensor &src_rows, int64_t n, const OptT_ &bias) {
+  TORCH_CHECK(!(opt(weight).defined() && opt(weight).requires_grad()),
+              "spmm_rows_from has no gradient for the edge weights: pass detached weights (bspmm_sum is the op with a weight gradient)");
+  return SpMMRowsFromFn::apply(index, weight, x, rows, src_rows, n, bias);
+}
+
 struct SegEpiFn : public torch::autograd::Function<SegEpiFn> {
   static Tensor forward(AutogradContext *ctx, const Tensor &x, const Tensor &index, int64_t N, bool mean, const OptT_ &add,
                         const OptT_ &bias, bool relu) {
@@ -2172,6 +2442,26 @@
 static std::tuple<Tensor, Tensor> rows_bwd_meta(const Tensor &, const OptT_ &, const Tensor &g, const Tensor &, int64_t n_src,
                                                 bool hb) {
   return {at::empty({n_src, g.size(1)}, g.options()), at::empty({hb ? g.size(1) : 0}, g.options())};
+}
+static Tensor rows_epi_meta(const Tensor &, const OptT_ &, const Tensor &x, const Tensor &rows, const OptT_ &, bool, double,
+                            bool full) {
+  return at::empty({full ? x.size(0) : rows.size(0), x.size(1)}, x.options());
+}
+static std::tuple<Tensor, Tensor> rows_epi_fwd_meta(const Tensor &, const OptT_ &, const Tensor &x, const Tensor &rows,
+                                                    const OptT_ &, bool, double, bool full) {
+  return {at::empty({full ? x.size(0) : rows.size(0), x.size(1)}, x.options()), at::empty({0}, x.options().dtype(at::kLong))};
+}
+static std::tuple<Tensor, Tensor> rows_epi_bwd_meta(const Tensor &, const OptT_ &, const Tensor &g, const Tensor &, const Tensor &,
+                                                    int64_t n_src, bool hb, bool, double, const Tensor &, bool) {
+  return {at::empty({n_src, g.size(1)}, g.options()), at::empty({hb ? g.size(1) : 0}, g.options())};
+}
+static Tensor rows_from_meta(const Tensor &, const OptT_ &, const Tensor &x, const Tensor &rows, const Tensor &, int64_t,
+                             const OptT_ &) {
+  return at::empty({rows.size(0), x.size(1)}, x.options());
+}
+static std::tuple<Tensor, Tensor> rows_from_bwd_meta(const Tensor &, const OptT_ &, const Tensor &g, const Tensor &,
+                                                     const Tensor &src_rows, int64_t, bool hb) {
+  return {at::empty({src_rows.size(0), g.size(1)}, g.options()), at::empty({hb ? g.size(1) : 0}, g.options())};
 }
 static Tensor seg_epi_meta(const Tensor &x, const Tensor &, int64_t N, bool, const OptT_ &, const OptT_ &, bool) {
   return at::empty(out_shape(x, N), x.options());
@@ -2350,6 +2640,46 @@
 TORCH_LIBRARY_IMPL(ggl_grad, CUDA, m) { m.impl("spmm_grad_w", ggl_torch::spmm_grad_w_kernel); }
 TORCH_LIBRARY_IMPL(ggl_grad, Meta, m) { m.impl("spmm_grad_w", ggl_torch::spmm_grad_w_meta); }
 
+TORCH_LIBRARY(ggl_rows, m) {
+  m.def("rows_sources(Tensor index, Tensor? weight, Tensor rows, int num_nodes) -> Tensor");
+  m.def("spmm_rows_epi(Tensor index, Tensor? weight, Tensor x, Tensor rows, Tensor? bias=None, bool relu=False, "
+        "float p_drop=0.0, bool full=False) -> Tensor");
+  m.def("spmm_rows_epi_forward(Tensor index, Tensor? weight, Tensor x, Tensor rows, Tensor? bias, bool relu, float p_drop, "
+        "bool full) -> "
+        "(Tensor, Tensor)");
+  m.def("spmm_rows_epi_backward(Tensor index, Tensor? weight, Tensor grad, Tensor y, Tensor rows, int n_src, bool has_bias, "
+        "bool relu, float p_drop, Tensor rng_used, bool full) -> (Tensor, Tensor)");
+  m.def("spmm_rows_from(Tensor index, Tensor? weight, Tensor x, Tensor rows, Tensor src_rows, int num_nodes, "
+        "Tensor? bias=None) -> Tensor");
+  m.def("spmm_rows_from_forward(Tensor index, Tensor? weight, Tensor x, Tensor rows, Tensor src_rows, int num_nodes, "
+        "Tensor? bias) -> Tensor");
+  m.def("spmm_rows_from_backward(Tensor index, Tensor? weight, Tensor grad, Tensor rows, Tensor src_rows, int num_nodes, "
+        "bool has_bias) -> (Tensor, Tensor)");
+}
+#define GGL_ROWS_IMPL(KEY)                                                                \
+  TORCH_LIBRARY_IMPL(ggl_rows, KEY, m) {                                                  \
+    m.impl("rows_sources", ggl_torch::rows_sources_kernel);                               \
+    m.impl("spmm_rows_epi_forward", ggl_torch::spmm_rows_epi_forward_kernel);             \
+    m.impl("spmm_rows_epi_backward", ggl_torch::spmm_rows_epi_backward_kernel);           \
+    m.impl("spmm_rows_from_forward", ggl_torch::spmm_rows_from_forward_kernel);           \
+    m.impl("spmm_rows_from_backward", ggl_torch::spmm_rows_from_backward_kernel);         \
+  }
+GGL_ROWS_IMPL(CPU)
+GGL_ROWS_IMPL(CUDA)
+#undef GGL_ROWS_IMPL
+TORCH_LIBRARY_IMPL(ggl_rows, Autograd, m) {
+  m.impl("spmm_rows_epi", ggl_torch::spmm_rows_epi_autograd);
+  m.impl("spmm_rows_from", ggl_torch::spmm_rows_from_autograd);
+}
+TORCH_LIBRARY_IMPL(ggl_rows, Meta, m) {
+  m.impl("spmm_rows_epi", ggl_torch::rows_epi_meta);
+  m.impl("spmm_rows_epi_forward", ggl_torch::rows_epi_fwd_meta);
+  m.impl("spmm_rows_epi_backward", ggl_torch::rows_epi_bwd_meta);
+  m.impl("spmm_rows_from", ggl_torch::rows_from_meta);
+  m.impl("spmm_rows_from_forward", ggl_torch::rows_from_meta);
+  m.impl("spmm_rows_from_backward", ggl_torch::rows_from_bwd_meta);
+}
+
 TORCH_LIBRARY(ggl_attn, m) {
   m.def("edge_softmax_aggregate(Tensor index, Tensor logits, Tensor x, int? num_nodes=None, float dropout_rate=0.) -> Tensor");
   m.def("edge_softmax_aggregate_forward(Tensor index, Tensor logits, Tensor x, int num_nodes, float dropout_rate) -> "
diff --git a/gammagl_amd/dist.py b/gammagl_amd/dist.py
--- a/gammagl_amd/dist.py
+++ b/gammagl_amd/dist.py
@@ -12,6 +12,8 @@
 DIST_EXACT = os.environ.get("GGL_DIST_EXACT", "1") == "1"
 A2A_MODE = os.environ.get("GGL_HALO_A2A", "a2a")
 OUT_ROWS = os.environ.get("GGL_OUT_ROWS", "1") != "0"
+HIDDEN_ROWS = int(os.environ.get("GGL_HIDDEN_ROWS", "1"))
+HIDDEN_ROWS_MAX_SHARE = 0.75
 
 
 def balanced_bounds(dst, num_nodes, world):
@@ -134,6 +136,7 @@
         self.halo_chunks = {}
         self._const = {}
         self.profile = None
+        self._hidden = None
 
     def _buf(self, tag, rows, cols, dtype, device):
         need = int(rows) * int(cols)
@@ -218,12 +221,50 @@
     def release(self):
         _restore_dist_exact(self)
 
-    def aggregate(self, h, bias=None, relu=False, p_drop=0.0, training=True, halo_included=False, out_rows=None):
+    def hidden_rows(self, out_rows):
+        if not HIDDEN_ROWS or self.comm:
+            return None
+        if self._hidden is None:
+            from .plans import _PlanCache
+
+            self._hidden = _PlanCache(cap=4)
+        extra = (self.route, HIDDEN_ROWS_MAX_SHARE)
+        hit = self._hidden.get(out_rows, extra)
+        if hit is None:
+            if out_rows.is_cuda and torch.cuda.is_current_stream_capturing():
+                return None
+            if self.route == "cpp":
+                from . import cpp_ops
+
+                r1 = cpp_ops.load_rows().rows_sources(self.ei_loc, self.w_loc, out_rows, self.n_local)
+            else:
+                r1 = self.eng.rows_sources(self.gp_loc, self.w_loc, out_rows)
+            hit = (r1 if int(r1.numel()) <= HIDDEN_ROWS_MAX_SHARE * self.n_local else False,)
+            self._hidden.put(out_rows, extra, hit)
+        return hit[0] if hit[0] is not False else None
+
+    def aggregate(self, h, bias=None, relu=False, p_drop=0.0, training=True, halo_included=False, out_rows=None,
+                  hidden_rows=None, src_rows=None, bwd_only=False):
         p = float(p_drop) if training else 0.0
+        if hidden_rows is not None:
+            if self.comm or halo_included or out_rows is not None or src_rows is not None or h.shape[1] % 4 != 0:
+                raise RuntimeError("aggregate(hidden_rows=...) is the one-GPU form of the last hidden layer: no halo, a feature "
+                                   "width that is a multiple of 4")
+            if self.route == "cpp":
+                from . import cpp_ops
+
+                return cpp_ops.load_rows().spmm_rows_epi(self.ei_loc, self.w_loc, h, hidden_rows, bias, bool(relu), p, bool(bwd_only))
+            return self.eng.spmm_rows_epi(self.gp_loc, self.w_loc, h, hidden_rows, bias, relu, p, full=bwd_only)
         if out_rows is not None:
             if self.comm or halo_included or relu or p > 0 or h.shape[1] % 4 != 0:
                 raise RuntimeError("aggregate(out_rows=...) is the one-GPU output layer's form: no halo, no ReLU / dropout, "
                                    "a feature width that is a multiple of 4")
+            if src_rows is not None:
+                if self.route == "cpp":
+                    from . import cpp_ops
+
+                    return cpp_ops.load_rows().spmm_rows_from(self.ei_loc, self.w_loc, h, out_rows, src_rows, self.n_local, bias)
+                return self.eng.spmm_rows_from(self.gp_loc, self.w_loc, h, out_rows, src_rows, bias)
             if self.route == "cpp":
                 return _cpp_ops().spmm_rows(self.ei_loc, self.w_loc, h, out_rows, bias)
             return self.eng.spmm_rows(self.gp_loc, self.w_loc, h, out_rows, bias)
@@ -459,11 +500,18 @@
                 w.grad.add_(gw)
         self._sink.clear()
 
+    def _restricts_output(self, pg):
+        n_out = self.lin[-1].weight.shape[0]
+        pad = (-n_out) % 4 if n_out >= 8 else 0
+        agg_first = self.aggregate_first and self.lin[-1].weight.shape[1] < n_out and self.lin[-1].weight.shape[1] % 4 == 0
+        return not pg.comm and (n_out + pad) % 4 == 0 and not agg_first
+
     def forward(self, x, pg, out_rows=None):
         n = len(self.lin)
         if x.is_cuda and self.side is None and self.overlap_wgrad:
             self.side = torch.cuda.Stream(device=x.device)
         n_agg = 0
+        src_rows = None
         pre = bool(self.const_input_halo and pg.comm and not x.requires_grad)
         if pre:
             x = pg.with_halo(x)
@@ -487,7 +535,19 @@
                     h = _LinearSideWgrad.apply(x, self.lin[i].weight, self.side, self._sink, pad)
                     rows = out_rows if (i == n - 1 and out_rows is not None and not pg.comm and not pre
                                         and (n_out + pad) % 4 == 0) else None
-                    x = pg.aggregate(h, bias, relu=hidden, p_drop=p, training=self.training, halo_included=pre, out_rows=rows)
+                    if i == n - 2 and out_rows is not None and not pre and (n_out + pad) % 4 == 0 and self._restricts_output(pg):
+                        src_rows = pg.hidden_rows(out_rows)
+                        if src_rows is not None:
+                            compact = int(HIDDEN_ROWS) >= 2
+                            x = pg.aggregate(h, bias, relu=hidden, p_drop=p, training=self.training, hidden_rows=src_rows,
+                                             bwd_only=not compact)
+                            if pad:
+                                x = x[:, :n_out]
+                            if not compact:
+                                src_rows = None
+                            continue
+                    x = pg.aggregate(h, bias, relu=hidden, p_drop=p, training=self.training, halo_included=pre, out_rows=rows,
+                                     src_rows=src_rows if rows is not None else None)
                     if rows is not None:
                         out_rows = None
                         if pad:
diff --git a/gammagl_amd/ops.py b/gammagl_amd/ops.py
--- a/gammagl_amd/ops.py
+++ b/gammagl_amd/ops.py
@@ -231,6 +231,7 @@
         w = weight
         rp = RowsPlan()
         rp.R, rp.N_dst, rp.N_src, rp.rows = R, gp.N_dst, gp.N_src, rows
+        rp.srcs = rp.cpair = None
         rp.w_ref = StorageWeakRef(weight.untyped_storage()) if weight is not None else None
         rowptr_r = torch.empty(R + 1, dtype=torch.int64, device=dev)
         n = ctypes.c_int64(0)
@@ -261,20 +262,74 @@
 
     def spmm_rows(self, gp, weight, x, rows, bias=None):
         self._dev(x, weight, bias, rows)
+        weight = self._check_rows_op("spmm_rows", gp, weight, x, bias, gp.N_src)
+        return autograd.SpMMRows.apply(self, gp, weight, x.contiguous(), rows, bias)
+
+    def _no_capture(self, t, what):
+        if t.is_cuda and torch.cuda.is_current_stream_capturing():
+            raise RuntimeError(f"{what} must be built before a hipGraph capture (run one eager step first)")
+
+    def rows_sources(self, gp, weight, rows):
+        rp = self.rows_plan(gp, weight, rows)
+        if rp.srcs is None:
+            self._no_capture(rows, "rows_sources: the source list")
+            rp.srcs = torch.unique(rp.col).to(torch.int64)
+        else:
+            self.stats["plan_hits"] += 1
+        return rp.srcs
+
+    def rows_src_plan(self, rp, src_rows):
+        key = _PlanCache.key(src_rows, ())
+        hit = rp.cpair
+        if hit is not None and hit[0] == key and not hit[1].expired():
+            self.stats["plan_hits"] += 1
+            return hit[2], hit[3]
+        if src_rows.dim() != 1 or src_rows.dtype != torch.int64:
+            raise RuntimeError(f"src_rows must be a 1-D int64 tensor, got {tuple(src_rows.shape)} {src_rows.dtype}")
+        self._no_capture(src_rows, "spmm_rows_from: the compacted-source plan")
+        src = src_rows.contiguous()
+        dev, L, st = src.device, self.lib, self._stream(src.device)
+        S, E_r = int(src.shape[0]), int(rp.col.shape[0])
+        wsb = L.ggl_plan_rows_workspace_bytes(E_r, rp.N_src, S)
+        ws = torch.empty(wsb, dtype=torch.uint8, device=dev)
+        rank = torch.empty(max(rp.N_src, 1), dtype=torch.int32, device=dev)
+        self._check(L.ggl_plan_rows_rank(_ptr(src), S, rp.N_src, _ptr(rank), _ptr(ws), wsb, st))
+        col_c = rank[rp.col.long()]
+        if E_r > 0 and int(col_c.min()) < 0:
+            raise RuntimeError("src_rows does not hold every source of the edges into the listed rows")
+        rowptr_c = torch.cat([rp.bwd.rowptr[src], rp.bwd.rowptr[-1:]])
+        bwd_c = self.plan_from_rowptr(rowptr_c, E_r, chunk=rp.bwd.chunk)
+        rp.cpair = (key, StorageWeakRef(src_rows.untyped_storage()), col_c, bwd_c)
+        return col_c, bwd_c
+
+    def _check_rows_op(self, what, gp, weight, x, bias, n_rows):
         self._check_f32("x", x)
         if x.dim() != 2 or x.shape[1] % 4 != 0 or x.shape[1] == 0:
-            raise RuntimeError(f"spmm_rows needs a 2-D f32 x whose width is a multiple of 4, got {tuple(x.shape)}")
-        if int(x.shape[0]) != gp.N_src:
-            raise RuntimeError(f"spmm_rows: x has {int(x.shape[0])} rows, the graph {gp.N_src} source nodes")
+            raise RuntimeError(f"{what} needs a 2-D f32 x whose width is a multiple of 4, got {tuple(x.shape)}")
+        if int(x.shape[0]) != n_rows:
+            raise RuntimeError(f"{what}: x has {int(x.shape[0])} rows, expected {n_rows}")
         if weight is not None and weight.requires_grad:
-            raise RuntimeError("spmm_rows has no gradient for the edge weights: pass detached weights (c_bspmm_sum is the "
+            raise RuntimeError(f"{what} has no gradient for the edge weights: pass detached weights (c_bspmm_sum is the "
                                "op with a weight gradient)")
         weight = self._check_weight(weight, gp)
         if bias is not None:
             self._check_f32("bias", bias)
             if bias.numel() != x.shape[1]:
                 raise RuntimeError("bias must hold one value per column")
-        return autograd.SpMMRows.apply(self, gp, weight, x.contiguous(), rows, bias)
+        return weight
+
+    def spmm_rows_epi(self, gp, weight, x, rows, bias=None, relu=False, p_drop=0.0, training=True, full=False):
+        self._dev(x, weight, bias, rows)
+        weight = self._check_rows_op("spmm_rows_epi", gp, weight, x, bias, gp.N_src)
+        p = float(p_drop) if training else 0.0
+        if not 0.0 <= p < 1.0:
+            raise RuntimeError("p_drop must be in [0, 1)")
+        return autograd.SpMMRowsEpi.apply(self, gp, weight, x.contiguous(), rows, bias, bool(relu), p, bool(full))
+
+    def spmm_rows_from(self, gp, weight, x, rows, src_rows, bias=None):
+        self._dev(x, weight, bias, rows, src_rows)
+        weight = self._check_rows_op("spmm_rows_from", gp, weight, x, bias, int(src_rows.shape[0]))
+        return autograd.SpMMRowsFrom.apply(self, gp, weight, x.contiguous(), rows, src_rows, bias)
 
     def gather_i32(self, src_i64, perm):
         dev = src_i64.device
diff --git a/gammagl_amd/plans.py b/gammagl_amd/plans.py
--- a/gammagl_amd/plans.py
+++ b/gammagl_amd/plans.py
@@ -151,7 +151,7 @@
 
 class RowsPlan:
 
-    __slots__ = ("R", "N_dst", "N_src", "rows", "fwd", "col", "w_fwd", "bwd", "colT", "w_bwd", "w_ref")
+    __slots__ = ("R", "N_dst", "N_src", "rows", "fwd", "col", "w_fwd", "bwd", "colT", "w_bwd", "w_ref", "srcs", "cpair")
 
 
 class _PlanCache:
diff --git a/include/ggl_mpops.h b/include/ggl_mpops.h
--- a/include/ggl_mpops.h
+++ b/include/ggl_mpops.h
@@ -175,6 +175,13 @@
                     const float *x, int64_t x_ld, int64_t K, float *out, int64_t out_ld, int accumulate,
                     int mean, const float *add, int64_t add_ld, const float *bias, int relu, float p_drop,
                     int64_t *rng_state, int64_t epi_K, int64_t epi_col0, int advance_rng, void *stream);
+int ggl_spmm_rows_epi(const ggl_segplan_t *plan, const int32_t *col, const float *w, int w_by_pos, const float *x,
+                      int64_t x_ld, int64_t K, float *out, int64_t out_ld, const int64_t *rows, int64_t N_full,
+                      const float *bias, int relu, float p_drop, int64_t *rng_state, int64_t epi_K, int64_t epi_col0,
+                      int advance_rng, void *stream);
+int ggl_bias_act_bwd_rows(const float *g, const float *y, const int64_t *rows, int64_t R, int64_t N, int64_t K, int relu,
+                          float p_drop, const int64_t *rng_used, int gy_full, float *ga, float *gbias, void *workspace,
+                          size_t workspace_bytes, void *stream);
 int ggl_spmm_epi_x16(const ggl_segplan_t *plan, const int32_t *col, const float *w, int w_by_pos, int x_dtype, const void *x,
                      int64_t x_ld, int64_t K, int out_dtype, void *out, int64_t out_ld, int mean, const void *add,
                      int64_t add_ld, const float *bias, int relu, float p_drop, int64_t *rng_state, int64_t epi_K,
```

Result: faster. 11.13 billion edges/s (median of 6 runs) (+2.3%).
